# kohnakagawa/md_neighbor_list

Hardware: AMD Instinct MI355X
Metric: Verlet-list build ms and Mpairs/s at N=1M rho=1.0; achieved HBM GB/s (higher is better)
Workload: dtype f32

## Files before the change

### include/nl_hip.h

```cpp
#ifndef NL_HIP_H
#define NL_HIP_H

#include <stddef.h>
#include <stdint.h>

#ifdef __cplusplus
extern "C" {
#endif

typedef struct nl_handle_s* nl_handle_t;

typedef enum nl_dtype {
  NL_F32 = 0,
  NL_F64 = 1
} nl_dtype;

typedef enum nl_status {
  NL_OK = 0,
  NL_ERR_ARG = 1,
  NL_ERR_NOMEM = 2,
  NL_ERR_OUT_OF_BOX = 3,
  NL_ERR_CAPACITY = 4,
  NL_ERR_HIP = 5,
  NL_ERR_STATE = 6,
// ... 20 lines not shown

int nl_set_graph(nl_handle_t h, int on);

int nl_set_periodic(nl_handle_t h, int minimum_image);

int nl_set_periodic_axes(nl_handle_t h, int mask);
int nl_get_periodic_axes(nl_handle_t h, int* mask);

int nl_set_box(nl_handle_t h, double Lx, double Ly, double Lz, double xy, double xz, double yz);
int nl_get_box(nl_handle_t h, double box[6]);

int nl_destroy(nl_handle_t h);


int nl_make_list(nl_handle_t h, const void* q_dev, int32_t q_stride, int32_t n, void* stream, int sync);

#define NL_GID_IN_W ((const int32_t*)1)
int nl_make_list_slab(nl_handle_t h, const void* q_dev, int32_t q_stride, const int32_t* gid_dev, int32_t n_rows,
                      int32_t n, int32_t z_lo, int32_t z_hi, void* stream, int sync);

int nl_make_list_slab_begin(nl_handle_t h, const void* q_dev, int32_t q_stride, const int32_t* gid_dev, int32_t n_rows,
                            int32_t n, int32_t n_ghost_lo, int32_t z_lo, int32_t z_hi, void* stream);
int nl_make_list_slab_finish(nl_handle_t h, void* stream, int sync);

int nl_set_local_ids(nl_handle_t h, int on);
int nl_get_local_ids(nl_handle_t h, int* on);


typedef struct nl_comm_s* nl_comm_t;
#define NL_UNIQUE_ID_BYTES 128
typedef int (*nl_sendrecv_fn)(void* user, int peer_to, const void* send, size_t send_bytes, int peer_from, void* recv,
                              size_t recv_bytes);
int nl_comm_unique_id(void* id_out );
int nl_comm_create(nl_comm_t* out, int rank, int world, const void* unique_id, int device_id);
int nl_comm_create_callbacks(nl_comm_t* out, int rank, int world, nl_sendrecv_fn fn, void* user, int device_id);
int nl_comm_destroy(nl_comm_t comm);
int nl_comm_layers(nl_handle_t h, nl_comm_t comm, int32_t* z_lo, int32_t* z_hi);
int nl_make_list_distributed(nl_handle_t h, nl_comm_t comm, void* q_dev, int32_t q_capacity, int32_t n_owned, void* stream,
                             int sync);
int nl_distributed_ghosts(nl_comm_t comm, int32_t* n_ghost_lo, int32_t* n_ghost_hi);

int nl_synchronize(nl_handle_t h);


int nl_set_skin(nl_handle_t h, double skin);
int nl_update_list(nl_handle_t h, const void* q_dev, int32_t q_stride, int32_t n, void* stream, int sync);
int nl_get_update_stats(nl_handle_t h, int64_t stats[2]);


int nl_set_exclusions(nl_handle_t h, const int32_t* pairs_dev, int64_t n_pairs, int32_t n);
int nl_set_exclusions_global(nl_handle_t h, const int32_t* pairs_dev, int64_t n_pairs, int32_t n_ids);
int nl_get_exclusions(nl_handle_t h, const int32_t** offsets_dev, const int32_t** ids_dev, int32_t* n, int64_t* n_unique);


#define NL_MAX_TYPES 32
int nl_set_type_cutoffs(nl_handle_t h, const int32_t* types_dev, int32_t n, int32_t ntypes, const double* rc_host);
int nl_get_types(nl_handle_t h, const int32_t** types_dev, int32_t* n, int32_t* ntypes);


int nl_set_pair_images(nl_handle_t h, int on);
int nl_get_pair_images(nl_handle_t h, const int8_t** images_dev, int64_t* nentries);
int nl_pair_vectors(nl_handle_t h, const void* q_dev, int32_t q_stride, void* out_dev, void* stream);
int nl_pair_vectors_enqueue(nl_handle_t h, const void* q_dev, int32_t q_stride, void* out_dev, void* stream);


int nl_get_half_csr(nl_handle_t h, const int32_t** key_pointer_dev, const int32_t** sorted_list_dev,
                    const int32_t** number_of_partners_dev, int64_t* npairs);

int nl_get_full_csr(nl_handle_t h, const int32_t** key_pointer_dev, const int32_t** list_dev,
                    const int32_t** number_of_partners_dev, int64_t* nentries);

int nl_get_half_csr64(nl_handle_t h, const int64_t** key_pointer_dev, const int32_t** sorted_list_dev,
                      const int32_t** number_of_partners_dev, int64_t* npairs);
int nl_get_full_csr64(nl_handle_t h, const int64_t** key_pointer_dev, const int32_t** list_dev,
                      const int32_t** number_of_partners_dev, int64_t* nentries);

int nl_list_checksum(nl_handle_t h, uint64_t* checksum, int64_t* nentries);

int nl_get_full_transposed(nl_handle_t h, const int32_t** list_dev, const int32_t** count_dev, int64_t* row_stride,
                           int32_t* max_partners);

int nl_number_of_pairs(nl_handle_t h, int64_t* npairs);


int nl_get_cell_order(nl_handle_t h, const int32_t** order_dev, int32_t* n);
int nl_resort(nl_handle_t h, void* array_dev, size_t elem_bytes, void* stream);


int nl_lj_forces(nl_handle_t h, const void* q_dev, int32_t q_stride, double epsilon, double sigma, double rc_force,
                 void* f_dev, void* stream);
int nl_lj_forces_enqueue(nl_handle_t h, const void* q_dev, int32_t q_stride, double epsilon, double sigma, double rc_force,
                         void* f_dev, void* stream);
int nl_set_lj_type_params(nl_handle_t h, int32_t ntypes, const double* epsilon, const double* sigma, const double* rc_force);
int nl_lj_forces_typed(nl_handle_t h, const void* q_dev, int32_t q_stride, void* f_dev, void* stream);
int nl_lj_forces_typed_enqueue(nl_handle_t h, const void* q_dev, int32_t q_stride, void* f_dev, void* stream);

#define NL_VIRIAL_BLOCKS 2048
int nl_lj_virial(nl_handle_t h, const void* q_dev, int32_t q_stride, double epsilon, double sigma, double rc_force,
                 double* out_dev, void* stream);
int nl_lj_virial_enqueue(nl_handle_t h, const void* q_dev, int32_t q_stride, double epsilon, double sigma, double rc_force,
                         double* out_dev, void* stream);
int nl_lj_virial_typed(nl_handle_t h, const void* q_dev, int32_t q_stride, double* out_dev, void* stream);
int nl_lj_virial_typed_enqueue(nl_handle_t h, const void* q_dev, int32_t q_stride, double* out_dev, void* stream);

#define NL_TABLE_MAX_KNOTS 4096
#define NL_TABLE_BLOCKS 512
#define NL_TABLE_LDS_BYTES 65280
int nl_set_pair_table(nl_handle_t h, int32_t ntypes, int32_t nknots, double r_min, double r_max, const double* F_host,
                      const double* U_host);
int nl_get_pair_table(nl_handle_t h, int32_t* ntypes, int32_t* nknots, double* r_min, double* r_max);
int nl_table_forces(nl_handle_t h, const void* q_dev, int32_t q_stride, void* f_dev, void* stream);
int nl_table_forces_enqueue(nl_handle_t h, const void* q_dev, int32_t q_stride, void* f_dev, void* stream);
int nl_table_virial(nl_handle_t h, const void* q_dev, int32_t q_stride, double* out_dev, void* stream);
int nl_table_virial_enqueue(nl_handle_t h, const void* q_dev, int32_t q_stride, double* out_dev, void* stream);

int nl_set_eam(nl_handle_t h, int32_t ntypes, int32_t nknots_d, double r_min_d, double r_max_d, const double* f_host,
               const double* G_host, int32_t nknots_e, double rho_max, const double* E_host, const double* P_host);
int nl_get_eam(nl_handle_t h, int32_t* ntypes, int32_t* nknots_d, double* r_min_d, double* r_max_d, int32_t* nknots_e,
               double* rho_max, int32_t* lds_density, int32_t* lds_forces);
int nl_eam_forces(nl_handle_t h, const void* q_dev, int32_t q_stride, void* f_dev, void* stream);
int nl_eam_forces_enqueue(nl_handle_t h, const void* q_dev, int32_t q_stride, void* f_dev, void* stream);
int nl_eam_virial(nl_handle_t h, const void* q_dev, int32_t q_stride, double* out_dev, void* stream);
int nl_eam_virial_enqueue(nl_handle_t h, const void* q_dev, int32_t q_stride, double* out_dev, void* stream);
int nl_eam_get_density(nl_handle_t h, const void** rho_dev, const void** fp_dev, int32_t* n);

#define NL_SW_MAX_TYPES 4
#define NL_SW_MAX_NEAR 64
int nl_set_sw(nl_handle_t h, int32_t ntypes, int32_t nknots, double r_min_3, double r_max_3, const double* g_host,
              const double* G_host, const double* lambda_host, const double* cos0_host);
int nl_get_sw(nl_handle_t h, int32_t* ntypes, int32_t* nknots, double* r_min_3, double* r_max_3, int32_t* lds);
int nl_sw_forces(nl_handle_t h, const void* q_dev, int32_t q_stride, void* f_dev, void* stream);
int nl_sw_forces_enqueue(nl_handle_t h, const void* q_dev, int32_t q_stride, void* f_dev, void* stream);
int nl_sw_virial(nl_handle_t h, const void* q_dev, int32_t q_stride, double* out_dev, void* stream);
int nl_sw_virial_enqueue(nl_handle_t h, const void* q_dev, int32_t q_stride, double* out_dev, void* stream);

#define NL_HIST_MAX_BINS 4096
#define NL_HIST_LDS_COUNTERS 4096
int nl_pair_histogram(nl_handle_t h, const void* q_dev, int32_t q_stride, double r_max, int32_t nbins, uint64_t* hist_dev,
                      void* stream);
int nl_pair_histogram_enqueue(nl_handle_t h, const void* q_dev, int32_t q_stride, double r_max, int32_t nbins,
                              uint64_t* hist_dev, void* stream);
int nl_pair_histogram_typed(nl_handle_t h, const void* q_dev, int32_t q_stride, double r_max, int32_t nbins, uint64_t* hist_dev,
                            void* stream);
int nl_pair_histogram_typed_enqueue(nl_handle_t h, const void* q_dev, int32_t q_stride, double r_max, int32_t nbins,
                                    uint64_t* hist_dev, void* stream);


int nl_get_mesh(nl_handle_t h, int32_t mesh[3], int64_t* ncell);
int nl_get_sorted(nl_handle_t h, const int32_t** cell_start_dev, const void** sorted_pos_dev,
                  const int32_t** sorted_row_dev, int64_t* ncell_local);
int nl_debug_read(nl_handle_t h, uint64_t* out, int32_t n, int reset);
int nl_debug_occupancy(int32_t out[8]);
int nl_get_build_info(nl_handle_t h, int32_t info[8]);
int nl_get_build_stats(nl_handle_t h, int64_t stats[4]);
int nl_last_error(nl_handle_t h);
int nl_last_hip_error(nl_handle_t h);

enum {
  NL_STAGE_HASH = 0,
  NL_STAGE_CELL_SCAN = 1,
  NL_STAGE_REORDER = 2,
  NL_STAGE_COUNT = 3,
  NL_STAGE_ROW_SCAN = 4,
  NL_STAGE_FILL = 5,
  NL_STAGE_TOTAL = 6,
  NL_NUM_STAGES = 7
};
int nl_profile_stages(nl_handle_t h, const void* q_dev, int32_t q_stride, int32_t n, int32_t reps,
                      double ms[NL_NUM_STAGES]);
int nl_profile_last_build(nl_handle_t h, int32_t reps, double ms[NL_NUM_STAGES]);


int nl_buf_alloc(void** dev, void** host, size_t bytes);
int nl_buf_free(void* dev, void* host);
int nl_buf_h2d(void* dev, const void* host, size_t bytes);
int nl_buf_d2h(void* host, const void* dev, size_t bytes);
int nl_buf_fill32(void* dev, uint32_t pattern, size_t count);
int nl_buf_fill64(void* dev, uint64_t pattern, size_t count);
int nl_device_synchronize(void);
int nl_device_count(int* count);

#ifdef __cplusplus
}
#endif
#endif
```

### md_neighbor_list_amd/_lib.py

```python
from __future__ import annotations

import ctypes as C
import os

_HERE = os.path.dirname(os.path.abspath(__file__))
LIB_PATH = os.environ.get("NL_HIP_LIB") or os.path.join(_HERE, "lib", "libnl_hip.so")

NL_F32, NL_F64 = 0, 1
NL_OK = 0
(NL_ERR_ARG, NL_ERR_NOMEM, NL_ERR_OUT_OF_BOX, NL_ERR_CAPACITY, NL_ERR_HIP, NL_ERR_STATE, NL_ERR_MESH,
 NL_ERR_INDEX_OVERFLOW, NL_ERR_NO_DEVICE, NL_ERR_DOMAIN, NL_ERR_COMM) = range(1, 12)
NL_UNIQUE_ID_BYTES = 128
NL_MAX_TYPES = 32
SENDRECV_FN = C.CFUNCTYPE(C.c_int, C.c_void_p, C.c_int, C.c_void_p, C.c_size_t, C.c_int, C.c_void_p, C.c_size_t)
_P, _I32, _I64, _SZ, _D = C.c_void_p, C.c_int32, C.c_int64, C.c_size_t, C.c_double
NL_NUM_STAGES = 7
STAGE_NAMES = ("hash", "cell_scan", "reorder", "count", "row_scan", "fill", "total")

PROTOTYPES = {
    "nl_status_string": (C.c_char_p, [C.c_int]),
    "nl_create": (C.c_int, [C.POINTER(_P), C.c_int, _D, _D, _D, _D, C.c_int]),
    "nl_initialize": (C.c_int, [_P, _I32]),
    "nl_set_capacity": (C.c_int, [_P, _I64]),
    "nl_set_list_kind": (C.c_int, [_P, C.c_int]),
    "nl_set_periodic": (C.c_int, [_P, C.c_int]),
    "nl_set_periodic_axes": (C.c_int, [_P, C.c_int]),
    "nl_get_periodic_axes": (C.c_int, [_P, C.POINTER(C.c_int)]),
    "nl_set_box": (C.c_int, [_P, C.c_double, C.c_double, C.c_double, C.c_double, C.c_double, C.c_double]),
    "nl_get_box": (C.c_int, [_P, C.POINTER(C.c_double * 6)]),
    "nl_set_graph": (C.c_int, [_P, C.c_int]),
    "nl_set_local_ids": (C.c_int, [_P, C.c_int]),
    "nl_get_local_ids": (C.c_int, [_P, C.POINTER(C.c_int)]),
    "nl_destroy": (C.c_int, [_P]),
    "nl_make_list": (C.c_int, [_P, _P, _I32, _I32, _P, C.c_int]),
    "nl_make_list_slab": (C.c_int, [_P, _P, _I32, _P, _I32, _I32, _I32, _I32, _P, C.c_int]),
    "nl_make_list_slab_begin": (C.c_int, [_P, _P, _I32, _P, _I32, _I32, _I32, _I32, _I32, _P]),
    "nl_make_list_slab_finish": (C.c_int, [_P, _P, C.c_int]),
    "nl_synchronize": (C.c_int, [_P]),
    "nl_comm_unique_id": (C.c_int, [_P]),
    "nl_comm_create": (C.c_int, [C.POINTER(_P), C.c_int, C.c_int, _P, C.c_int]),
    "nl_comm_create_callbacks": (C.c_int, [C.POINTER(_P), C.c_int, C.c_int, SENDRECV_FN, _P, C.c_int]),
    "nl_comm_destroy": (C.c_int, [_P]),
    "nl_comm_layers": (C.c_int, [_P, _P, C.POINTER(_I32), C.POINTER(_I32)]),
    "nl_make_list_distributed": (C.c_int, [_P, _P, _P, _I32, _I32, _P, C.c_int]),
    "nl_distributed_ghosts": (C.c_int, [_P, C.POINTER(_I32), C.POINTER(_I32)]),
    "nl_get_half_csr": (C.c_int, [_P, C.POINTER(_P), C.POINTER(_P), C.POINTER(_P), C.POINTER(_I64)]),
    "nl_get_full_csr": (C.c_int, [_P, C.POINTER(_P), C.POINTER(_P), C.POINTER(_P), C.POINTER(_I64)]),
    "nl_get_half_csr64": (C.c_int, [_P, C.POINTER(_P), C.POINTER(_P), C.POINTER(_P), C.POINTER(_I64)]),
    "nl_get_full_csr64": (C.c_int, [_P, C.POINTER(_P), C.POINTER(_P), C.POINTER(_P), C.POINTER(_I64)]),
    "nl_list_checksum": (C.c_int, [_P, C.POINTER(C.c_uint64), C.POINTER(_I64)]),
    "nl_set_offset_width": (C.c_int, [_P, C.c_int]),
    "nl_get_cell_order": (C.c_int, [_P, C.POINTER(_P), C.POINTER(_I32)]),
    "nl_resort": (C.c_int, [_P, _P, _SZ, _P]),
    "nl_lj_forces": (C.c_int, [_P, _P, _I32, _D, _D, _D, _P, _P]),
    "nl_lj_forces_enqueue": (C.c_int, [_P, _P, _I32, _D, _D, _D, _P, _P]),
    "nl_set_skin": (C.c_int, [_P, _D]),
    "nl_update_list": (C.c_int, [_P, _P, _I32, _I32, _P, C.c_int]),
    "nl_get_update_stats": (C.c_int, [_P, C.POINTER(_I64 * 2)]),
    "nl_set_exclusions": (C.c_int, [_P, _P, _I64, _I32]),
    "nl_set_exclusions_global": (C.c_int, [_P, _P, _I64, _I32]),
    "nl_get_exclusions": (C.c_int, [_P, C.POINTER(_P), C.POINTER(_P), C.POINTER(_I32), C.POINTER(_I64)]),
    "nl_set_type_cutoffs": (C.c_int, [_P, _P, _I32, _I32, C.POINTER(_D)]),
    "nl_get_types": (C.c_int, [_P, C.POINTER(_P), C.POINTER(_I32), C.POINTER(_I32)]),
    "nl_set_lj_type_params": (C.c_int, [_P, _I32, C.POINTER(_D), C.POINTER(_D), C.POINTER(_D)]),
    "nl_lj_forces_typed": (C.c_int, [_P, _P, _I32, _P, _P]),
    "nl_lj_forces_typed_enqueue": (C.c_int, [_P, _P, _I32, _P, _P]),
    "nl_lj_virial": (C.c_int, [_P, _P, _I32, _D, _D, _D, _P, _P]),
    "nl_lj_virial_enqueue": (C.c_int, [_P, _P, _I32, _D, _D, _D, _P, _P]),
    "nl_lj_virial_typed": (C.c_int, [_P, _P, _I32, _P, _P]),
    "nl_lj_virial_typed_enqueue": (C.c_int, [_P, _P, _I32, _P, _P]),
    "nl_set_pair_table": (C.c_int, [_P, _I32, _I32, _D, _D, C.POINTER(_D), C.POINTER(_D)]),
    "nl_get_pair_table": (C.c_int, [_P, C.POINTER(_I32), C.POINTER(_I32), C.POINTER(_D), C.POINTER(_D)]),
    "nl_table_forces": (C.c_int, [_P, _P, _I32, _P, _P]),
    "nl_table_forces_enqueue": (C.c_int, [_P, _P, _I32, _P, _P]),
    "nl_table_virial": (C.c_int, [_P, _P, _I32, _P, _P]),
    "nl_table_virial_enqueue": (C.c_int, [_P, _P, _I32, _P, _P]),
    "nl_set_eam": (C.c_int, [_P, _I32, _I32, _D, _D, C.POINTER(_D), C.POINTER(_D), _I32, _D, C.POINTER(_D), C.POINTER(_D)]),
    "nl_get_eam": (C.c_int, [_P, C.POINTER(_I32), C.POINTER(_I32), C.POINTER(_D), C.POINTER(_D), C.POINTER(_I32), C.POINTER(_D),
                             C.POINTER(_I32), C.POINTER(_I32)]),
    "nl_eam_forces": (C.c_int, [_P, _P, _I32, _P, _P]),
    "nl_eam_forces_enqueue": (C.c_int, [_P, _P, _I32, _P, _P]),
    "nl_eam_virial": (C.c_int, [_P, _P, _I32, _P, _P]),
    "nl_eam_virial_enqueue": (C.c_int, [_P, _P, _I32, _P, _P]),
    "nl_eam_get_density": (C.c_int, [_P, C.POINTER(_P), C.POINTER(_P), C.POINTER(_I32)]),
    "nl_set_sw": (C.c_int, [_P, _I32, _I32, _D, _D, C.POINTER(_D), C.POINTER(_D), C.POINTER(_D), C.POINTER(_D)]),
    "nl_get_sw": (C.c_int, [_P, C.POINTER(_I32), C.POINTER(_I32), C.POINTER(_D), C.POINTER(_D), C.POINTER(_I32)]),
    "nl_sw_forces": (C.c_int, [_P, _P, _I32, _P, _P]),
    "nl_sw_forces_enqueue": (C.c_int, [_P, _P, _I32, _P, _P]),
    "nl_sw_virial": (C.c_int, [_P, _P, _I32, _P, _P]),
    "nl_sw_virial_enqueue": (C.c_int, [_P, _P, _I32, _P, _P]),
    "nl_pair_histogram": (C.c_int, [_P, _P, _I32, _D, _I32, _P, _P]),
    "nl_pair_histogram_enqueue": (C.c_int, [_P, _P, _I32, _D, _I32, _P, _P]),
    "nl_pair_histogram_typed": (C.c_int, [_P, _P, _I32, _D, _I32, _P, _P]),
    "nl_pair_histogram_typed_enqueue": (C.c_int, [_P, _P, _I32, _D, _I32, _P, _P]),
    "nl_set_pair_images": (C.c_int, [_P, C.c_int]),
    "nl_get_pair_images": (C.c_int, [_P, C.POINTER(_P), C.POINTER(_I64)]),
    "nl_pair_vectors": (C.c_int, [_P, _P, _I32, _P, _P]),
    "nl_pair_vectors_enqueue": (C.c_int, [_P, _P, _I32, _P, _P]),
    "nl_get_full_transposed": (C.c_int, [_P, C.POINTER(_P), C.POINTER(_P), C.POINTER(_I64), C.POINTER(_I32)]),
    "nl_number_of_pairs": (C.c_int, [_P, C.POINTER(_I64)]),
    "nl_get_mesh": (C.c_int, [_P, C.POINTER(_I32 * 3), C.POINTER(_I64)]),
    "nl_get_sorted": (C.c_int, [_P, C.POINTER(_P), C.POINTER(_P), C.POINTER(_P), C.POINTER(_I64)]),
    "nl_debug_read": (C.c_int, [_P, C.c_void_p, _I32, C.c_int]),
    "nl_debug_occupancy": (C.c_int, [C.POINTER(_I32 * 8)]),
    "nl_get_build_info": (C.c_int, [_P, C.POINTER(_I32 * 8)]),
    "nl_get_build_stats": (C.c_int, [_P, C.POINTER(_I64 * 4)]),
    "nl_last_error": (C.c_int, [_P]),
    "nl_last_hip_error": (C.c_int, [_P]),
    "nl_profile_stages": (C.c_int, [_P, _P, _I32, _I32, _I32, C.POINTER(_D * NL_NUM_STAGES)]),
    "nl_profile_last_build": (C.c_int, [_P, _I32, C.POINTER(_D * NL_NUM_STAGES)]),
    "nl_buf_alloc": (C.c_int, [C.POINTER(_P), C.POINTER(_P), _SZ]),
    "nl_buf_free": (C.c_int, [_P, _P]),
    "nl_buf_h2d": (C.c_int, [_P, _P, _SZ]),
    "nl_buf_d2h": (C.c_int, [_P, _P, _SZ]),
    "nl_buf_fill32": (C.c_int, [_P, C.c_uint32, _SZ]),
    "nl_buf_fill64": (C.c_int, [_P, C.c_uint64, _SZ]),
    "nl_device_synchronize": (C.c_int, []),
    "nl_device_count": (C.c_int, [C.POINTER(C.c_int)]),
}


class NLError(RuntimeError):

    def __init__(self, code, what=""):
        self.code = int(code)
        try:
            msg = load().nl_status_string(self.code).decode()
        except Exception:
            msg = "?"
        super().__init__(f"libnl_hip: status {self.code} ({msg}){' in ' + what if what else ''}")


_lib = None


def load():
    global _lib
    if _lib is None:
        if not os.path.exists(LIB_PATH):
            raise RuntimeError(
                f"{LIB_PATH} not found: the HIP extension is not built (run `make lib` or "
                "`python -c 'import __graft_entry__ as g; g.build()'`). There is no CPU fallback."
            )
        lib = C.CDLL(LIB_PATH)
        for name, (res, args) in PROTOTYPES.items():
            f = getattr(lib, name)
            f.restype, f.argtypes = res, args
        _lib = lib
    return _lib


def check(code, what=""):
    if code != NL_OK:
        raise NLError(code, what)
```

### md_neighbor_list_amd/csrc/nl_api.hip

```cpp
#include "../../include/nl_hip.h"

#include <hip/hip_runtime.h>

#include <algorithm>
#include <cmath>
#include <cstdio>
#include <cstdlib>
#include <cstring>
#include <new>
#include <tuple>
#include <type_traits>
#include <vector>

#include "nl_devbuf.hpp"
#include "nl_kernels.hpp"
#include "nl_stage.hpp"

using namespace nl;

namespace {

struct HostResult {
  uint32_t status;
  uint32_t tickets[17];
  uint32_t total_lo, total_hi;
  uint32_t bin_words[2];
  uint32_t kept_lo, kept_hi;
  int64_t total() const { return (int64_t)(((uint64_t)total_hi << 32) | total_lo); }
  int64_t kept() const { return (int64_t)(((uint64_t)kept_hi << 32) | kept_lo); }
};
constexpr int META_TOTAL = 18;
constexpr int META_FULL27 = 1;
constexpr int META_FILL_LIST = 10;
constexpr int META_WORDS = 20;
constexpr int META_KEPT = 22;
constexpr int META_WORDS_EXCL = 24;
constexpr int32_t LIST_QUIET_BUILDS = 4;

struct BuildArgs {
  const void* q = nullptr;
  int32_t stride = 4;
  const int32_t* gid = nullptr;
  int32_t n_rows = 0, n = 0;
  int32_t n_ghost_lo = 0;
  int32_t z_lo = 0, mzl = 0, slab = 0;
  const int32_t* dyn = nullptr;
  const int32_t* dyn_host = nullptr;
  int32_t n_est = 0;
  auto tie() const { return std::tie(q, stride, gid, n_rows, n, n_ghost_lo, z_lo, mzl, slab, dyn, dyn_host, n_est); }
  bool operator==(const BuildArgs& o) const { return tie() == o.tie(); }
};

enum Binning : int32_t {
  BINNING_BUCKET,
  BINNING_TWO_PASS,
  BINNING_ATOMIC,
};
enum Search : int32_t {
  SEARCH_ROWS,
  SEARCH_MASKS,
  SEARCH_DENSE,
  SEARCH_SWEEPS,
};

struct BuildPlan {
  int32_t binning = BINNING_ATOMIC;
  int32_t cap_row = 0;
  bool split = false;
  int32_t search = SEARCH_SWEEPS;
  int32_t rows_v = 0;
  int32_t mask_nb = 1;
  bool small = false;
  bool rows12 = false;
  bool list = true;
  bool full = false;
  bool wide = false;
  bool filter = false;
  bool images = false;
  int32_t pbc = 0;
  int32_t idc = 0;
  int32_t id_shift = 0;
  bool cull = false;
  bool id_rows = false;
  Box box = {{0, 0, 0}, 0, 0, 0};
  int32_t tilt = 0;
  bool rerun = false;
  auto tie() const {
    return std::tie(rerun, binning, cap_row, split, search, rows_v, mask_nb, small, rows12, list, full, wide, filter, images, pbc, idc, id_shift, cull, id_rows,
                    box.L[0], box.L[1], box.L[2], box.xy, box.xz, box.yz, tilt);
  }
  bool operator==(const BuildPlan& o) const { return tie() == o.tie(); }
};

struct GraphKey {
  BuildArgs args;
  BuildPlan plan;
  int64_t capacity = 0;
  uint64_t buffers_epoch = 0;
  uint64_t ex_gen = 0;
  uint64_t ty_gen = 0;
  int32_t update = 0;
  double skin = 0;
  auto tie() const { return std::tie(args, plan, capacity, buffers_epoch, ex_gen, ty_gen, update, skin); }
  bool operator==(const GraphKey& o) const { return tie() == o.tie(); }
};

}

struct nl_handle_s {
  int dtype = NL_F32, device = 0;
  double rc = 0, L[3] = {0, 0, 0}, rc2 = 0;
  int32_t m[3] = {0, 0, 0};
  int64_t ncell = 0;
  double xy = 0, xz = 0, yz = 0, shear[3] = {0, 0, 0}, L0[3] = {0, 0, 0};
  int64_t mesh_cells_cap = 0, mesh_rows_cap = 0;
  DevBuf<double> lat_dev;
  float ims_f[3];
  double ims_d[3];
  float rc2_f = 0;
  float ms_f[3];

  int32_t n_max = 0;
  int64_t capacity = 0;
  bool capacity_user = false;
  int list_kind = NL_LIST_HALF;
  int pbc = 0;
  bool local_ids = false;

  DevBuf<int32_t> rank;
  DevBuf<void> sorted;
  DevBuf<int32_t> sorted_row;
  DevBuf<int32_t> sorted_gid;
  DevBuf<int32_t> count;
  DevBuf<void> key_pointer;
  DevBuf<void> kp_alt;
  bool kp_alt_valid = false;
  int offset_width = 0;
  DevBuf<int32_t> progress;
  int32_t* row_count = nullptr;
  DevBuf<int32_t> row_start;
  DevBuf<int32_t> blk_base;
  DevBuf<void> tmp_pos;
  DevBuf<int32_t> tmp_row;
  size_t tmp_slots = 0;
  DevBuf<int32_t> row_cursor;
  int bucket_env = 1;
  int32_t bucket_scale = 1;
  bool bucket_off = false;
  int32_t bin_blocks = 0, bin_chunk = 0;
  bool bin_two_level = true;
  DevBuf<void> base_sorted;
  DevBuf<uint32_t> masks;
  DevBuf<int32_t> full27_list;
  DevBuf<void> resort_buf;
  int rows_env = -1;
  size_t dense_masks_limit = (size_t)64 << 30;
  int sweep_variant = 3;
  int num_cus = 256;
  DevBuf<unsigned long long> dbg_buf;
  int dbg_flags = 0;
  DevBuf<int32_t> cell_count;
  DevBuf<int32_t> cell_start;
  DevBuf<int32_t> cls_start;
  int idclass_env = 2;
  DevBuf<uint64_t> cull_bits;
  int cull_env = 1;
  DevBuf<uint64_t> scan_look;
  int32_t scan_blocks = 0;
  DevBuf<int64_t> totals;
  uint32_t* status = nullptr;
  DevBuf<int32_t> list;
  DevBuf<int32_t> t_list;
  DevBuf<int32_t> t_count;
  DevBuf<int32_t> t_cursor;
  int64_t t_rows_cap = 0;
  int32_t t_max = 0;
  bool t_valid = false;

  HostResult* host = nullptr;
  hipStream_t own_stream = nullptr;
  bool use_graph = false;
  hipGraph_t graph = nullptr;
  hipGraphExec_t graph_exec = nullptr;
  GraphKey graph_key;
  uint64_t buffers_epoch = 1;
  bool begun = false;
  hipStream_t last_stream = nullptr;
  hipEvent_t ev[NL_NUM_STAGES + 1] = {};

  BuildArgs args;
  BuildPlan plan;
  int32_t list_quiet = 0;
  int64_t reruns[2] = {0, 0};
  bool built = false, pending = false;
  int32_t n = 0, n_rows = 0;
  int last_error = NL_OK, last_hip = 0;

  double skin = 0;
  const uint32_t* gate = nullptr;
  DevBuf<void> snap;
  DevBuf<uint32_t> skin_words;
  bool upd_valid = false;
  bool last_update = false;
  const void* upd_q = nullptr;
  int32_t upd_stride = 0, upd_n = 0;

  DevBuf<int32_t> ex_off;
  DevBuf<int32_t> ex_ids;
  int32_t ex_n = 0;
  bool ex_global = false;
  int64_t ex_unique = 0;
  uint64_t ex_gen = 0;
  bool ex_relabel = false;
  DevBuf<void> kp_pre;
  DevBuf<int32_t> list_pre;

  DevBuf<int32_t> ty_types;
  DevBuf<void> ty_rc2;
  int32_t ty_n = 0, ty_ntypes = 0;
  double ty_rc[NL_MAX_TYPES * NL_MAX_TYPES] = {};
  uint64_t ty_gen = 0;
  DevBuf<void> lj_par;
  int32_t lj_ntypes = 0;
  double lj_rcf[NL_MAX_TYPES * NL_MAX_TYPES] = {};
  DevBuf<double> vir_part;

  struct TableSet {
    DevBuf<void> tab;
    int32_t ntypes = 0, nslots = 0, nknots = 0;
    double r_min = 0, r_max = 0;
    double x0 = 0, xc = 0, iD = 0;
    int lds_env = 1;
  };
  TableSet tb;
  TableSet ea;
  int32_t ea_nke = 0;
  double ea_rhomax = 0, ea_iDrho = 0;
  DevBuf<void> ea_part;
  TableSet sw;

  bool pair_images = false;
  DevBuf<uint32_t> images;
  DevBuf<uint16_t> img_code;
  DevBuf<uint32_t> img_words;
};

namespace {

#define HIPCHK(h, call)                         \
  do {                                          \
    hipError_t e_ = (call);                     \
    if (e_ != hipSuccess) {                     \
      (h)->last_hip = (int)e_;                  \
      (h)->last_error = NL_ERR_HIP;             \
      return NL_ERR_HIP;                        \
    }                                           \
  } while (0)

int fail(nl_handle_t h, int code) {
  if (h) h->last_error = code;
  return code;
}

int launch_exclude(nl_handle_t h, int32_t n_rows, hipStream_t s);
int excl_relabel(nl_handle_t h);
int launch_filter(nl_handle_t h, int32_t n_rows, hipStream_t s);
int types_relabel(nl_handle_t h);
int launch_images(nl_handle_t h, int32_t n_rows, hipStream_t s);

template <typename F> int dispatch_t_off(nl_handle_t h, F&& f) {
  const bool f32 = h->dtype == NL_F32;
  if (h->plan.wide) return f32 ? f(float(), int64_t()) : f(double(), int64_t());
  return f32 ? f(float(), int32_t()) : f(double(), int32_t());
}
template <typename F> void with_flag(bool v, F&& f) { v ? f(std::true_type()) : f(std::false_type()); }

int consumer_ready(nl_handle_t h, hipStream_t s, bool enqueue) {
  if (enqueue) {
    if (!h->pending && !h->built) return fail(h, NL_ERR_STATE);
    if (h->pending && (!h->last_update || s != h->last_stream)) return fail(h, NL_ERR_STATE);
  } else if (int rc = nl_synchronize(h)) {
    return rc;
  }
  if ((h->args.slab || h->n_rows != h->n) && (!h->local_ids || h->args.gid || h->args.dyn)) return fail(h, NL_ERR_STATE);
  return NL_OK;
}

bool filter_tables(nl_handle_t h) { return h->ex_ids || h->ty_types; }
bool filter_rows_only(nl_handle_t h) { return h->ty_types || (h->ex_ids && !h->ex_global); }
enum { PART_ALL = 0, PART_BEGIN = 1, PART_FINISH = 2 };

bool partial_build(const BuildArgs& a, int part) { return a.slab || a.gid || a.dyn || part != PART_ALL; }
bool excl_refuses(nl_handle_t h, const int32_t* gid, int32_t n_rows) {
  if (!h->ex_ids) return false;
  return h->ex_global ? !gid && n_rows > h->ex_n : n_rows != h->ex_n;
}
void* search_kp(nl_handle_t h) { return h->plan.filter ? h->kp_pre : h->key_pointer; }
int32_t* search_list(nl_handle_t h) { return h->plan.filter ? h->list_pre : h->list; }
int64_t list_total(nl_handle_t h) { return h->plan.filter ? h->host->kept() : h->host->total(); }

int hip_status(nl_handle_t h, hipError_t e) {
  if (e == hipSuccess) return NL_OK;
  (void)hipGetLastError();
  h->last_hip = (int)e;
  return fail(h, e == hipErrorOutOfMemory ? NL_ERR_NOMEM : NL_ERR_HIP);
}
template <typename T> int dev_alloc(nl_handle_t h, DevBuf<T>& b, size_t bytes, int64_t items = 0) {
  h->buffers_epoch++;
  return hip_status(h, b.replace(bytes, items));
}
template <typename T> int swap_alloc(nl_handle_t h, DevBuf<T>& b, size_t bytes, int64_t items = 0) {
  const hipError_t e = b.replace_keeping(bytes, items);
  if (e == hipSuccess) h->buffers_epoch++;
  return hip_status(h, e);
}
template <typename T> int side_alloc(nl_handle_t h, DevBuf<T>& b, size_t bytes) { return hip_status(h, b.replace(bytes)); }

constexpr int IMG_WORDS = 4;

// ... 47 lines not shown
    if ((rc = swap_alloc(h, h->row_start, 4 * (2 * rows_cap + 64)))) return rc;
    if ((rc = swap_alloc(h, h->blk_base, 4 * (rows_cap * (size_t)h->bin_blocks + 16)))) return rc;
    if ((rc = swap_alloc(h, h->row_cursor, 4 * (rows_cap + 16)))) return rc;
  }
  if (cells_cap > (size_t)h->mesh_cells_cap || rows_cap > (size_t)h->mesh_rows_cap) {
    if ((rc = swap_alloc(h, h->full27_list, 4 * (cells_cap + 16)))) return rc;
    if ((rc = swap_alloc(h, h->cell_count, 4 * (cells_cap + 64 + 2 * rows_cap)))) return rc;
    if ((rc = swap_alloc(h, h->cell_start, 4 * (4 * cells_cap + 32)))) return rc;
    if ((rc = swap_alloc(h, h->cls_start, 4 * (4 * cells_cap + 32)))) return rc;
    const size_t nblk = std::max<size_t>(n, cells_cap) / SCAN_BLOCK + 2;
    if ((rc = swap_alloc(h, h->scan_look, 8 * (nblk + 1)))) return rc;
    h->scan_blocks = (int32_t)nblk;
  }
  h->mesh_rows_cap = (int64_t)rows_cap, h->mesh_cells_cap = (int64_t)cells_cap;
  h->row_count = h->cell_count + h->ncell + 32;
  h->status = reinterpret_cast<uint32_t*>(h->cell_count + h->ncell);
  h->buffers_epoch++;
  HIPCHK(h, hipMemset(h->row_cursor, 0, 4 * (rows_cap + 16)));
  HIPCHK(h, hipMemset(h->scan_look, 0, 8 * ((size_t)h->scan_blocks + 1)));
  HIPCHK(h, hipMemset(h->cell_count, 0, 4 * (cells_cap + 64 + 2 * rows_cap)));
  return NL_OK;
}

float floor_to_float(double v) {
  float f = (float)v;
  if ((double)f > v) f = std::nextafterf(f, -INFINITY);
  return f;
}

int status_to_error(uint32_t st) {
  if (st & ST_OUT_OF_BOX) return NL_ERR_OUT_OF_BOX;
  if (st & ST_DOMAIN) return NL_ERR_DOMAIN;
  if (st & ST_ID_RANGE) return NL_ERR_ARG;
  if (st & ST_INDEX_OVERFLOW) return NL_ERR_INDEX_OVERFLOW;
  if (st & ST_CAPACITY) return NL_ERR_CAPACITY;
  return NL_OK;
}

bool has_tilt(nl_handle_t h) { return h->xy != 0 || h->xz != 0 || h->yz != 0; }
Box box_of(nl_handle_t h) { return Box{{h->L[0], h->L[1], h->L[2]}, h->xy, h->xz, h->yz}; }
void lattice_table(const Box& b, double* lat) {
  for (int wr = 0; wr < LATTICE_CODES; wr++) {
    const double na = (wr & 3) - 1, nb = ((wr >> 2) & 3) - 1, nc = ((wr >> 4) & 3) - 1;
    lat[3 * wr + 0] = (na * b.L[0] + nb * b.xy) + nc * b.xz;
    lat[3 * wr + 1] = nb * b.L[1] + nc * b.yz;
    lat[3 * wr + 2] = nc * b.L[2];
  }
}
bool box_changed(nl_handle_t h) {
  return has_tilt(h) || h->L[0] != h->L0[0] || h->L[1] != h->L0[1] || h->L[2] != h->L0[2];
}
bool tilt_mask_ok(nl_handle_t h) {
  return (h->xy == 0 || (h->pbc & 3) == 3) && (h->xz == 0 || (h->pbc & 5) == 5) && (h->yz == 0 || (h->pbc & 6) == 6);
}

template <typename T> Grid<T> make_grid(nl_handle_t h, const BuildArgs& a, int pbc) {
  Grid<T> g;
  for (int d = 0; d < 3; d++) {
    g.ims[d] = sizeof(T) == 4 ? (T)h->ims_f[d] : (T)h->ims_d[d];
    g.m[d] = h->m[d];
  }
  g.mzl = a.mzl;
  g.slab = a.slab;
  g.z_origin = a.slab ? ((a.z_lo - 1) % h->m[2] + h->m[2]) % h->m[2] : 0;
  g.n_rows = a.n_rows;
  g.pbc = pbc;
  g.dbg = h->dbg_flags;
  g.z_first = a.slab ? a.z_lo - 1 : 0;
  for (int d = 0; d < 3; d++) g.L[d] = (T)h->L[d];
  g.gate = h->gate;
  g.tilt = has_tilt(h) ? 1 : 0;
  for (int d = 0; d < 3; d++) g.k[d] = (T)h->shear[d];
  g.lat = h->lat_dev;
  return g;
}

template <typename OFF>
int launch_scan(nl_handle_t h, const int32_t* in, int64_t n, OFF* out, int64_t* total, hipStream_t s,
                uint32_t* total_split = nullptr) {
  if (n <= 0) {
    HIPCHK(h, hipMemsetAsync(out, 0, sizeof(OFF), s));
    HIPCHK(h, hipMemsetAsync(total, 0, sizeof(int64_t), s));
    if (total_split) HIPCHK(h, hipMemsetAsync(total_split, 0, 2 * sizeof(uint32_t), s));
    return NL_OK;
  }
  if (n <= SCAN_SMALL_MAX) {
    hipLaunchKernelGGL(k_scan_small<OFF>, dim3(1), dim3(1024), 0, s, in, (int32_t)n, total, out, total_split, h->gate);
    return NL_OK;
  }
  const int32_t nb = (int32_t)((n + SCAN_BLOCK - 1) / SCAN_BLOCK);
  if (nb > h->scan_blocks) return fail(h, NL_ERR_ARG);
  hipLaunchKernelGGL(k_scan_chained<OFF>, dim3(nb), dim3(SCAN_THREADS), 0, s, in, n, h->scan_look, h->scan_blocks, total, out,
                     h->status, total_split, h->gate);
  return NL_OK;
}

int32_t stage_grid(nl_handle_t h, int32_t units) { return std::max(1, std::min((units + 3) / 4, 16 * h->num_cus)); }

template <typename OFF, typename A>
int launch_passes(nl_handle_t h, int32_t n_rows, int32_t units, hipStream_t s, const A& a, void (*count)(A, int32_t*),
                  void (*compact)(A, const OFF*, int32_t*)) {
  const dim3 grid(stage_grid(h, units));
  if (n_rows > 0) hipLaunchKernelGGL(count, grid, dim3(STAGE_THREADS), 0, s, a, h->count);
  if (int rc = launch_scan(h, h->count, n_rows, static_cast<OFF*>(h->key_pointer), h->totals + 2, s, h->status + META_KEPT)) return rc;
  if (n_rows > 0) hipLaunchKernelGGL(compact, grid, dim3(STAGE_THREADS), 0, s, a, static_cast<const OFF*>(h->key_pointer), h->list);
  HIPCHK(h, hipGetLastError());
  return NL_OK;
}

FastDiv fastdiv_make(uint32_t d) {
  FastDiv f;
  f.d = d;
  uint32_t s = 0;
  while ((1ull << s) < d) s++;
  f.s = s;
  f.m = (uint32_t)(((1ull << 32) * ((1ull << s) - d)) / d + 1);
  return f;
}

template <typename T> SweepArgs<T> sweep_args(nl_handle_t h) {
  SweepArgs<T> a;
  a.sorted = static_cast<const Pos<T>*>(h->sorted);
  a.sorted_row = h->sorted_row;
  a.sorted_gid = h->plan.id_rows ? h->sorted_row : h->sorted_gid;
  a.cell_start = h->cell_start;
  a.cls_start = h->cls_start;
  a.mx = h->m[0], a.my = h->m[1], a.mzl = h->args.mzl, a.slab = h->args.slab;
  a.div_mx = fastdiv_make((uint32_t)h->m[0]), a.div_my = fastdiv_make((uint32_t)h->m[1]);
  a.rc2 = sizeof(T) == 4 ? (T)h->rc2_f : (T)h->rc2;
  a.count = h->count;
  a.progress = h->progress;
  a.key_pointer = search_kp(h);
  a.wide = h->plan.wide ? 1 : 0;
  a.n_rows = h->n_rows;
  a.list = search_list(h);
  a.total = h->totals + 1;
  a.capacity = h->capacity;
  a.status = h->status;
  a.masks = h->masks;
  a.masks_hi = reinterpret_cast<uint8_t*>(h->masks.get()) + h->masks.bytes() / MASK_ROW_BYTES * MASK_LO_BYTES;
  a.isplit = 1;
  a.mask_nb = h->plan.mask_nb;
  a.full27_list = h->full27_list;
  a.full27_count = reinterpret_cast<int32_t*>(h->status) + META_FULL27;
  a.fill_list_count = reinterpret_cast<int32_t*>(h->status) + META_FILL_LIST;
  a.pbc = h->plan.pbc;
  for (int d = 0; d < 3; d++) a.ms[d] = (T)(h->L[d] / h->m[d]);
  for (int d = 0; d < 3; d++) a.L[d] = (T)h->L[d];
  a.z_origin = h->args.slab ? h->args.z_lo - 1 : 0;
  a.dbg = h->dbg_flags;
  a.dbg_buf = h->dbg_buf;
  a.gate = h->gate;
  a.cull_bits = h->plan.cull ? h->cull_bits.get() : nullptr;
  for (int d = 0; d < 3; d++) a.k[d] = (T)h->shear[d];
  a.lat = h->lat_dev;
  return a;
}

RowsArgs rows_args(nl_handle_t h) {
  RowsArgs a;
  a.sorted = static_cast<const Pos<float>*>(h->sorted);
  a.sorted_row = h->sorted_row, a.sorted_gid = h->plan.id_rows ? h->sorted_row : h->sorted_gid;
  a.fine_start = h->cell_start;
  a.mx = h->m[0], a.my = h->m[1], a.mzl = h->args.mzl, a.slab = h->args.slab;
  a.div_mx = fastdiv_make((uint32_t)h->m[0]), a.div_my = fastdiv_make((uint32_t)h->m[1]);
  a.rc2 = h->rc2_f;
  a.count = h->count;
  a.masks = h->masks;
  a.key_pointer = search_kp(h);
  a.list = search_list(h);
  a.total = h->totals + 1;
  a.capacity = h->capacity;
  a.status = h->status;
  a.over_list = h->full27_list;
  a.over_count = reinterpret_cast<int32_t*>(h->status) + META_FULL27;
  a.wide = h->plan.wide ? 1 : 0;
  a.dbg_buf = h->dbg_buf;
  a.gate = h->gate;
  return a;
}

template <int V, bool FULL, typename OFF> void launch_rows(nl_handle_t h, int mode, int32_t ncells, hipStream_t s) {
  const RowsArgs a = rows_args(h);
  const int32_t over_grid = 2 * h->num_cus;
  if (mode == MODE_COUNT) {
    hipLaunchKernelGGL((k_sweep_rows_f32<V, FULL>), dim3(ncells), dim3(ROWS_WAVES * WAVE), 0, s, a);
    hipLaunchKernelGGL((k_rows_overflow<MODE_COUNT, FULL, int32_t>), dim3(over_grid), dim3(ROWS_WAVES * WAVE), 0, s, a);
    return;
  }
  hipLaunchKernelGGL((k_fill_rows<V, FULL, OFF>), dim3(ncells), dim3(ROWS_FW * WAVE), 0, s, a);
  hipLaunchKernelGGL((k_rows_overflow<MODE_FILL, FULL, OFF>), dim3(over_grid), dim3(ROWS_WAVES * WAVE), 0, s, a);
}

template <typename T, bool FULL, bool PBC, typename OFF> void launch_search(nl_handle_t h, int mode, hipStream_t s) {
  const BuildPlan& p = h->plan;
  const int32_t ncells = h->m[0] * h->m[1] * (h->args.slab ? h->args.mzl - 2 : h->args.mzl);
  constexpr bool F32_OPEN = sizeof(T) == 4 && !PBC;
  if (p.search == SEARCH_ROWS) {
    if constexpr (F32_OPEN) {
      if (p.rows_v == 0) launch_rows<0, FULL, OFF>(h, mode, ncells, s);
      else if (p.rows_v == 1) launch_rows<1, FULL, OFF>(h, mode, ncells, s);
      else launch_rows<2, FULL, OFF>(h, mode, ncells, s);
    }
    return;
  }
  const SweepArgs<T> a = sweep_args<T>(h);
  const dim3 cells(ncells), wg(SWEEP_WAVES * WAVE), list_grid(2 * h->num_cus);
  auto count_masks = [&] {
    if constexpr (sizeof(T) == 4) hipLaunchKernelGGL((k_sweep_count_masks_f32<FULL, PBC>), cells, wg, 0, s, a);
    else hipLaunchKernelGGL((k_sweep<T, MODE_COUNT_MASKS, FULL, PBC>), cells, wg, 0, s, a);
  };
  switch (p.search) {
    case SEARCH_MASKS:
      if (mode == MODE_COUNT) {
        if constexpr (F32_OPEN) {
          constexpr int CAP = SweepCfg<float>::CAP;
          if (p.small && p.id_rows) hipLaunchKernelGGL((k_sweep_lean_f32<FULL, 2, LEAN_SMALL_CAP, true>), cells, dim3(2 * WAVE), 0, s, a);
          else if (p.small) hipLaunchKernelGGL((k_sweep_lean_f32<FULL, 2, LEAN_SMALL_CAP>), cells, dim3(2 * WAVE), 0, s, a);
          else if (!FULL && p.idc == 2) hipLaunchKernelGGL((k_sweep_class_f32<2>), cells, wg, 0, s, a);
          else if (!FULL && p.idc == 4) hipLaunchKernelGGL((k_sweep_class_f32<4>), cells, wg, 0, s, a);
          else if (p.id_rows) hipLaunchKernelGGL((k_sweep_lean_f32<FULL, SWEEP_WAVES, CAP, true>), cells, wg, 0, s, a);
          else hipLaunchKernelGGL((k_sweep_lean_f32<FULL>), cells, wg, 0, s, a);
          if (p.list) hipLaunchKernelGGL((k_sweep_list_f32<FULL>), list_grid, wg, 0, s, a);
        } else {
          count_masks();
        }
        return;
      }
      if (p.small) {
        if constexpr (F32_OPEN)
          hipLaunchKernelGGL((k_fill_masks<T, FULL, PBC, OFF, 24, 1, SweepCfg<T>::CAP / 2>), cells, dim3(WAVE), 0, s, a);
      } else if (F32_OPEN && !FULL && p.idc) {
        if constexpr (F32_OPEN && !FULL) {
          constexpr int CAP = SweepCfg<T>::CAP;
          if (p.rows12 && p.idc == 2) hipLaunchKernelGGL((k_fill_masks<T, false, false, OFF, 12, EXPAND_WAVES, CAP, 2>), cells, dim3(EXPAND_WAVES * WAVE), 0, s, a);
          else if (p.rows12) hipLaunchKernelGGL((k_fill_masks<T, false, false, OFF, 12, EXPAND_WAVES, CAP, 4>), cells, dim3(EXPAND_WAVES * WAVE), 0, s, a);
          else if (p.idc == 2) hipLaunchKernelGGL((k_fill_masks<T, false, false, OFF, 24, EXPAND_WAVES, CAP, 2>), cells, dim3(EXPAND_WAVES * WAVE), 0, s, a);
          else hipLaunchKernelGGL((k_fill_masks<T, false, false, OFF, 24, EXPAND_WAVES, CAP, 4>), cells, dim3(EXPAND_WAVES * WAVE), 0, s, a);
        }
      } else if (p.rows12) {
        hipLaunchKernelGGL((k_fill_masks<T, FULL, PBC, OFF, 12>), cells, dim3(EXPAND_WAVES * WAVE), 0, s, a);
      } else {
        hipLaunchKernelGGL((k_fill_masks<T, FULL, PBC, OFF, 24>), cells, dim3(EXPAND_WAVES * WAVE), 0, s, a);
      }
      if (p.list) hipLaunchKernelGGL((k_fill_list<T, FULL, PBC>), list_grid, wg, 0, s, a);
      return;
    case SEARCH_DENSE:
      if (mode == MODE_COUNT) {
        count_masks();
        return;
      }
      if (h->n > 0)
        hipLaunchKernelGGL(k_row_base<OFF>, dim3((h->n + 255) / 256), dim3(256), 0, s, static_cast<const OFF*>(search_kp(h)),
                           h->sorted_row, h->n_rows, h->n, static_cast<OFF*>(h->base_sorted), h->gate);
      hipLaunchKernelGGL((k_fill_dense<T, FULL, PBC, OFF>), cells, dim3(FD_WAVES * WAVE), 0, s, a, static_cast<const OFF*>(h->base_sorted));
      return;
    default:
      if (mode == MODE_FILL) hipLaunchKernelGGL((k_sweep<T, MODE_FILL, FULL, PBC>), cells, wg, 0, s, a);
      else if constexpr (sizeof(T) == 4) hipLaunchKernelGGL((k_sweep_count_f32<FULL, PBC>), cells, wg, 0, s, a);
      else hipLaunchKernelGGL((k_sweep<T, MODE_COUNT, FULL, PBC>), cells, wg, 0, s, a);
  }
}

template <typename T, typename OFF> void launch_sweep_kind(nl_handle_t h, int mode, hipStream_t s) {
  const bool pbc = h->plan.pbc != 0;
  if (h->plan.full) pbc ? launch_search<T, true, true, OFF>(h, mode, s) : launch_search<T, true, false, OFF>(h, mode, s);
  else pbc ? launch_search<T, false, true, OFF>(h, mode, s) : launch_search<T, false, false, OFF>(h, mode, s);
}

template <typename T> void launch_sweep(nl_handle_t h, int mode, hipStream_t s) {
  if (h->plan.wide) launch_sweep_kind<T, int64_t>(h, mode, s);
  else launch_sweep_kind<T, int32_t>(h, mode, s);
}

bool mask_rows_ready(nl_handle_t h, int64_t nb, size_t row_bytes = MASK_ROW_BYTES) {
  const size_t need = row_bytes * (size_t)nb * ((size_t)h->n_max + 64);
  if (need > h->dense_masks_limit) return false;
  if (need > h->masks.bytes() || !h->masks) return dev_alloc(h, h->masks, need) == NL_OK;
  return true;
}

bool cull_bits_ready(nl_handle_t h, int64_t cells) {
  return follow(h, h->cull_bits, cells, sizeof(uint64_t) * CULL_WORDS * (size_t)cells) == NL_OK;
}

bool two_level_ok(nl_handle_t h, int32_t mzl) {
  return h->bin_two_level && (int64_t)h->m[1] * mzl <= BIN_MAX_ROWS && h->m[0] <= BIN_MAX_MX;
}

bool rows_layout_ok(nl_handle_t h, int32_t mzl) {
  const int64_t nrows = (int64_t)h->m[1] * mzl;
  return h->bin_two_level && nrows <= BIN_MAX_ROWS && h->m[0] <= BIN_FINE_MAX_MX && 4 * (int64_t)h->m[0] * nrows < 2147483000LL;
}
bool rows_margin_ok(nl_handle_t h) {
  const double ms = h->L[2] / h->m[2];
  return ms / h->rc >= 1.0 + 8.0 * h->m[2] * 5.9604644775390625e-8 + 9.5367431640625e-7;
}

template <typename T> int32_t bucket_cap(nl_handle_t h, int32_t n, int32_t mzl) {
  if (!h->bucket_env || h->bucket_off || !two_level_ok(h, mzl)) return 0;
  const int64_t nrows = (int64_t)h->m[1] * mzl;
  const int64_t cap = (int64_t)h->bucket_scale * ((int64_t)(1.25 * (double)n / (double)nrows) + 256);
  const size_t slots = (size_t)(nrows * cap) + 16;
  if (slots > 4 * ((size_t)h->n_max + 16) + 512 * (size_t)nrows) {
    h->bucket_off = true;
    return 0;
  }
  if (slots > h->tmp_slots) {
    if (dev_alloc(h, h->tmp_pos, sizeof(Pos<T>) * slots) || dev_alloc(h, h->tmp_row, sizeof(int32_t) * slots)) {
      h->bucket_off = true;
      h->tmp_slots = 0;
      const size_t n_slots = (size_t)h->n_max + 16;
      if (dev_alloc(h, h->tmp_pos, sizeof(Pos<T>) * n_slots) == NL_OK && dev_alloc(h, h->tmp_row, sizeof(int32_t) * n_slots) == NL_OK)
        h->tmp_slots = n_slots, h->last_error = NL_OK;
      return 0;
    }
    h->tmp_slots = slots;
  }
  return (int32_t)cap;
}

template <typename T> BuildPlan plan_build(nl_handle_t h, const BuildArgs& a, int part, bool rerun) {
  BuildPlan p;
  p.rerun = rerun;
  p.full = h->list_kind == NL_LIST_FULL;
  p.pbc = h->pbc;
  p.box = box_of(h);
  p.tilt = has_tilt(h) ? 1 : 0;
  p.filter = filter_tables(h);
  p.images = h->pair_images;
  p.wide = h->offset_width == 64 || (h->offset_width == 0 && h->capacity > 2147483647LL);

  const int32_t n = a.dyn ? a.n_est : a.n;
  const int64_t ncl = (int64_t)h->m[0] * h->m[1] * a.mzl;
  const bool variant3 = h->sweep_variant >= 3;
  const double mean_stream = ncl > 0 ? 27.0 * n / (double)ncl : 0.0;
  const bool sparse_enough = mean_stream <= 0.85 * SweepCfg<T>::CAP;
  bool masks = variant3 && sparse_enough && mask_rows_ready(h, 1);
  bool rows = false;
  if (sizeof(T) == 4 && variant3 && p.pbc == 0 && h->rows_env != 0 && rows_layout_ok(h, a.mzl) && rows_margin_ok(h)) {
    int v = -1;
    if (h->rows_env > 0 && h->rows_env <= 3) {
      v = h->rows_env - 1;
    } else if (h->rows_env == 4 || !sparse_enough) {
      const double span = mean_stream * 27.0 / 36.0;
      const int cap[3] = {RowsCfg<0>::CAP, RowsCfg<1>::CAP, RowsCfg<2>::CAP}, bits[3] = {16, 32, 32};
      for (int k = 0; k < 3 && v < 0; k++)
        if (mean_stream + 5.0 * std::sqrt(mean_stream) <= cap[k] && span + 6.0 * std::sqrt(span) <= 64.0 * bits[k]) v = k;
    }
    if (v >= 0 && mask_rows_ready(h, 1, v == 0 ? 128 : 256)) rows = true, p.rows_v = v, masks = true;
  }
  if (variant3 && !sparse_enough) {
    const int64_t nb = (int64_t)((mean_stream + 5.0 * std::sqrt(mean_stream) + 64.0) / SweepCfg<T>::CAP) + 1;
    if (nb <= FD_NB && mask_rows_ready(h, nb)) masks = true, p.mask_nb = (int32_t)nb;
  }
  p.search = rows ? SEARCH_ROWS : !masks ? SEARCH_SWEEPS : p.mask_nb > 1 ? SEARCH_DENSE : SEARCH_MASKS;
  p.small = sizeof(T) == 4 && p.search == SEARCH_MASKS && p.pbc == 0 &&
            mean_stream + 5.0 * std::sqrt(mean_stream) <= (double)LEAN_SMALL_CAP;
  p.rows12 = (double)a.n <= 21.0 * (double)std::max<int64_t>(1, ncl);

  const bool two_level = two_level_ok(h, a.mzl);
  p.split = part != PART_ALL && two_level && a.slab;
  const bool again_ok = !p.split && !a.dyn && !rerun;
  p.list = !again_ok || h->list_quiet < LIST_QUIET_BUILDS;
  p.cap_row = again_ok ? bucket_cap<T>(h, n, a.mzl) : 0;
  p.binning = !two_level ? BINNING_ATOMIC : p.cap_row > 0 ? BINNING_BUCKET : BINNING_TWO_PASS;
  p.id_rows = !a.gid && !p.tilt && p.binning != BINNING_ATOMIC;
  if (sizeof(T) == 4 && p.search == SEARCH_MASKS && !p.small && !p.full && p.pbc == 0 && h->idclass_env > 0 && !a.gid &&
      !a.slab && !a.dyn && !p.split && p.binning != BINNING_ATOMIC && h->m[0] * h->idclass_env <= 4 * BIN_FINE_MAX_MX &&
      h->m[0] >= 3 && h->m[1] >= 3 && a.mzl >= 3 && n > 0) {
    p.idc = h->idclass_env;
    while (((uint32_t)(n - 1) >> p.id_shift) >= (uint32_t)p.idc) p.id_shift++;
    p.cull = h->cull_env != 0 && cull_bits_ready(h, ncl);
  }
  return p;
}

BuildPlan plan_for(nl_handle_t h, const BuildArgs& a, int part, bool rerun) {
  return h->dtype == NL_F32 ? plan_build<float>(h, a, part, rerun) : plan_build<double>(h, a, part, rerun);
}

void adopt_build(nl_handle_t h, const BuildArgs& a, const BuildPlan& p) {
  h->args = a;
  h->plan = p;
  h->ex_relabel = true;
  h->kp_alt_valid = false;
}

template <typename T, bool BUCKET, typename L> void launch_unrolled(nl_handle_t h, L&& launch) {
  auto by_id = [&](auto u) {
    if (h->plan.id_rows) launch(u, std::true_type());
    else launch(u, std::false_type());
  };
  if constexpr (sizeof(T) == 4 || !BUCKET) {
    if (h->bin_chunk >= 8 * BIN_THREADS) return by_id(std::integral_constant<int, 8>());
  }
  by_id(std::integral_constant<int, 4>());
}

template <typename T>
void launch_bin_cells(nl_handle_t h, const Grid<T>& g, int32_t grid, int32_t nrows, const int32_t* row_start, const BinPhase& ph,
                      int32_t cap_row, hipStream_t s) {
  auto launch_as = [&](auto fine, auto idc, auto idrow) {
    hipLaunchKernelGGL((k_bin_cells<T, decltype(fine)::value, decltype(idc)::value, decltype(idrow)::value>), dim3(grid), dim3(256), 0, s, g, nrows, row_start,
                       static_cast<const Pos<T>*>(h->tmp_pos), h->tmp_row, h->cell_start, static_cast<Pos<T>*>(h->sorted),
                       h->sorted_row, h->sorted_gid, ph, cap_row, h->cls_start, h->plan.id_shift);
  };
  auto launch = [&](auto fine, auto idc) {
    if constexpr (decltype(idc)::value > 0) {
      launch_as(fine, idc, std::true_type());
    } else {
      if (h->plan.id_rows) launch_as(fine, idc, std::true_type());
      else launch_as(fine, idc, std::false_type());
    }
  };
  if constexpr (sizeof(T) == 4) {
    if (h->plan.search == SEARCH_ROWS) return launch(std::true_type(), std::integral_constant<int, 0>());
    if (h->plan.idc == 2) return launch(std::false_type(), std::integral_constant<int, 2>());
    if (h->plan.idc == 4) return launch(std::false_type(), std::integral_constant<int, 4>());
  }
  launch(std::false_type(), std::integral_constant<int, 0>());
}

template <typename T>
int enqueue_build(nl_handle_t h, const BuildArgs& a, const BuildPlan& p, hipStream_t s, hipEvent_t* ev, int part = PART_ALL) {
  adopt_build(h, a, p);
  if (p.filter && (excl_refuses(h, a.gid, a.n_rows) || (h->ty_types && a.n != h->ty_n) || (filter_rows_only(h) && partial_build(a, part))))
    return fail(h, NL_ERR_STATE);
  if (p.images && partial_build(a, part)) return fail(h, NL_ERR_STATE);
  if (!stage_ready(h, p)) return fail(h, NL_ERR_NOMEM);
  if (part != PART_ALL && !p.split) {
    if (part == PART_BEGIN) return NL_OK;
    part = PART_ALL;
  }
  const Grid<T> g = make_grid<T>(h, a, p.pbc);
  const int32_t n = a.n, nrows = h->m[1] * a.mzl, my = h->m[1];
  const T* q = static_cast<const T*>(a.q);
  auto run_pass = [&](const BinPhase& ph, int32_t* rc_arr, int32_t* rs_arr, int32_t cells_grid, bool events) {
    const int32_t np = ph.i_end - ph.i_beg;
    const int32_t blocks = std::max(1, (np + h->bin_chunk - 1) / h->bin_chunk);
    hipLaunchKernelGGL((k_bin_rows<T>), dim3(blocks), dim3(BIN_THREADS), 0, s, q, a.stride, n, h->bin_chunk, g, nrows, rc_arr,
                       h->blk_base, h->status, ph);
    if (events) (void)hipEventRecord(ev[NL_STAGE_CELL_SCAN], s);
    if (events) (void)hipEventRecord(ev[NL_STAGE_REORDER], s);
    launch_unrolled<T, false>(h, [&](auto u, auto idrow) {
      hipLaunchKernelGGL((k_bin_scatter<T, decltype(u)::value, decltype(idrow)::value>), dim3(blocks), dim3(BIN_THREADS), 0, s, q, a.stride, a.gid, n,
                         h->bin_chunk, g, nrows, rc_arr, rs_arr, h->blk_base, static_cast<Pos<T>*>(h->tmp_pos), h->tmp_row,
                         h->status, ph);
    });
    launch_bin_cells<T>(h, g, cells_grid, nrows, rs_arr, ph, 0, s);
  };
  switch (p.binning) {
    case BINNING_BUCKET: {
      if (ev) HIPCHK(h, hipEventRecord(ev[NL_STAGE_HASH], s));
      const int32_t blocks = std::max(1, (n + h->bin_chunk - 1) / h->bin_chunk);
      launch_unrolled<T, true>(h, [&](auto u, auto idrow) {
        hipLaunchKernelGGL((k_bin_bucket<T, decltype(u)::value, decltype(idrow)::value>), dim3(blocks), dim3(BIN_THREADS), 0, s, q, a.stride, a.gid, n,
                           h->bin_chunk, g, nrows, p.cap_row, h->row_cursor, h->row_start, static_cast<Pos<T>*>(h->tmp_pos),
                           h->tmp_row, h->status);
      });
      if (ev) HIPCHK(h, hipEventRecord(ev[NL_STAGE_CELL_SCAN], s));
      if (ev) HIPCHK(h, hipEventRecord(ev[NL_STAGE_REORDER], s));
      const BinPhase all = {0, n, nrows, 0, 0, 0, nrows, nrows, -1, nullptr};
      launch_bin_cells<T>(h, g, nrows, nrows, h->row_start, all, p.cap_row, s);
      break;
    }
    case BINNING_TWO_PASS:
      if (part == PART_ALL) {
        if (!h->gate) HIPCHK(h, hipMemsetAsync(h->cell_count + h->ncell, 0, sizeof(int32_t) * (size_t)(32 + nrows), s));
        if (ev) HIPCHK(h, hipEventRecord(ev[NL_STAGE_HASH], s));
        const BinPhase all = {0, n, nrows, 0, 0, 0, nrows, nrows, -1, a.dyn};
        run_pass(all, h->row_count, h->row_start, nrows, ev != nullptr);
      } else if (part == PART_BEGIN) {
        HIPCHK(h, hipMemsetAsync(h->cell_count + h->ncell, 0, sizeof(int32_t) * (size_t)(32 + 2 * (size_t)nrows), s));
        const BinPhase owned = {0, a.n_rows, nrows, a.n_ghost_lo, a.n_ghost_lo, my, nrows - 2 * my, nrows, -1};
        run_pass(owned, h->row_count, h->row_start, nrows - 2 * my, false);
        HIPCHK(h, hipGetLastError());
        return NL_OK;
      } else {
        const BinPhase ghosts = {a.n_rows, n, nrows - my, 0, a.n_rows, 0, my, nrows - my, a.n_ghost_lo};
        run_pass(ghosts, h->row_count + nrows, h->row_start + nrows + 16, 2 * my, false);
      }
      break;
    default: {
      const int32_t nbp = (n + 255) / 256;
      if (h->gate) {
        const int64_t words = h->ncell + 32;
        hipLaunchKernelGGL(k_zero_words, dim3((uint32_t)std::min<int64_t>((words + 1023) / 1024, 2048)), dim3(256), 0, s, h->cell_count, words, h->gate);
      } else {
        HIPCHK(h, hipMemsetAsync(h->cell_count, 0, sizeof(int32_t) * (size_t)(h->ncell + 32), s));
      }
      if (ev) HIPCHK(h, hipEventRecord(ev[NL_STAGE_HASH], s));
      if (n > 0) hipLaunchKernelGGL((k_hash<T>), dim3(nbp), dim3(256), 0, s, q, a.stride, n, g, h->cell_count, h->rank, h->status);
      if (ev) HIPCHK(h, hipEventRecord(ev[NL_STAGE_CELL_SCAN], s));
      if (int rc = launch_scan(h, h->cell_count, (int64_t)h->m[0] * h->m[1] * a.mzl, h->cell_start.get(), h->totals, s)) return rc;
      if (ev) HIPCHK(h, hipEventRecord(ev[NL_STAGE_REORDER], s));
      if (n > 0)
        hipLaunchKernelGGL((k_reorder<T>), dim3(nbp), dim3(256), 0, s, q, a.stride, a.gid, n, g, h->cell_start, h->rank,
                           static_cast<Pos<T>*>(h->sorted), h->sorted_row, h->sorted_gid);
    }
  }
  if (ev) HIPCHK(h, hipEventRecord(ev[NL_STAGE_COUNT], s));
  launch_sweep<T>(h, MODE_COUNT, s);
  if (ev) HIPCHK(h, hipEventRecord(ev[NL_STAGE_ROW_SCAN], s));
  if (p.wide) {
    if (int rc = launch_scan(h, h->count, a.n_rows, static_cast<int64_t*>(search_kp(h)), h->totals + 1, s, h->status + META_TOTAL)) return rc;
  } else {
    if (int rc = launch_scan(h, h->count, a.n_rows, static_cast<int32_t*>(search_kp(h)), h->totals + 1, s, h->status + META_TOTAL)) return rc;
  }
  if (ev) HIPCHK(h, hipEventRecord(ev[NL_STAGE_FILL], s));
  launch_sweep<T>(h, MODE_FILL, s);
  if (p.filter)
    if (int rc = launch_filter(h, a.n_rows, s)) return rc;
  if (p.images)
    if (int rc = launch_images(h, a.n_rows, s)) return rc;
  if (ev) HIPCHK(h, hipEventRecord(ev[NL_STAGE_TOTAL], s));
  HIPCHK(h, hipGetLastError());
  return NL_OK;
}

int enqueue_result_copy(nl_handle_t h, hipStream_t s) {
  const int words = h->plan.filter ? META_WORDS_EXCL : META_WORDS;
  HIPCHK(h, hipMemcpyAsync(h->host, h->status, sizeof(uint32_t) * words, hipMemcpyDeviceToHost, s));
  return NL_OK;
}

// ... 147 lines not shown
  return NL_OK;
}

template <typename T, typename OFF>
__global__ void __launch_bounds__(256) k_list_checksum(const OFF* __restrict__ kp, const int32_t* __restrict__ list, int32_t n_rows,
                                                       const int32_t* __restrict__ gid, const T* __restrict__ q,
                                                       unsigned long long* __restrict__ acc) {
  __shared__ unsigned long long part[4];
  const int lane = threadIdx.x & 63, w = threadIdx.x >> 6;
  unsigned long long h = 0;
  for (int64_t row = (int64_t)blockIdx.x * 4 + w; row < n_rows; row += (int64_t)gridDim.x * 4) {
    uint32_t id = (uint32_t)row;
    if (gid == reinterpret_cast<const int32_t*>(1)) {
      if constexpr (sizeof(T) == 4) id = (uint32_t)__float_as_int(q[(size_t)row * 4 + 3]);
      else id = (uint32_t)__double_as_longlong(q[(size_t)row * 4 + 3]);
    } else if (gid) {
      id = (uint32_t)gid[row];
    }
    const OFF b = kp[row], e = kp[row + 1];
    for (OFF k = b + lane; k < e; k += 64) {
      unsigned long long v = ((unsigned long long)id << 32) | (uint32_t)list[k];
      v *= 0x9E3779B97F4A7C15ULL;
      v ^= v >> 29;
      h += v;
    }
  }
#pragma unroll
  for (int d = 32; d > 0; d >>= 1) h += __shfl_xor(h, d, 64);
  if (lane == 0) part[w] = h;
  __syncthreads();
  if (threadIdx.x == 0) atomicAdd(acc, part[0] + part[1] + part[2] + part[3]);
}

template <int W>
__global__ void __launch_bounds__(256) k_gather_words(const uint32_t* __restrict__ src, const int32_t* __restrict__ order, int32_t n,
                                                      uint32_t* __restrict__ dst) {
  const int32_t s = blockIdx.x * blockDim.x + threadIdx.x;
  if (s >= n) return;
  const uint32_t* p = src + (size_t)order[s] * W;
  uint32_t* d = dst + (size_t)s * W;
  if constexpr (W % 4 == 0) {
#pragma unroll
    for (int k = 0; k < W / 4; k++) reinterpret_cast<uint4*>(d)[k] = reinterpret_cast<const uint4*>(p)[k];
  } else if constexpr (W % 2 == 0) {
#pragma unroll
    for (int k = 0; k < W / 2; k++) reinterpret_cast<uint2*>(d)[k] = reinterpret_cast<const uint2*>(p)[k];
  } else {
#pragma unroll
    for (int k = 0; k < W; k++) d[k] = p[k];
  }
}

int get_csr(nl_handle_t h, bool full, int width, const void** key_pointer_dev, const int32_t** list_dev,
            const int32_t** number_of_partners_dev, int64_t* nentries) {
  if (!h) return NL_ERR_ARG;
  int rc = nl_synchronize(h);
  if (rc) return rc;
  if (h->plan.full != full) return fail(h, NL_ERR_STATE);
  if (key_pointer_dev)
    if ((rc = key_pointer_as(h, width, key_pointer_dev))) return rc;
  if (!key_pointer_dev && width == 32 && list_total(h) > 2147483647LL) return fail(h, NL_ERR_INDEX_OVERFLOW);
  if (list_dev) *list_dev = h->list;
  if (number_of_partners_dev) *number_of_partners_dev = h->count;
  if (nentries) *nentries = list_total(h);
  return NL_OK;
}
}


extern "C" {

const char* nl_status_string(int s) {
  switch (s) {
    case NL_OK: return "ok";
    case NL_ERR_ARG: return "bad argument";
    case NL_ERR_NOMEM: return "out of memory";
    case NL_ERR_OUT_OF_BOX: return "particle more than one box length outside the box (or NaN)";
    case NL_ERR_CAPACITY: return "pair list capacity exceeded";
    case NL_ERR_HIP: return "HIP runtime error";
    case NL_ERR_STATE: return "call order violated";
    case NL_ERR_MESH: return "fewer than 3 cells along an axis";
    case NL_ERR_INDEX_OVERFLOW: return "more than INT32_MAX list entries behind a 32-bit key_pointer";
    case NL_ERR_NO_DEVICE: return "no usable HIP device";
    case NL_ERR_DOMAIN: return "particle outside the layers declared for this rank";
    case NL_ERR_COMM: return "communication failed (RCCL not loadable, communicator or transport error)";
    default: return "unknown status";
  }
}

int nl_device_count(int* count) {
  if (!count) return NL_ERR_ARG;
  int c = 0;
  if (hipGetDeviceCount(&c) != hipSuccess) c = 0;
  *count = c;
  return NL_OK;
}

int nl_create(nl_handle_t* out, int dtype, double rc, double Lx, double Ly, double Lz, int device_id) {
  if (!out) return NL_ERR_ARG;
  *out = nullptr;
  if ((dtype != NL_F32 && dtype != NL_F64) || !(rc > 0) || !(Lx > 0) || !(Ly > 0) || !(Lz > 0)) return NL_ERR_ARG;
  const double L[3] = {Lx, Ly, Lz};
  int32_t m[3];
  for (int d = 0; d < 3; d++) {
    const double r = L[d] / rc;
    if (!(r < 2147483647.0)) return NL_ERR_ARG;
    m[d] = (int32_t)r;
    if (m[d] < 3) return NL_ERR_MESH;
  }
  if ((double)m[0] * m[1] * m[2] > 2.0e9) return NL_ERR_ARG;
  int ndev = 0;
  if (hipGetDeviceCount(&ndev) != hipSuccess || ndev <= 0) return NL_ERR_NO_DEVICE;
  int dev = device_id;
  if (dev < 0 && hipGetDevice(&dev) != hipSuccess) return NL_ERR_NO_DEVICE;
  if (dev >= ndev) return NL_ERR_ARG;
  if (hipSetDevice(dev) != hipSuccess) return NL_ERR_NO_DEVICE;

  nl_handle_t h = new (std::nothrow) nl_handle_s();
  if (!h) return NL_ERR_NOMEM;
  h->dtype = dtype, h->device = dev, h->rc = rc;
  h->rc2 = rc * rc;
  h->rc2_f = floor_to_float(h->rc2);
  for (int d = 0; d < 3; d++) {
    h->L[d] = L[d], h->m[d] = m[d], h->L0[d] = L[d];
    const float ms_f = (float)(L[d] / m[d]);
    h->ms_f[d] = ms_f;
    h->ims_f[d] = (float)(1.0 / (double)ms_f);
    const double ms_d = L[d] / m[d];
    h->ims_d[d] = 1.0 / ms_d;
  }
  h->ncell = (int64_t)m[0] * m[1] * m[2];
  double lat0[LATTICE_CODES * 3];
  lattice_table(box_of(h), lat0);
  if (h->lat_dev.replace(sizeof(lat0)) != hipSuccess ||
      hipMemcpy(h->lat_dev, lat0, sizeof(lat0), hipMemcpyHostToDevice) != hipSuccess ||
      hipStreamCreateWithFlags(&h->own_stream, hipStreamNonBlocking) != hipSuccess ||
      hipHostMalloc(reinterpret_cast<void**>(&h->host), sizeof(HostResult), hipHostMallocDefault) != hipSuccess) {
    nl_destroy(h);
    return NL_ERR_HIP;
  }
  for (auto& e : h->ev)
    if (hipEventCreate(&e) != hipSuccess) {
      nl_destroy(h);
      return NL_ERR_HIP;
    }
  memset(h->host, 0, sizeof(HostResult));
  {
    hipDeviceProp_t prop;
    if (hipGetDeviceProperties(&prop, dev) == hipSuccess && prop.multiProcessorCount > 0) h->num_cus = prop.multiProcessorCount;
    if (const char* v = getenv("NL_SWEEP_VARIANT")) h->sweep_variant = atoi(v) <= 1 ? 1 : 3;
    if (const char* v = getenv("NL_ROWS")) h->rows_env = std::max(-1, std::min(atoi(v), 4));
    if (const char* v = getenv("NL_IDCLASS")) h->idclass_env = atoi(v) >= 4 ? 4 : atoi(v) >= 2 ? 2 : 0;
    if (const char* v = getenv("NL_CULL")) h->cull_env = atoi(v) != 0;
    if (const char* v = getenv("NL_OFFSET_WIDTH")) h->offset_width = atoi(v) == 64 ? 64 : atoi(v) == 32 ? 32 : 0;
    if (const char* v = getenv("NL_BINNING")) h->bin_two_level = atoi(v) != 1;
    if (const char* v = getenv("NL_BIN_BUCKETS")) h->bucket_env = atoi(v) != 0;
    if (const char* v = getenv("NL_GRAPH")) h->use_graph = atoi(v) != 0;
    if (const char* v = getenv("NL_DEBUG_FLAGS")) h->dbg_flags = atoi(v);
  }
  *out = h;
  return NL_OK;
}

int nl_destroy(nl_handle_t h) {
  if (!h) return NL_ERR_ARG;
  (void)hipSetDevice(h->device);
  if (h->pending && h->last_stream) (void)hipStreamSynchronize(h->last_stream);
  if (h->host) (void)hipHostFree(h->host);
  for (auto& e : h->ev)
    if (e) (void)hipEventDestroy(e);
  if (h->graph_exec) (void)hipGraphExecDestroy(h->graph_exec);
  if (h->graph) (void)hipGraphDestroy(h->graph);
  if (h->own_stream) (void)hipStreamDestroy(h->own_stream);
  delete h;
  return NL_OK;
}

int nl_initialize(nl_handle_t h, int32_t n_max) {
  if (!h || n_max < 0) return fail(h, NL_ERR_ARG);
  HIPCHK(h, hipSetDevice(h->device));
  if (h->pending) {
    int rc = finish(h, false);
    (void)rc;
  }
  h->built = false;
  h->upd_valid = false;
  const size_t n = (size_t)n_max;
  const size_t pos_bytes = h->dtype == NL_F32 ? sizeof(Pos<float>) : sizeof(Pos<double>);
  int rc;
  if ((rc = dev_alloc(h, h->rank, 4 * (n + 16)))) return rc;
  if ((rc = dev_alloc(h, h->sorted, pos_bytes * (n + 16)))) return rc;
  if ((rc = dev_alloc(h, h->sorted_row, 4 * (n + 64)))) return rc;
  if ((rc = dev_alloc(h, h->sorted_gid, 4 * (n + 16)))) return rc;
  if ((rc = dev_alloc(h, h->count, 4 * (n + 32)))) return rc;
  HIPCHK(h, hipMemset(h->count, 0, 4 * (n + 32)));
  if ((rc = dev_alloc(h, h->key_pointer, 8 * (n + 32)))) return rc;
  h->kp_alt.release();
  h->kp_alt_valid = false;
  h->resort_buf.release();
  h->ea_part.release();
  h->t_list.release(), h->t_count.release(), h->t_cursor.release();
  h->t_rows_cap = 0;
  if ((rc = dev_alloc(h, h->progress, 4 * (n + 16)))) return rc;
  if ((rc = dev_alloc(h, h->base_sorted, 8 * (n + 64)))) return rc;
  h->bin_chunk = n >= (1 << 19) ? 8192 : 4096;
  if (const char* v = getenv("NL_DEBUG_BIN_CHUNK")) h->bin_chunk = std::max(1024, atoi(v));
  while ((n + h->bin_chunk - 1) / h->bin_chunk > 1024) h->bin_chunk *= 2;
  h->bin_blocks = (int32_t)((n + h->bin_chunk - 1) / h->bin_chunk);
  if (h->bin_blocks < 1) h->bin_blocks = 1;
  if ((rc = dev_alloc(h, h->tmp_pos, pos_bytes * (n + 16)))) return rc;
  if ((rc = dev_alloc(h, h->tmp_row, 4 * (n + 16)))) return rc;
  h->tmp_slots = n + 16;
  if (h->sweep_variant >= 3)
    if ((rc = dev_alloc(h, h->masks, (size_t)MASK_ROW_BYTES * (n + 64)))) return rc;
  if ((rc = dev_alloc(h, h->dbg_buf, 8 * (64 + 4 * 4096)))) return rc;
  HIPCHK(h, hipMemset(h->dbg_buf, 0, 8 * (64 + 4 * 4096)));
  if ((rc = dev_alloc(h, h->totals, 8 * 4))) return rc;
  HIPCHK(h, hipMemset(h->totals, 0, 32));
  for (DevBuf<int32_t>* b : {&h->row_start, &h->blk_base, &h->row_cursor, &h->full27_list, &h->cell_count, &h->cell_start, &h->cls_start})
    b->release();
  h->scan_look.release();
  h->mesh_cells_cap = h->mesh_rows_cap = 0;
  if ((rc = reserve_mesh(h, n))) return rc;
  h->n_max = n_max;
  if ((rc = estimate_capacity(h))) return rc;
  h->t_valid = false;
  return stage_reserve(h);
}

int nl_set_periodic_axes(nl_handle_t h, int mask) {
  if (!h) return NL_ERR_ARG;
  if (mask < 0 || mask > 7) return fail(h, NL_ERR_ARG);
  HIPCHK(h, hipSetDevice(h->device));
  if (h->pending) (void)finish(h, false);
  h->upd_valid = false;
  if (mask != h->pbc) {
    h->pbc = mask;
    h->built = false;
    h->t_valid = false;
  }
  return NL_OK;
}

int nl_set_box(nl_handle_t h, double Lx, double Ly, double Lz, double xy, double xz, double yz) {
  if (!h) return NL_ERR_ARG;
  const double L[3] = {Lx, Ly, Lz};
  for (double v : {Lx, Ly, Lz, xy, xz, yz})
    if (!std::isfinite(v)) return fail(h, NL_ERR_ARG);
  if (!(Lx > 0) || !(Ly > 0) || !(Lz > 0)) return fail(h, NL_ERR_ARG);
  const double sx = (xy * yz - Ly * xz) / (Ly * Lz);
  const double w[3] = {Lx / std::sqrt(1.0 + (xy / Ly) * (xy / Ly) + sx * sx), Ly / std::sqrt(1.0 + (yz / Lz) * (yz / Lz)), Lz};
  int32_t m[3];
  for (int d = 0; d < 3; d++) {
    const double r = w[d] / h->rc;
    if (!(r < 2147483647.0)) return fail(h, NL_ERR_ARG);
    m[d] = (int32_t)r;
  }
  if ((double)m[0] * m[1] * m[2] > 2.0e9) return fail(h, NL_ERR_ARG);
  for (int d = 0; d < 3; d++)
    if (m[d] < 3) return fail(h, NL_ERR_MESH);
  HIPCHK(h, hipSetDevice(h->device));
  if (h->pending) (void)finish(h, false);
  if (Lx == h->L[0] && Ly == h->L[1] && Lz == h->L[2] && xy == h->xy && xz == h->xz && yz == h->yz) return NL_OK;
  double old_L[3], old_ims_d[3], old_shear[3];
  float old_ms_f[3], old_ims_f[3];
  int32_t old_m[3];
  for (int d = 0; d < 3; d++)
    old_L[d] = h->L[d], old_m[d] = h->m[d], old_ms_f[d] = h->ms_f[d], old_ims_f[d] = h->ims_f[d], old_ims_d[d] = h->ims_d[d],
    old_shear[d] = h->shear[d];
  const double old_tilt[3] = {h->xy, h->xz, h->yz};
  const int64_t old_ncell = h->ncell;
  auto restore = [&](int rc) {
    for (int d = 0; d < 3; d++)
      h->L[d] = old_L[d], h->m[d] = old_m[d], h->ms_f[d] = old_ms_f[d], h->ims_f[d] = old_ims_f[d], h->ims_d[d] = old_ims_d[d],
      h->shear[d] = old_shear[d];
    h->xy = old_tilt[0], h->xz = old_tilt[1], h->yz = old_tilt[2];
    h->ncell = old_ncell;
    if (h->mesh_cells_cap > 0) (void)reserve_mesh(h, (size_t)h->n_max);
    double lat[LATTICE_CODES * 3];
    lattice_table(box_of(h), lat);
    (void)hipMemcpy(h->lat_dev, lat, sizeof(lat), hipMemcpyHostToDevice);
    return fail(h, rc);
  };
  for (int d = 0; d < 3; d++) {
    h->L[d] = L[d], h->m[d] = m[d];
    const float ms_f = (float)(L[d] / m[d]);
    h->ms_f[d] = ms_f;
    h->ims_f[d] = (float)(1.0 / (double)ms_f);
    h->ims_d[d] = 1.0 / (L[d] / m[d]);
  }
  h->xy = xy, h->xz = xz, h->yz = yz;
  h->shear[0] = xy / Ly, h->shear[1] = (xz * Ly - xy * yz) / (Ly * Lz), h->shear[2] = yz / Lz;
  h->ncell = (int64_t)m[0] * m[1] * m[2];
  if (h->mesh_cells_cap > 0) {
    if (int rc = reserve_mesh(h, (size_t)h->n_max)) return restore(rc);
    if (!h->capacity_user) {
      const int64_t want = estimate_want(h);
      if (want > h->capacity) {
        if (int rc = swap_alloc(h, h->list, 4 * (size_t)want)) return restore(rc);
        h->capacity = want;
      }
    }
    if (int rc = stage_reserve(h)) return restore(rc);
  }
  double lat[LATTICE_CODES * 3];
  lattice_table(box_of(h), lat);
// ... 195 lines not shown
  if (!h || !checksum) return fail(h, NL_ERR_ARG);
  int rc = nl_synchronize(h);
  if (rc) return rc;
  HIPCHK(h, hipSetDevice(h->device));
  hipStream_t s = h->last_stream;
  unsigned long long* acc = reinterpret_cast<unsigned long long*>(h->totals + 3);
  HIPCHK(h, hipMemsetAsync(acc, 0, 8, s));
  const int32_t n = h->n_rows;
  if (n > 0) {
    const int32_t grid = std::max(1, std::min((n + 3) / 4, 8 * h->num_cus));
    const bool w = h->plan.wide, f32 = h->dtype == NL_F32;
    const int32_t* gid = h->args.gid;
    const void* q = h->args.q;
    if (f32 && !w)
      hipLaunchKernelGGL((k_list_checksum<float, int32_t>), dim3(grid), dim3(256), 0, s, static_cast<const int32_t*>(h->key_pointer), h->list, n, gid, static_cast<const float*>(q), acc);
    else if (f32)
      hipLaunchKernelGGL((k_list_checksum<float, int64_t>), dim3(grid), dim3(256), 0, s, static_cast<const int64_t*>(h->key_pointer), h->list, n, gid, static_cast<const float*>(q), acc);
    else if (!w)
      hipLaunchKernelGGL((k_list_checksum<double, int32_t>), dim3(grid), dim3(256), 0, s, static_cast<const int32_t*>(h->key_pointer), h->list, n, gid, static_cast<const double*>(q), acc);
    else
      hipLaunchKernelGGL((k_list_checksum<double, int64_t>), dim3(grid), dim3(256), 0, s, static_cast<const int64_t*>(h->key_pointer), h->list, n, gid, static_cast<const double*>(q), acc);
    HIPCHK(h, hipGetLastError());
  }
  unsigned long long out = 0;
  HIPCHK(h, hipMemcpyAsync(&out, acc, 8, hipMemcpyDeviceToHost, s));
  HIPCHK(h, hipStreamSynchronize(s));
  *checksum = (uint64_t)out;
  if (nentries) *nentries = list_total(h);
  return NL_OK;
}

int nl_get_cell_order(nl_handle_t h, const int32_t** order_dev, int32_t* n) {
  if (!h) return NL_ERR_ARG;
  int rc = nl_synchronize(h);
  if (rc) return rc;
  if (order_dev) *order_dev = h->sorted_row;
  if (n) *n = h->n;
  return NL_OK;
}

int nl_resort(nl_handle_t h, void* array_dev, size_t elem_bytes, void* stream) {
  if (!h || !array_dev || elem_bytes == 0 || elem_bytes % 4 != 0 || elem_bytes > 32 || elem_bytes == 20 || elem_bytes == 28)
    return fail(h, NL_ERR_ARG);
  int rc = nl_synchronize(h);
  if (rc) return rc;
  if (h->args.slab || h->n_rows != h->n) return fail(h, NL_ERR_STATE);
  h->upd_valid = false;
  HIPCHK(h, hipSetDevice(h->device));
  const int32_t n = h->n;
  if (n == 0) return NL_OK;
  if (h->ex_relabel) {
    if (h->ex_ids && !h->ex_global && h->ex_n == n)
      if ((rc = excl_relabel(h))) return rc;
    if (h->ty_types && h->ty_n == n)
      if ((rc = types_relabel(h))) return rc;
    h->ex_relabel = false;
  }
  if (!h->resort_buf)
    if ((rc = side_alloc(h, h->resort_buf, 32 * ((size_t)h->n_max + 16)))) return rc;
  hipStream_t s = (hipStream_t)stream;
  if (s != h->last_stream) HIPCHK(h, hipStreamSynchronize(h->last_stream));
  const uint32_t* src = static_cast<const uint32_t*>(array_dev);
  uint32_t* buf = static_cast<uint32_t*>(h->resort_buf);
  const dim3 grid((n + 255) / 256), block(256);
  switch (elem_bytes / 4) {
    case 1: hipLaunchKernelGGL(k_gather_words<1>, grid, block, 0, s, src, h->sorted_row, n, buf); break;
    case 2: hipLaunchKernelGGL(k_gather_words<2>, grid, block, 0, s, src, h->sorted_row, n, buf); break;
    case 3: hipLaunchKernelGGL(k_gather_words<3>, grid, block, 0, s, src, h->sorted_row, n, buf); break;
    case 4: hipLaunchKernelGGL(k_gather_words<4>, grid, block, 0, s, src, h->sorted_row, n, buf); break;
    case 6: hipLaunchKernelGGL(k_gather_words<6>, grid, block, 0, s, src, h->sorted_row, n, buf); break;
    default: hipLaunchKernelGGL(k_gather_words<8>, grid, block, 0, s, src, h->sorted_row, n, buf); break;
  }
  HIPCHK(h, hipGetLastError());
  HIPCHK(h, hipMemcpyAsync(array_dev, buf, elem_bytes * (size_t)n, hipMemcpyDeviceToDevice, s));
  return NL_OK;
}

int nl_set_offset_width(nl_handle_t h, int bits) {
  if (!h || (bits != 0 && bits != 32 && bits != 64)) return fail(h, NL_ERR_ARG);
  HIPCHK(h, hipSetDevice(h->device));
  if (h->pending) (void)finish(h, false);
  h->upd_valid = false;
  if (bits != h->offset_width) {
    h->offset_width = bits;
    h->built = false;
    h->t_valid = false;
  }
  return NL_OK;
}

int nl_number_of_pairs(nl_handle_t h, int64_t* npairs) {
  if (!h || !npairs) return fail(h, NL_ERR_ARG);
  int rc = nl_synchronize(h);
  if (rc) return rc;
  *npairs = h->plan.full ? list_total(h) / 2 : list_total(h);
  return NL_OK;
}

int nl_get_mesh(nl_handle_t h, int32_t mesh[3], int64_t* ncell) {
  if (!h) return NL_ERR_ARG;
  if (mesh)
    for (int d = 0; d < 3; d++) mesh[d] = h->m[d];
  if (ncell) *ncell = h->ncell;
  return NL_OK;
}

int nl_get_sorted(nl_handle_t h, const int32_t** cell_start_dev, const void** sorted_pos_dev,
                  const int32_t** sorted_row_dev, int64_t* ncell_local) {
  if (!h) return NL_ERR_ARG;
  int rc = nl_synchronize(h);
  if (rc) return rc;
  if (cell_start_dev) *cell_start_dev = h->cell_start;
  if (sorted_pos_dev) *sorted_pos_dev = h->sorted;
  if (sorted_row_dev) *sorted_row_dev = h->sorted_row;
  if (ncell_local) *ncell_local = (int64_t)h->m[0] * h->m[1] * h->args.mzl;
  return NL_OK;
}

int nl_debug_read(nl_handle_t h, uint64_t* out, int32_t n, int reset) {
  if (!h || !out || !h->dbg_buf || n < 0 || n > 64 + 4 * 4096) return NL_ERR_ARG;
  HIPCHK(h, hipDeviceSynchronize());
  HIPCHK(h, hipMemcpy(out, h->dbg_buf, 8 * (size_t)n, hipMemcpyDeviceToHost));
  if (reset) HIPCHK(h, hipMemset(h->dbg_buf, 0, 8 * (64 + 4 * 4096)));
  return NL_OK;
}

int nl_debug_occupancy(int32_t out[8]) {
  if (!out) return NL_ERR_ARG;
  int v = 0;
  hipDeviceProp_t prop;
  if (hipGetDeviceProperties(&prop, 0) != hipSuccess) return NL_ERR_NO_DEVICE;
  out[0] = (int32_t)(prop.maxSharedMemoryPerMultiProcessor / 1024);
  out[1] = (int32_t)(prop.sharedMemPerBlock / 1024);
  out[2] = out[3] = 0;
  (void)hipOccupancyMaxActiveBlocksPerMultiprocessor(&v, k_sweep_count_f32<false, false>, SWEEP_WAVES * WAVE, 0);
  out[4] = v;
  (void)hipOccupancyMaxActiveBlocksPerMultiprocessor(&v, k_sweep<float, MODE_FILL>, SWEEP_WAVES * WAVE, 0);
  out[5] = v;
  hipFuncAttributes fa;
  (void)hipFuncGetAttributes(&fa, reinterpret_cast<const void*>(k_sweep_count_masks_f32<false, false>));
  out[6] = (int32_t)fa.sharedSizeBytes;
  out[7] = fa.numRegs;
  return NL_OK;
}

int nl_get_build_info(nl_handle_t h, int32_t info[8]) {
  if (!h || !info) return NL_ERR_ARG;
  for (int k = 4; k < 8; k++) info[k] = 0;
  const BuildPlan& p = h->plan;
  info[4] = p.wide ? 64 : 32;
  info[5] = p.mask_nb;
  info[6] = p.search == SEARCH_ROWS ? 1 + p.rows_v : 0;
  const int32_t binning = p.binning == BINNING_TWO_PASS ? 0 : p.binning == BINNING_BUCKET ? 1 : 2;
  info[7] = (p.small ? 1 : 0) | p.idc << 8 | binning << 16 | (p.cull ? 1 : 0) << 18;
  info[0] = p.search != SEARCH_SWEEPS ? 1 : 0;
  info[1] = h->sweep_variant;
  info[2] = h->dtype == NL_F32 ? SweepCfg<float>::CAP : SweepCfg<double>::CAP;
  info[3] = h->num_cus;
  return NL_OK;
}

int nl_get_build_stats(nl_handle_t h, int64_t stats[4]) {
  if (!h || !stats) return NL_ERR_ARG;
  stats[0] = h->reruns[0];
  stats[1] = h->reruns[1];
  stats[2] = h->plan.cap_row;
  stats[3] = h->plan.list ? 1 : 0;
  return NL_OK;
}

int nl_last_error(nl_handle_t h) { return h ? h->last_error : NL_ERR_ARG; }
int nl_last_hip_error(nl_handle_t h) { return h ? h->last_hip : 0; }

int nl_profile_last_build(nl_handle_t h, int32_t reps, double ms[NL_NUM_STAGES]) {
  if (!h || !ms || reps <= 0) return fail(h, NL_ERR_ARG);
  int rc = nl_synchronize(h);
  if (rc) return rc;
  HIPCHK(h, hipSetDevice(h->device));
  for (int k = 0; k < NL_NUM_STAGES; k++) ms[k] = 0;
  hipStream_t s = h->own_stream;
  HIPCHK(h, hipStreamSynchronize(h->last_stream));
  BuildArgs a = h->args;
  a.n = h->n;
  h->upd_valid = false, h->last_update = false;
  h->built = false;
  h->t_valid = false;
  const BuildPlan p = plan_for(h, a, PART_ALL, h->plan.rerun);
  for (int r = 0; r < reps; r++) {
    rc = dispatch_build(h, a, p, s, h->ev);
    if (rc) return rc;
    HIPCHK(h, hipStreamSynchronize(s));
    for (int k = 0; k < NL_STAGE_TOTAL; k++) {
      float t = 0;
      HIPCHK(h, hipEventElapsedTime(&t, h->ev[k], h->ev[k + 1]));
      ms[k] += t;
    }
    float t = 0;
    HIPCHK(h, hipEventElapsedTime(&t, h->ev[0], h->ev[NL_STAGE_TOTAL]));
    ms[NL_STAGE_TOTAL] += t;
  }
  for (int k = 0; k < NL_NUM_STAGES; k++) ms[k] /= reps;
  rc = enqueue_result_copy(h, s);
  if (rc) return rc;
  h->last_stream = s;
  h->pending = true;
  return finish(h, false);
}

int nl_profile_stages(nl_handle_t h, const void* q_dev, int32_t q_stride, int32_t n, int32_t reps,
                      double ms[NL_NUM_STAGES]) {
  if (!h || !ms || reps <= 0) return fail(h, NL_ERR_ARG);
  HIPCHK(h, hipSetDevice(h->device));
  HIPCHK(h, hipDeviceSynchronize());
  int rc = nl_make_list(h, q_dev, q_stride, n, nullptr, 1);
  if (rc) return rc;
  return nl_profile_last_build(h, reps, ms);
}


int nl_buf_alloc(void** dev, void** host, size_t bytes) {
  if (!dev && !host) return NL_ERR_ARG;
  if (dev) *dev = nullptr;
  if (host) *host = nullptr;
  if (dev && hipMalloc(dev, bytes ? bytes : 16) != hipSuccess) return NL_ERR_NOMEM;
  if (host && hipHostMalloc(host, bytes ? bytes : 16, hipHostMallocDefault) != hipSuccess) {
    if (dev) {
      (void)hipFree(*dev);
      *dev = nullptr;
    }
    return NL_ERR_NOMEM;
  }
  return NL_OK;
}
int nl_buf_free(void* dev, void* host) {
  int rc = NL_OK;
  if (dev && hipFree(dev) != hipSuccess) rc = NL_ERR_HIP;
  if (host && hipHostFree(host) != hipSuccess) rc = NL_ERR_HIP;
  return rc;
}
int nl_buf_h2d(void* dev, const void* host, size_t bytes) {
  return hipMemcpy(dev, host, bytes, hipMemcpyHostToDevice) == hipSuccess ? NL_OK : NL_ERR_HIP;
}
int nl_buf_d2h(void* host, const void* dev, size_t bytes) {
  return hipMemcpy(host, dev, bytes, hipMemcpyDeviceToHost) == hipSuccess ? NL_OK : NL_ERR_HIP;
}
int nl_buf_fill32(void* dev, uint32_t pattern, size_t count) {
  if (hipMemsetD32(reinterpret_cast<hipDeviceptr_t>(dev), (int)pattern, count) != hipSuccess) return NL_ERR_HIP;
  return hipDeviceSynchronize() == hipSuccess ? NL_OK : NL_ERR_HIP;
}
int nl_buf_fill64(void* dev, uint64_t pattern, size_t count) {
  const uint32_t lo = (uint32_t)pattern, hi = (uint32_t)(pattern >> 32);
  if (lo == hi) return nl_buf_fill32(dev, lo, count * 2);
  uint64_t* tmp = static_cast<uint64_t*>(malloc(sizeof(uint64_t) * (count ? count : 1)));
  if (!tmp) return NL_ERR_NOMEM;
  for (size_t i = 0; i < count; i++) tmp[i] = pattern;
  const hipError_t e = hipMemcpy(dev, tmp, sizeof(uint64_t) * count, hipMemcpyHostToDevice);
  free(tmp);
  return e == hipSuccess ? NL_OK : NL_ERR_HIP;
}
int nl_device_synchronize(void) { return hipDeviceSynchronize() == hipSuccess ? NL_OK : NL_ERR_HIP; }

}

#include "nl_transpose.inc"
#include "nl_skin.inc"
#include "nl_consumer.inc"
#include "nl_dist.inc"
#include "nl_exclude.inc"
#include "nl_types.inc"
#include "nl_images.inc"
#include "nl_virial.inc"
#include "nl_table.inc"
#include "nl_eam.inc"
#include "nl_sw.inc"
#include "nl_histogram.inc"
```

### md_neighbor_list_amd/csrc/nl_kernels.hpp

```cpp
#pragma once

#include <hip/hip_runtime.h>
#include <stdint.h>

#include <type_traits>

namespace nl {

constexpr int WAVE = 64;

enum : uint32_t { ST_OUT_OF_BOX = 1u, ST_CAPACITY = 2u, ST_DOMAIN = 4u, ST_INDEX_OVERFLOW = 8u, ST_ROW_OVERFLOW = 16u, ST_ID_RANGE = 32u };

template <typename T> struct Pos;
template <> struct alignas(16) Pos<float> {
  float x, y, z;
  int32_t gid;
};
template <> struct alignas(32) Pos<double> {
  double x, y, z;
  int32_t gid;
  int32_t row;
};

struct Box {
// ... 659 lines not shown
  const int32_t r = bx < ph.cells_n0 ? ph.cells_row0 + bx : ph.cells_row1 + (bx - ph.cells_n0);
  const int32_t beg = row_start[r], end = row_start[r + 1];
  const Pos<T>* __restrict__ src = cap_row ? tmp + ((int64_t)r * cap_row - beg) : tmp;
  const int32_t* __restrict__ src_row = cap_row ? tmp_row + ((int64_t)r * cap_row - beg) : tmp_row;
  for (int32_t c = tid; c < nb; c += 256) cnt[c] = 0;
  if (tid == 0) carry_s = 0;
  __syncthreads();
  auto xcell1 = [&](T x) {
    const T tx = mul_rn(x, g.ims[0]);
    int32_t v = (int32_t)tx;
    if ((g.pbc & 1) && tx < (T)0 && (T)v != tx) v -= 1;
    if (v < 0) v += mx;
    if (v >= mx) v -= mx;
    return v;
  };
  auto quarter = [&](T q, T ims) {
    const T t = mul_rn(q, ims);
    const T f = sub_rn(t, (T)(int32_t)t);
    return (f >= (T)0.25 ? 1 : 0) + (f >= (T)0.5 ? 1 : 0) + (f >= (T)0.75 ? 1 : 0);
  };
  const bool tilt = !FINE && IDC == 0 && !IDROW && g.tilt;
  auto bin_of = [&](const Pos<T>& p) {
    const int32_t c = tilt ? p.gid : xcell1(p.x);
    if constexpr (FINE) return quarter(p.z, g.ims[2]) * mx + c;
    else if constexpr (IDC > 0) return c * IDC + min((int32_t)((uint32_t)p.gid >> id_shift), IDC - 1);
    else return c;
  };
  constexpr int BC_KEEP = 6;
  const bool keep = end - beg <= BC_KEEP * 256 && end > beg && !(g.dbg & 512);
  Pos<T> pk[BC_KEEP];
  int32_t rk[BC_KEEP];
  if (keep) {
#pragma unroll
    for (int u = 0; u < BC_KEEP; u++) {
      const int32_t k = min(beg + tid + u * 256, end - 1);
      pk[u] = src[k];
      if constexpr (!IDROW) rk[u] = src_row[k];
    }
#pragma unroll
    for (int u = 0; u < BC_KEEP; u++) {
      keep_in_flight(pk[u].x), keep_in_flight(pk[u].y), keep_in_flight(pk[u].z), keep_in_flight(pk[u].gid);
      if constexpr (!IDROW) keep_in_flight(rk[u]);
      if constexpr (sizeof(T) == 8) keep_in_flight(pk[u].row);
    }
#pragma unroll
    for (int u = 0; u < BC_KEEP; u++)
      if (beg + tid + u * 256 < end) atomicAdd(&cnt[bin_of(pk[u])], 1);
  } else {
    for (int32_t k = beg + tid; k < end; k += 256) atomicAdd(&cnt[bin_of(src[k])], 1);
  }
  __syncthreads();
  for (int32_t base = 0; base < nb; base += 256) {
    const int32_t c = base + tid;
    const int32_t v = c < nb ? cnt[c] : 0;
    const int32_t inc = wave_incl_scan(v, lane);
    if (lane == 63) wsum[w] = inc;
    __syncthreads();
    int32_t woff = 0;
    for (int k = 0; k < w; k++) woff += wsum[k];
    const int32_t carry = carry_s;
    const int32_t excl = carry + woff + inc - v;
    if (c < nb) {
      cnt[c] = excl;
      if constexpr (FINE) {
        cell_start[((size_t)r * mx + (c % mx)) * 4 + c / mx] = beg + excl;
      } else if constexpr (IDC > 0) {
        cls_start[(size_t)r * nb + c] = beg + excl;
        if (c % IDC == 0) cell_start[(size_t)r * mx + c / IDC] = beg + excl;
      } else {
        cell_start[(size_t)r * nb + c] = beg + excl;
      }
    }
    __syncthreads();
    if (tid == 255) carry_s = carry + woff + inc;
    __syncthreads();
  }
  if (r == nrows - 1 && tid == 0) {
    if constexpr (IDC > 0) cls_start[(size_t)nrows * nb] = end, cell_start[(size_t)nrows * mx] = end;
    else cell_start[(size_t)nrows * nb] = end;
  }
  auto place = [&](Pos<T> p, int32_t row_of) {
    const int32_t dst = beg + atomicAdd(&cnt[bin_of(p)], 1);
    if (tilt) {
      p.gid = row_of;
    } else if (g.pbc & 1) {
      const T tx = mul_rn(p.x, g.ims[0]);
      int32_t v = (int32_t)tx;
      if (tx < (T)0 && (T)v != tx) v -= 1;
      if (v < 0) p.x = add_rn(p.x, g.L[0]);
      if (v >= mx) p.x = add_rn(p.x, -g.L[0]);
    }
    sorted[dst] = p;
    sorted_row[dst] = row_of;
    if constexpr (!IDROW) sorted_gid[dst] = p.gid;
  };
  if (keep) {
#pragma unroll
    for (int u = 0; u < BC_KEEP; u++)
      if (beg + tid + u * 256 < end) place(pk[u], IDROW ? pk[u].gid : rk[u]);
  } else {
    for (int32_t k = beg + tid; k < end; k += 256) {
      const Pos<T> p = src[k];
      place(p, IDROW ? p.gid : src_row[k]);
    }
  }
}

enum { MODE_COUNT = 0, MODE_FILL = 1, MODE_COUNT_MASKS = 2 };

struct FastDiv {
  uint32_t d, m, s;
};
__device__ __forceinline__ uint32_t fastdiv(uint32_t n, const FastDiv& f) {
  if (f.d == 1) return n;
  const uint32_t t = __umulhi(n, f.m);
  return (t + ((n - t) >> 1)) >> (f.s - 1);
}

template <typename T> struct SweepArgs {
  const Pos<T>* __restrict__ sorted;
  const int32_t* __restrict__ sorted_row;
  const int32_t* __restrict__ sorted_gid;
  const int32_t* __restrict__ cell_start;
  const int32_t* __restrict__ cls_start;
  int32_t mx, my, mzl, slab;
  FastDiv div_mx, div_my;
  T rc2;
  int32_t* __restrict__ count;
  int32_t* __restrict__ progress;
  const void* __restrict__ key_pointer;
  int32_t wide;
  int32_t n_rows;
  int32_t* __restrict__ list;
  const int64_t* __restrict__ total;
  int64_t capacity;
  uint32_t* __restrict__ status;
  T L[3];
  int32_t pbc;
  T ms[3];
  int32_t z_origin;
  int32_t isplit;
  int32_t mask_nb;
  int32_t* __restrict__ full27_list;
  int32_t* __restrict__ full27_count;
  int32_t* __restrict__ fill_list_count;
  uint32_t* __restrict__ masks;
  uint8_t* __restrict__ masks_hi;
  unsigned long long* dbg_buf;
  int32_t dbg;
  const uint32_t* gate = nullptr;
  T k[3];
  const double* lat;
  uint64_t* cull_bits = nullptr;
};

template <typename T>
__device__ __forceinline__ void face_shift(const SweepArgs<T>& a, int32_t wr, T& sx, T& sy, T& sz) {
  T s[3];
  lattice_shift(a.lat, wr, s);
  sx = s[0], sy = s[1], sz = s[2];
}

__device__ __forceinline__ void recheck_image(const SweepArgs<double>& a, int32_t wr, Pos<double>& pe) {
  const double* p = a.lat + 3 * wr;
  pe.x = add_rn(pe.x, p[0]);
  __builtin_amdgcn_sched_barrier(0);
  pe.y = add_rn(pe.y, p[1]);
  __builtin_amdgcn_sched_barrier(0);
  pe.z = add_rn(pe.z, p[2]);
}

template <typename T> struct SweepCfg;
constexpr int MASK_LO_BYTES = 2 * WAVE, MASK_HI_BYTES = WAVE, MASK_ROW_BYTES = MASK_LO_BYTES + MASK_HI_BYTES;
__device__ __forceinline__ bool hi_plane_used(int32_t mask_nb, int32_t ntiles) { return mask_nb > 1 || ntiles > 16; }
template <bool NT = false>
__device__ __forceinline__ void mask_store(uint32_t* masks, uint8_t* masks_hi, size_t row, int lane, uint32_t bits, bool hi) {
  uint16_t* const lo_p = reinterpret_cast<uint16_t*>(reinterpret_cast<char*>(masks) + row * MASK_LO_BYTES) + lane;
  uint8_t* const hi_p = masks_hi + row * MASK_HI_BYTES + lane;
  if constexpr (NT) {
    __builtin_nontemporal_store((uint16_t)bits, lo_p);
    if (hi) __builtin_nontemporal_store((uint8_t)(bits >> 16), hi_p);
  } else {
    *lo_p = (uint16_t)bits;
    if (hi) *hi_p = (uint8_t)(bits >> 16);
  }
}
template <bool NT, typename P> __device__ __forceinline__ P mask_ld(const P* p) {
  if constexpr (NT) return __builtin_nontemporal_load(p);
  else return *p;
}
__device__ __forceinline__ uint32_t mask_load(const uint32_t* masks, const uint8_t* masks_hi, size_t row, int lane) {
  return (uint32_t)reinterpret_cast<const uint16_t*>(reinterpret_cast<const char*>(masks) + row * MASK_LO_BYTES)[lane] |
         (uint32_t)(masks_hi + row * MASK_HI_BYTES)[lane] << 16;
}
template <> struct SweepCfg<float> { static constexpr int CAP = 1280; };
template <> struct SweepCfg<double> { static constexpr int CAP = 1280; };

constexpr int SWEEP_WAVES = 4;
constexpr int SWEEP_G = 5;
constexpr int NSEG = 18;

struct alignas(16) PosS {
  float x, y, z;
  int32_t gid;
};
struct ScreenCtx {
  float lo, hi;
  float lo_in, hi_out;
  const int32_t* sidx;
  const uint8_t* swrap;
};
template <typename T, bool SCREEN> struct TileOf { typedef Pos<T> type; };
template <typename T> struct TileOf<T, true> { typedef PosS type; };

#ifndef NL_STAMP
#define NL_STAMP 0
#endif
#ifndef NL_STAMP_FILL
#define NL_STAMP_FILL 0
#endif
#ifndef NL_DIAG
#define NL_DIAG 0
#endif
constexpr int NL_PRIO = 3;
template <int GC>
__device__ __forceinline__ void r2_group_f32(float xj, float yj, float zj, const float* xi, const float* yi, const float* zi, float* r2) {
#pragma unroll
  for (int k = 0; k < GC; k++) {
    const float dx = sub_rn(xj, xi[k]), dy = sub_rn(yj, yi[k]), dz = sub_rn(zj, zi[k]);
    r2[k] = add_rn(add_rn(mul_rn(dx, dx), mul_rn(dy, dy)), mul_rn(dz, dz));
  }
}

template <typename T, int MODE, int GC, bool FULL = false, bool NOSELF = false, bool SCREEN = false, bool PBC = false>
__device__ __forceinline__ int32_t search_group(const SweepArgs<T>& a, const typename TileOf<T, SCREEN>::type* tile, int32_t nj,
                                                int32_t ntiles, int lane, const Pos<T>& pi_l, int64_t base_l,
                                                int32_t slot0 = 0, bool store_masks = false, int32_t self0 = 0, int32_t batch = 0,
                                                const ScreenCtx* sc = nullptr, float uxi_l = 0.f, float uyi_l = 0.f, float uzi_l = 0.f,
                                                uint32_t* words_out = nullptr) {
  static_assert(!NOSELF || (FULL && MODE == MODE_COUNT_MASKS), "NOSELF is a form of the full-list COUNT_MASKS search");
  static_assert(SweepCfg<T>::CAP / WAVE <= 24, "one bit per j-tile in the 24-bit word a lane keeps (mask_store)");
  static_assert(!SCREEN || sizeof(T) == 8, "the screened search is the fp64 search");
  typedef typename TileOf<T, SCREEN>::type TileT;
  typedef typename std::conditional<SCREEN, float, T>::type R;
  R xi[GC], yi[GC], zi[GC];
  int32_t gi[GC];
  uint32_t cur[GC];
  int32_t* rowp[GC];
  uint32_t bits[GC];
  constexpr bool VBITS_F32 = MODE == MODE_COUNT_MASKS && !SCREEN && sizeof(T) == 4 && (!FULL || NOSELF);
  constexpr bool VBITS_SCREEN = MODE == MODE_COUNT_MASKS && SCREEN && (!FULL || NOSELF);
  constexpr bool VBITS = VBITS_F32 || VBITS_SCREEN;
  uint32_t gi1[GC];
#pragma unroll
  for (int k = 0; k < GC; k++) bits[k] = 0;
#pragma unroll
  for (int k = 0; k < GC; k++) {
    if constexpr (SCREEN) {
      xi[k] = __builtin_bit_cast(float, __builtin_amdgcn_readlane(__builtin_bit_cast(int32_t, uxi_l), k));
      yi[k] = __builtin_bit_cast(float, __builtin_amdgcn_readlane(__builtin_bit_cast(int32_t, uyi_l), k));
      zi[k] = __builtin_bit_cast(float, __builtin_amdgcn_readlane(__builtin_bit_cast(int32_t, uzi_l), k));
    } else if constexpr (sizeof(T) == 4) {
      xi[k] = __builtin_bit_cast(float, __builtin_amdgcn_readlane(__builtin_bit_cast(int32_t, pi_l.x), k));
      yi[k] = __builtin_bit_cast(float, __builtin_amdgcn_readlane(__builtin_bit_cast(int32_t, pi_l.y), k));
      zi[k] = __builtin_bit_cast(float, __builtin_amdgcn_readlane(__builtin_bit_cast(int32_t, pi_l.z), k));
    } else {
      xi[k] = __shfl(pi_l.x, k, WAVE);
      yi[k] = __shfl(pi_l.y, k, WAVE);
      zi[k] = __shfl(pi_l.z, k, WAVE);
    }
    gi[k] = __builtin_amdgcn_readlane(pi_l.gid, k);
    cur[k] = 0u;
    gi1[k] = (uint32_t)gi[k] + 1u;
    if (MODE == MODE_FILL) {
      const uint32_t lo = (uint32_t)__builtin_amdgcn_readlane((int32_t)(uint32_t)base_l, k);
      const uint32_t hi = (uint32_t)__builtin_amdgcn_readlane((int32_t)(uint32_t)((uint64_t)base_l >> 32), k);
      rowp[k] = a.list + (int64_t)(((uint64_t)hi << 32) | lo);
    }
  }

  auto test_tile = [&](const TileT& pj, int32_t tix) {
    if constexpr (VBITS_SCREEN) {
      constexpr int HALF = (GC + 1) / 2;
      uint32_t uacc = 0;
#pragma unroll
      for (int k = 0; k < GC; k++) {
        if (k == HALF) __builtin_amdgcn_sched_barrier(0);
        const float dx = pj.x - xi[k], dy = pj.y - yi[k], dz = pj.z - zi[k];
        const float r2 = __builtin_fmaf(dz, dz, __builtin_fmaf(dy, dy, dx * dx));
        const uint32_t t_in = __builtin_bit_cast(uint32_t, sc->lo_in - r2), t_out = __builtin_bit_cast(uint32_t, r2 - sc->hi_out);
        uint32_t w = t_in;
        if (!NOSELF) w |= (uint32_t)pj.gid - gi1[k];
        bits[k] = __builtin_amdgcn_alignbit(bits[k], w, 31);
        uacc |= t_in & t_out;
      }
      if (__builtin_amdgcn_ballot_w64((int32_t)uacc < 0) != 0) {
        const int32_t at = tix * WAVE + lane;
        Pos<double> pe;
        pe.x = 0, pe.y = 0, pe.z = 0;
        if ((int32_t)uacc < 0) {
          pe = a.sorted[sc->sidx[at]];
          if (PBC) recheck_image(a, sc->swrap[at], pe);
        }
#pragma unroll
        for (int k = 0; k < GC; k++) {
          const float dx = pj.x - xi[k], dy = pj.y - yi[k], dz = pj.z - zi[k];
// ... 389 lines not shown
    int64_t pre_base = 0;
    auto fetch_group = [&](int32_t g) {
      const int32_t idx = ibeg + min(group_begin(g) + lane, ni - 1);
      pre_p = a.sorted[idx];
      pre_row = a.sorted_row[idx];
      if (MODE == MODE_FILL)
        pre_base = a.wide ? static_cast<const int64_t*>(a.key_pointer)[pre_row] : (int64_t)static_cast<const int32_t*>(a.key_pointer)[pre_row];
      pre_prog = batch ? a.progress[pre_row] : 0;
    };
    const bool ahead = !(a.dbg & 1024);
    if (wave < ngroups && ahead) fetch_group(wave);
    for (int32_t g = wave; g < ngroups; g += NW) {
      const int32_t i0 = group_begin(g);
      const int32_t gcount = gbase + (g < grem ? 1 : 0);
      if (gcount <= 0) break;
      if (!ahead) fetch_group(g);
      Pos<T> pi_l = pre_p;
      const int32_t row_l = pre_row, before = pre_prog;
      int64_t base_l = pre_base + before;
      if (lane >= gcount) pi_l.x = 0, pi_l.y = 0, pi_l.z = 0, pi_l.gid = 0;
      if (ahead && g + NW < ngroups && group_begin(g + NW) < ni) fetch_group(g + NW);
      const int32_t slot0 = ibeg + i0;
      float uxi = 0.f, uyi = 0.f, uzi = 0.f;
      ScreenCtx sc;
      sc.lo = sc.hi = 0.f, sc.sidx = sidx, sc.swrap = swrap;
      if constexpr (SCREEN) {
        float ri = 0.f;
        if (lane < gcount) {
          uxi = (float)(pi_l.x - ox), uyi = (float)(pi_l.y - oy), uzi = (float)(pi_l.z - oz);
          ri = fabsf(uxi) + fabsf(uyi) + fabsf(uzi);
        }
#pragma unroll
        for (int d = 32; d > 0; d >>= 1) ri = fmaxf(ri, __shfl_xor(ri, d, WAVE));
        const float rc2f = (float)a.rc2;
        const float band = 9.5367432e-7f * (ri + rj) * (ri + rj) + 2.3841858e-7f * rc2f;
        sc.lo = rc2f - band, sc.hi = rc2f + band;
        sc.lo_in = nextafterf(sc.lo, -1.0f), sc.hi_out = nextafterf(sc.hi, 3.0e38f);
      }
      const bool keep = nbatch <= a.mask_nb && CAP == SweepCfg<T>::CAP;
      int32_t mine;
      if constexpr (CAN_NOSELF) {
        if (nbatch == 1) {
          switch (gcount) {
            case 1: mine = search_group<T, MODE, 1, FULL, true, SCREEN, PBC>(a, tile, nj, ntiles, lane, pi_l, base_l, slot0, keep, own + i0, 0, &sc, uxi, uyi, uzi); break;
            case 2: mine = search_group<T, MODE, 2, FULL, true, SCREEN, PBC>(a, tile, nj, ntiles, lane, pi_l, base_l, slot0, keep, own + i0, 0, &sc, uxi, uyi, uzi); break;
            case 3: mine = search_group<T, MODE, 3, FULL, true, SCREEN, PBC>(a, tile, nj, ntiles, lane, pi_l, base_l, slot0, keep, own + i0, 0, &sc, uxi, uyi, uzi); break;
            case 4: mine = search_group<T, MODE, 4, FULL, true, SCREEN, PBC>(a, tile, nj, ntiles, lane, pi_l, base_l, slot0, keep, own + i0, 0, &sc, uxi, uyi, uzi); break;
            default: mine = search_group<T, MODE, 5, FULL, true, SCREEN, PBC>(a, tile, nj, ntiles, lane, pi_l, base_l, slot0, keep, own + i0, 0, &sc, uxi, uyi, uzi); break;
          }
          if (lane < gcount) a.count[row_l] = mine;
          continue;
        }
      }
#if NL_STAMP
      stamp(3);
#endif
      switch (gcount) {
        case 1: mine = search_group<T, MODE, 1, FULL, false, SCREEN, PBC>(a, tile, nj, ntiles, lane, pi_l, base_l, slot0, keep, 0, batch, &sc, uxi, uyi, uzi); break;
        case 2: mine = search_group<T, MODE, 2, FULL, false, SCREEN, PBC>(a, tile, nj, ntiles, lane, pi_l, base_l, slot0, keep, 0, batch, &sc, uxi, uyi, uzi); break;
        case 3: mine = search_group<T, MODE, 3, FULL, false, SCREEN, PBC>(a, tile, nj, ntiles, lane, pi_l, base_l, slot0, keep, 0, batch, &sc, uxi, uyi, uzi); break;
        case 4: mine = search_group<T, MODE, 4, FULL, false, SCREEN, PBC>(a, tile, nj, ntiles, lane, pi_l, base_l, slot0, keep, 0, batch, &sc, uxi, uyi, uzi); break;
        default: mine = search_group<T, MODE, 5, FULL, false, SCREEN, PBC>(a, tile, nj, ntiles, lane, pi_l, base_l, slot0, keep, 0, batch, &sc, uxi, uyi, uzi); break;
      }
#if NL_STAMP
      stamp(4);
      n_tests += (uint64_t)(gcount * ntiles);
#endif
      if (lane < gcount) {
        if (nbatch > 1) {
          mine += before;
          a.progress[row_l] = mine;
        }
        if (MODE != MODE_FILL && batch == nbatch - 1) a.count[row_l] = mine;
      }
#if NL_STAMP
      stamp(5);
#endif
    }
  }
#if NL_STAMP
  if (MODE == MODE_COUNT_MASKS && lane == 0) {
    unsigned long long* const slot = a.dbg_buf + 64 + (blockIdx.x & 1023) * 16;
    for (int ph = 1; ph < 6; ph++) atomicAdd(slot + ph, (unsigned long long)t_acc[ph]);
    atomicAdd(slot + 8, (unsigned long long)n_tests);
    atomicAdd(slot + 9, 1ull);
  }
#endif
}

template <typename T, int MODE> constexpr int sweep_cap() { return SweepCfg<T>::CAP; }

template <typename T, int MODE, bool FULL = false, bool PBC = false>
__device__ __forceinline__ void sweep_cell(const SweepArgs<T>& a) {
  if (gate_closed(a.gate)) return;
  constexpr int CAP = sweep_cap<T, MODE>();
  constexpr bool SCREEN = sizeof(T) == 8;
  __shared__ __attribute__((aligned(32))) char tile_bytes[SCREEN ? screen_lds_bytes(CAP) : CAP * (int)sizeof(Pos<T>)];
  Pos<T>* const tile = reinterpret_cast<Pos<T>*>(tile_bytes);
  if (MODE == MODE_FILL) {
    if (a.total[0] > a.capacity) {
      if (blockIdx.x == 0 && threadIdx.x == 0) atomicOr(a.status, ST_CAPACITY);
      return;
    }
  }
  const int tid = threadIdx.x, lane = tid & 63, wave = __builtin_amdgcn_readfirstlane(tid >> 6);
  CellCtx c;
  if (MODE == MODE_COUNT_MASKS) __builtin_amdgcn_s_setprio(NL_PRIO);
#if NL_STAMP
  const uint64_t t_entry = __builtin_amdgcn_s_memtime();
#endif
  if (MODE == MODE_COUNT_MASKS || a.isplit <= 1) {
    if (!cell_setup(a, lane, c)) return;
  } else {
    const int32_t wp = xcd_cell_index(), w = wp / a.isplit, part = wp - w * a.isplit;
    const int32_t wy = (int32_t)fastdiv((uint32_t)w, a.div_mx), cx = w - wy * a.mx;
    const int32_t wz = (int32_t)fastdiv((uint32_t)wy, a.div_my), cy = wy - wz * a.my, cz = wz + (a.slab ? 1 : 0);
    if (!cell_setup_at(a, lane, cx, cy, cz, c)) return;
    const int32_t lo = (int32_t)((int64_t)c.ni * part / a.isplit), hi = (int32_t)((int64_t)c.ni * (part + 1) / a.isplit);
    c.ibeg += lo, c.ni = hi - lo;
    if (c.ni <= 0) return;
  }
#if NL_STAMP
  if (MODE == MODE_COUNT_MASKS && lane == 0) atomicAdd(a.dbg_buf + 64 + (blockIdx.x & 1023) * 16, (unsigned long long)(__builtin_amdgcn_s_memtime() - t_entry));
#endif
  cell_search<T, MODE, CAP, SWEEP_WAVES, FULL, PBC, SCREEN>(a, c, tile, tid, lane, wave);
}

template <typename T, int MODE, bool FULL = false, bool PBC = false>
__global__ void __launch_bounds__(SWEEP_WAVES* WAVE) k_sweep(SweepArgs<T> a) {
  sweep_cell<T, MODE, FULL, PBC>(a);
}
template <bool FULL = false, bool PBC = false>
__global__ void __launch_bounds__(SWEEP_WAVES* WAVE) __attribute__((amdgpu_num_sgpr(80)))
k_sweep_count_f32(SweepArgs<float> a) {
  sweep_cell<float, MODE_COUNT, FULL, PBC>(a);
}
template <bool FULL = false, bool PBC = false>
__global__ void __launch_bounds__(SWEEP_WAVES* WAVE) __attribute__((amdgpu_num_sgpr(80)))
k_sweep_count_masks_f32(SweepArgs<float> a) {
  sweep_cell<float, MODE_COUNT_MASKS, FULL, PBC>(a);
}

__device__ __forceinline__ int32_t scan64_dpp(int32_t v) {
  v += __builtin_amdgcn_update_dpp(0, v, 0x111, 0xf, 0xf, false);
  v += __builtin_amdgcn_update_dpp(0, v, 0x112, 0xf, 0xf, false);
  v += __builtin_amdgcn_update_dpp(0, v, 0x114, 0xf, 0xf, false);
  v += __builtin_amdgcn_update_dpp(0, v, 0x118, 0xf, 0xf, false);
  v += __builtin_amdgcn_update_dpp(0, v, 0x142, 0xa, 0xf, false);
  v += __builtin_amdgcn_update_dpp(0, v, 0x143, 0xc, 0xf, false);
  return v;
}

constexpr int CLS_OWN = 13;
template <int IDC> struct ClsCtx {
  static constexpr int NWIN = 27 * IDC, NT = (NWIN + WAVE - 1) / WAVE;
  int32_t ibeg, ni, total_j;
  int32_t cx, cy, cz;
  int32_t src[NT], len[NT], off[NT];
  __device__ __forceinline__ int32_t get(const int32_t (&v)[NT], int32_t w) const {
    if constexpr (NT == 1) return __builtin_amdgcn_readlane(v[0], w);
    else return w < WAVE ? __builtin_amdgcn_readlane(v[0], w) : __builtin_amdgcn_readlane(v[1], w - WAVE);
  }
};

template <int IDC>
__device__ __forceinline__ bool cls_setup_at(const SweepArgs<float>& a, int lane, int32_t cx, int32_t cy, int32_t cz, ClsCtx<IDC>& c) {
  typedef ClsCtx<IDC> X;
  const int32_t cell = cx + (cy + cz * a.my) * a.mx;
  const uint32_t st_word = *a.status;
  c.ibeg = a.cell_start[cell];
  c.ni = a.cell_start[cell + 1] - c.ibeg;
  c.cx = cx, c.cy = cy, c.cz = cz;
#pragma unroll
  for (int j = 0; j < X::NT; j++) {
    const int32_t w = j * WAVE + lane;
    int32_t src = 0, len = 0;
    if (w < X::NWIN) {
      const int32_t k = w / 27, s = w - 27 * k, r9 = s / 3;
      int32_t x = cx + (s - 3 * r9) - 1, y = cy + r9 % 3 - 1, z = cz + r9 / 3 - 1;
      x += x < 0 ? a.mx : x >= a.mx ? -a.mx : 0;
      y += y < 0 ? a.my : y >= a.my ? -a.my : 0;
      z += z < 0 ? a.mzl : z >= a.mzl ? -a.mzl : 0;
      const int32_t e = (x + (y + z * a.my) * a.mx) * IDC + k;
      src = a.cls_start[e];
      len = a.cls_start[e + 1] - src;
    }
    c.src[j] = src, c.len[j] = len;
  }
  if (c.ni <= 0 || (st_word & ST_DOMAIN)) return false;
  int32_t carry = 0;
#pragma unroll
  for (int j = 0; j < X::NT; j++) {
    const int32_t incl = scan64_dpp(c.len[j]);
    c.off[j] = carry + incl - c.len[j];
    carry += __builtin_amdgcn_readlane(incl, 63);
  }
  c.total_j = carry;
  return true;
}
template <int IDC> __device__ __forceinline__ bool cls_setup(const SweepArgs<float>& a, int lane, ClsCtx<IDC>& c) {
  const int32_t w = xcd_cell_index();
  const int32_t wy = (int32_t)fastdiv((uint32_t)w, a.div_mx), cx = w - wy * a.mx;
  const int32_t cz = (int32_t)fastdiv((uint32_t)wy, a.div_my), cy = wy - cz * a.my;
  return cls_setup_at(a, lane, cx, cy, cz, c);
}

template <int IDC, int NW, typename E>
__device__ __forceinline__ void cls_stage(const E* __restrict__ from, const ClsCtx<IDC>& c, E* dst, int lane, int wave) {
#pragma unroll 1
  for (int32_t pc = wave; pc < 9 * IDC; pc += NW) {
    const int32_t w = 3 * pc;
    const int32_t s0 = c.get(c.src, w), l0 = c.get(c.len, w), s1 = c.get(c.src, w + 1), l1 = c.get(c.len, w + 1);
    const int32_t s2 = c.get(c.src, w + 2), l2 = c.get(c.len, w + 2), off = c.get(c.off, w);
    const int32_t len = l0 + l1 + l2;
#pragma unroll 1
    for (int32_t kb = 0; kb < len; kb += WAVE) {
      const int32_t i = kb + lane;
      if (i < len) {
        const int32_t at = i < l0 ? s0 + i : i < l0 + l1 ? s1 + (i - l0) : s2 + (i - l0 - l1);
        const __attribute__((address_space(1))) void* const gp = (const __attribute__((address_space(1))) void*)(from + at);
        __attribute__((address_space(3))) void* const lp = (__attribute__((address_space(3))) void*)(dst + off + kb);
        if constexpr (sizeof(E) == 16) __builtin_amdgcn_global_load_lds(gp, lp, 16, 0, 0);
        else __builtin_amdgcn_global_load_lds(gp, lp, 4, 0, 0);
      }
    }
  }
}

constexpr int CULL_WORDS = SweepCfg<float>::CAP / WAVE;
constexpr float CULL_DELTA = 1.0f / (float)(1 << 20);

__device__ __forceinline__ float min_raw(float a, float b) {
  float r;
  asm("v_min_f32 %0, %1, %2" : "=v"(r) : "v"(a), "v"(b));
  return r;
}
__device__ __forceinline__ void wave_min6(float (&v)[6]) {
#define NL_MIN6_STEP(ctrl) \
  "v_min_f32_dpp %0, %0, %0 " ctrl "\n\tv_min_f32_dpp %1, %1, %1 " ctrl "\n\tv_min_f32_dpp %2, %2, %2 " ctrl "\n\t" \
  "v_min_f32_dpp %3, %3, %3 " ctrl "\n\tv_min_f32_dpp %4, %4, %4 " ctrl "\n\tv_min_f32_dpp %5, %5, %5 " ctrl "\n\t"
  asm("s_nop 1\n\t" NL_MIN6_STEP("row_shr:1 row_mask:0xf bank_mask:0xf") NL_MIN6_STEP("row_shr:2 row_mask:0xf bank_mask:0xf")
      NL_MIN6_STEP("row_shr:4 row_mask:0xf bank_mask:0xf") NL_MIN6_STEP("row_shr:8 row_mask:0xf bank_mask:0xf")
      NL_MIN6_STEP("row_bcast:15 row_mask:0xa bank_mask:0xf") NL_MIN6_STEP("row_bcast:31 row_mask:0xc bank_mask:0xf") "s_nop 1"
      : "+v"(v[0]), "+v"(v[1]), "+v"(v[2]), "+v"(v[3]), "+v"(v[4]), "+v"(v[5]));
#undef NL_MIN6_STEP
#pragma unroll
  for (int k = 0; k < 6; k++) v[k] = __builtin_bit_cast(float, __builtin_amdgcn_readlane(__builtin_bit_cast(int32_t, v[k]), 63));
}

struct CullMap {
  uint32_t lo, hi;
  int32_t excl;
  int32_t kept;
};
__device__ __forceinline__ CullMap cull_map(uint64_t word) {
  CullMap m;
  m.lo = (uint32_t)word, m.hi = (uint32_t)(word >> 32);
  const int32_t cnt = __popc(m.lo) + __popc(m.hi);
  const int32_t incl = scan64_dpp(cnt);
  m.excl = incl - cnt;
  m.kept = __builtin_amdgcn_readlane(incl, 63);
  return m;
}
__device__ __forceinline__ int32_t cull_rank(const CullMap& m, int32_t s) {
  const int32_t at = (s >> 6) << 2, b = s & 63;
  const uint32_t lo = (uint32_t)__builtin_amdgcn_ds_bpermute(at, (int32_t)m.lo), hi = (uint32_t)__builtin_amdgcn_ds_bpermute(at, (int32_t)m.hi);
  const int32_t ex = __builtin_amdgcn_ds_bpermute(at, m.excl);
  const uint32_t below_lo = b >= 32 ? 0xFFFFFFFFu : (1u << (b & 31)) - 1u, below_hi = b > 32 ? (1u << (b & 31)) - 1u : 0u;
  return ex + __popc(lo & below_lo) + __popc(hi & below_hi);
}
__device__ __forceinline__ bool cull_slot(const CullMap& m, int32_t t, int32_t& dst) {
  const uint32_t lo = (uint32_t)__builtin_amdgcn_readlane((int32_t)m.lo, t), hi = (uint32_t)__builtin_amdgcn_readlane((int32_t)m.hi, t);
  dst = __builtin_amdgcn_readlane(m.excl, t) + (int32_t)__builtin_amdgcn_mbcnt_hi(hi, __builtin_amdgcn_mbcnt_lo(lo, 0u));
  return (((uint64_t)hi << 32 | lo) >> (threadIdx.x & 63) & 1u) != 0;
}
template <int IDC> __device__ __forceinline__ void cull_offsets(const CullMap& m, ClsCtx<IDC>& c) {
#pragma unroll
  for (int j = 0; j < ClsCtx<IDC>::NT; j++) c.off[j] = cull_rank(m, c.off[j]);
  c.total_j = m.kept;
}

template <int IDC, int NW, int CAP>
__device__ __forceinline__ void cls_cull(const SweepArgs<float>& a, ClsCtx<IDC>& c, Pos<float>* buf, int32_t cell, int tid, int lane, int wave) {
  constexpr int TW = (CAP / WAVE + NW - 1) / NW;
  static_assert(CAP / WAVE == CULL_WORDS && CAP % WAVE == 0, "a ballot word per tile of the buffer");
  const int32_t nj = c.total_j, ntiles = (nj + WAVE - 1) / WAVE;
  uint64_t* const out = a.cull_bits + (size_t)cell * CULL_WORDS;
  if (ntiles * WAVE > CAP - WAVE) {
    if (wave == 0 && lane < ntiles) out[lane] = lane + 1 < ntiles ? ~0ull : ~0ull >> (ntiles * WAVE - nj);
    return;
  }
  uint64_t* const words = reinterpret_cast<uint64_t*>(buf + CAP) - CULL_WORDS;
  const float inf = __builtin_inff();
  float bx[6] = {inf, inf, inf, inf, inf, inf};
  float chk = 0.f;
  for (int32_t kb = 0; kb < c.ni; kb += WAVE) {
    int32_t i = min(kb + lane, c.ni - 1), slot = 0;
#pragma unroll
    for (int k = IDC - 1; k >= 0; k--) {
      const int32_t own = c.get(c.off, 27 * k + CLS_OWN), first = c.get(c.src, 27 * k + CLS_OWN) - c.ibeg;
      slot = (k == IDC - 1 || i < first + c.get(c.len, 27 * k + CLS_OWN)) ? own + (i - first) : slot;
    }
    const Pos<float> p = buf[slot];
    bx[0] = min_raw(bx[0], p.x), bx[1] = min_raw(bx[1], p.y), bx[2] = min_raw(bx[2], p.z);
    bx[3] = min_raw(bx[3], -p.x), bx[4] = min_raw(bx[4], -p.y), bx[5] = min_raw(bx[5], -p.z);
    chk = chk + ((p.x + p.y) + p.z);
  }
  wave_min6(bx);
  const float lx = bx[0], ly = bx[1], lz = bx[2], hx = -bx[3], hy = -bx[4], hz = -bx[5];
  const float reach = __builtin_amdgcn_ballot_w64(chk != chk) != 0 ? inf : mul_rn(a.rc2, 1.0f + CULL_DELTA);
  Pos<float> p[TW];
#pragma unroll
  for (int u = 0; u < TW; u++) p[u] = buf[min(wave + u * NW, ntiles - 1) * WAVE + lane];
#pragma unroll
  for (int u = 0; u < TW; u++) {
    const int32_t t = wave + u * NW;
    if (t >= ntiles) break;
    const float gx = fmaxf(fmaxf(sub_rn(p[u].x, hx), sub_rn(lx, p[u].x)), 0.f);
    const float gy = fmaxf(fmaxf(sub_rn(p[u].y, hy), sub_rn(ly, p[u].y)), 0.f);
    const float gz = fmaxf(fmaxf(sub_rn(p[u].z, hz), sub_rn(lz, p[u].z)), 0.f);
    float g2 = add_rn(add_rn(mul_rn(gx, gx), mul_rn(gy, gy)), mul_rn(gz, gz));
    g2 = __builtin_fmaf(add_rn(add_rn(p[u].x, p[u].y), p[u].z), 0.f, g2);
    uint64_t kept = __builtin_amdgcn_ballot_w64(!(g2 > reach));
    if (t == ntiles - 1) kept &= ~0ull >> (ntiles * WAVE - nj);
    if (lane == 0) words[t] = kept;
  }
  asm volatile("s_waitcnt lgkmcnt(0)\n\ts_barrier" ::: "memory");
  const CullMap m = cull_map(lane < ntiles ? words[lane] : 0ull);
  if (wave == 0 && lane < ntiles) out[lane] = (uint64_t)m.hi << 32 | m.lo;
#pragma unroll
  for (int u = 0; u < TW; u++) {
    const int32_t t = wave + u * NW;
    if (t >= ntiles) break;
    int32_t dst;
    if (cull_slot(m, t, dst)) buf[dst] = p[u];
  }
  const int32_t pad = m.kept + tid;
  if (pad < ((m.kept + WAVE - 1) & ~(WAVE - 1))) {
    Pos<float> sentinel;
    sentinel.x = 1.0e18f, sentinel.y = 0.f, sentinel.z = 0.f, sentinel.gid = INT32_MIN;
    buf[pad] = sentinel;
  }
  cull_offsets<IDC>(m, c);
  asm volatile("s_waitcnt lgkmcnt(0)\n\ts_barrier" ::: "memory");
}

template <bool FULL> constexpr int EXPAND_RMAX_OF = FULL ? 192 : 160;
constexpr int EXPAND_WAVES = 2;

template <typename T, bool FULL = false, bool PBC = false, typename OFF = int32_t, int RB = 24, int EW = EXPAND_WAVES, int CAP = SweepCfg<T>::CAP,
          int IDC = 0>
__global__ void __launch_bounds__(EW* WAVE, (sizeof(OFF) == 8 ? 4 : sizeof(T) == 4 ? (FULL || RB > 12 ? 7 : 8) : 4)) __attribute__((amdgpu_num_sgpr(80)))
k_fill_masks(SweepArgs<T> a) {
  static_assert(IDC == 0 || (sizeof(T) == 4 && !FULL && !PBC), "id classes: fp32 half list, open box");
  if (gate_closed(a.gate)) return;
  constexpr int EXPAND_RMAX = EXPAND_RMAX_OF<FULL>;
  __shared__ __attribute__((aligned(32))) int32_t lds[CAP + EW * 4 * EXPAND_RMAX];
  int32_t* const gids = lds;
  const int tid = threadIdx.x, lane = tid & 63, wave = __builtin_amdgcn_readfirstlane(tid >> 6);
#if NL_STAMP_FILL
  uint64_t ft_prev = __builtin_amdgcn_s_memtime(), ft_acc[6] = {0, 0, 0, 0, 0, 0};
  auto fstamp = [&](int phase) {
    const uint64_t now = __builtin_amdgcn_s_memtime();
    ft_acc[phase] += now - ft_prev;
    ft_prev = now;
  };
#endif
  const int64_t total = a.total[0];
  uint64_t kept_word = 0;
  if constexpr (IDC > 0) {
    static_assert(EW * 4 * EXPAND_RMAX >= CAP, "the staged ids of a cull build land in the row buffers");
    if (a.cull_bits) kept_word = a.cull_bits[(size_t)xcd_cell_index() * CULL_WORDS + min(lane, CULL_WORDS - 1)];
  }
  typename std::conditional<(IDC > 0), ClsCtx<IDC ? IDC : 2>, CellCtx>::type c;
  bool ok;
  if constexpr (IDC > 0) ok = cls_setup<IDC>(a, lane, c);
  else ok = cell_setup(a, lane, c);
#if NL_STAMP_FILL
  fstamp(0);
#endif
  if (total > a.capacity) {
    if (blockIdx.x == 0 && threadIdx.x == 0) atomicOr(a.status, ST_CAPACITY);
    return;
  }
  if (!ok) return;
  if (c.total_j > CAP) {
    if (tid == 0) a.full27_list[atomicAdd(a.fill_list_count, 1)] = c.cx + (c.cy + c.cz * a.my) * a.mx;
    return;
  }

  const int32_t per_wave = (c.ni + EW - 1) / EW;
  const int32_t r_beg = min(wave * per_wave, c.ni), r_end = min(r_beg + per_wave, c.ni);
  uint32_t w[RB];
  OFF base_l;
  CullMap cm = {0u, 0u, 0, 0};
  bool cull = false;
  const int32_t staged_tiles = (c.total_j + WAVE - 1) / WAVE;
  if constexpr (IDC > 0) {
    cull = a.cull_bits != nullptr;
    if (cull) cm = cull_map(lane < staged_tiles ? kept_word : 0ull);
  }
  const bool hi_plane = hi_plane_used(1, ((cull ? cm.kept : c.total_j) + WAVE - 1) / WAVE);
  auto load_rows = [&](int32_t r0) {
    {
      const int32_t srow = a.sorted_row[c.ibeg + r0 + min(lane, RB - 1)];
      base_l = static_cast<const OFF*>(a.key_pointer)[min((uint32_t)srow, (uint32_t)a.n_rows)];
    }
    const size_t slot0 = (size_t)(c.ibeg + r0);
    const char* const lo0 = reinterpret_cast<const char*>(a.masks) + slot0 * MASK_LO_BYTES;
    if (hi_plane) {
      const uint8_t* const hi0 = a.masks_hi + slot0 * MASK_HI_BYTES;
#pragma unroll
      for (int u = 0; u < RB; u++)
        w[u] = (uint32_t)mask_ld<EW == 2>(reinterpret_cast<const uint16_t*>(lo0 + u * MASK_LO_BYTES) + lane) | (uint32_t)mask_ld<EW == 2>(hi0 + u * MASK_HI_BYTES + lane) << 16;
    } else {
#pragma unroll
      for (int u = 0; u < RB; u++) w[u] = (uint32_t)mask_ld<EW == 2>(reinterpret_cast<const uint16_t*>(lo0 + u * MASK_LO_BYTES) + lane);
    }
  };
  auto base = [&](int u) -> OFF {
    const uint32_t lo = (uint32_t)__builtin_amdgcn_readlane((int32_t)(uint32_t)base_l, u);
    if constexpr (sizeof(OFF) == 4) return (OFF)lo;
    const uint32_t hi = (uint32_t)__builtin_amdgcn_readlane((int32_t)(uint32_t)((uint64_t)base_l >> 32), u);
    return (OFF)((uint64_t)hi << 32 | lo);
  };
  load_rows(r_beg);
  if (a.dbg & 32) return;

  int32_t cls_row[IDC > 0 ? IDC : 1], cls_t0[IDC > 0 ? IDC : 1];
  int32_t* const staged = cull ? lds + CAP : gids;
  (void)staged;
  if constexpr (IDC > 0) {
    cls_stage<IDC, EW>(a.sorted_gid, c, staged, lane, wave);
  } else
#pragma unroll
  for (int s = 0; s < (NSEG + EW - 1) / EW; s++) {
    const int sg = min(wave + s * EW, NSEG - 1);
    const int32_t len = wave + s * EW < NSEG ? __builtin_amdgcn_readlane(c.seg_len, sg) : 0;
    const int32_t src = __builtin_amdgcn_readlane(c.seg_src, sg);
    const int32_t off = __builtin_amdgcn_readlane(c.seg_off, sg);
    for (int32_t kb = 0; kb < len; kb += WAVE) {
      if (kb + lane < len)
        __builtin_amdgcn_global_load_lds((const __attribute__((address_space(1))) void*)(a.sorted_gid + src + kb + lane),
                                         (__attribute__((address_space(3))) void*)(gids + off + kb), 4, 0, 0);
    }
  }
#if NL_STAMP_FILL
  fstamp(1);
#endif
  __syncthreads();
#if NL_STAMP_FILL
  fstamp(2);
#endif
  if constexpr (IDC > 0) {
    if (cull) {
      for (int32_t t = wave; t < staged_tiles; t += EW) {
        int32_t dst;
        const int32_t id = staged[t * WAVE + lane];
        if (cull_slot(cm, t, dst)) gids[dst] = id;
      }
      cull_offsets<IDC>(cm, c);
      __syncthreads();
    }
#pragma unroll
    for (int k = 0; k < IDC; k++) {
      cls_row[k] = c.get(c.src, 27 * k + CLS_OWN) - c.ibeg;
      cls_t0[k] = c.get(c.off, 27 * k) & ~(WAVE - 1);
    }
  }

  const int32_t* const g = gids + lane;
  for (int32_t r0 = r_beg; r0 < r_end; r0 += RB) {
    if (r0 != r_beg) load_rows(r0);
#pragma unroll
    for (int u0 = 0; u0 < RB; u0 += 4) {
      if (r0 + u0 >= r_end) continue;
      uint32_t word[4], ptr[4];
      int32_t nrow[4];
      const int32_t* gq[4];
#pragma unroll
      for (int q = 0; q < 4; q++) {
        if constexpr (IDC > 0) {
          int32_t t0 = cls_t0[0];
#pragma unroll
          for (int k = 1; k < IDC; k++) t0 = r0 + u0 + q >= cls_row[k] ? cls_t0[k] : t0;
          gq[q] = g + t0;
        } else {
          gq[q] = g;
        }
      }
#pragma unroll
      for (int q = 0; q < 4; q++) {
        word[q] = r0 + u0 + q < r_end ? (w[u0 + q] & 0xFFFFFFu) : 0u;
        if (a.dbg & 16) word[q] = 0;
        const int32_t cnt = __popc(word[q]);
        const int32_t incl = scan64_dpp(cnt);
        nrow[q] = __builtin_amdgcn_readlane(incl, 63);
        ptr[q] = (uint32_t)(incl - cnt);
      }
      const int32_t nmax = max(max(nrow[0], nrow[1]), max(nrow[2], nrow[3]));
#if NL_STAMP_FILL
      fstamp(3);
#endif
      __amdgpu_buffer_rsrc_t dst[4];
#pragma unroll
      for (int q = 0; q < 4; q++) dst[q] = __builtin_amdgcn_make_buffer_rsrc(a.list + (ptrdiff_t)base(u0 + q), 0, nrow[q] * 4, 0x00020000);
      typedef __attribute__((address_space(3))) int32_t lds_i32;
      uint32_t src[4];
#pragma unroll
      for (int q = 0; q < 4; q++) src[q] = (uint32_t)(uintptr_t)(lds_i32*)gq[q];
      auto read_next = [&](int32_t (&val)[4], bool (&on)[4]) {
        uint32_t rd[4];
#pragma unroll
        for (int q = 0; q < 4; q++) rd[q] = src[q] + ((uint32_t)__builtin_ctz(word[q]) << 8);
        asm volatile("" : "+v"(rd[0]), "+v"(rd[1]), "+v"(rd[2]), "+v"(rd[3]));
#pragma unroll
        for (int q = 0; q < 4; q++) {
          on[q] = word[q] != 0;
          val[q] = *(const lds_i32*)(uintptr_t)(on[q] ? rd[q] : src[q]);
        }
        asm volatile("" : "+v"(val[0]), "+v"(val[1]), "+v"(val[2]), "+v"(val[3]));
      };
      if (nmax < EXPAND_RMAX) {
        const uint32_t cw = (uint32_t)(uintptr_t)(lds_i32*)(lds + CAP + wave * 4 * EXPAND_RMAX);
        uint32_t dump = cw + 4 * (uint32_t)nrow[0];
        asm volatile("" : "+v"(dump));
        uint32_t at[4];
#pragma unroll
        for (int q = 0; q < 4; q++) at[q] = cw + 4 * (q * EXPAND_RMAX + ptr[q]);
        do {
          int32_t val[4];
          bool on[4];
          read_next(val, on);
#pragma unroll
          for (int q = 0; q < 4; q++) {
            *(lds_i32*)(uintptr_t)(on[q] ? at[q] : dump) = val[q];
            at[q] += 4;
            word[q] &= word[q] - 1;
          }
        } while (__builtin_amdgcn_ballot_w64((word[0] | word[1] | word[2] | word[3]) != 0) != 0);
#if NL_STAMP_FILL
        fstamp(4);
#endif
        __builtin_amdgcn_wave_barrier();
        for (int32_t e0 = 0; e0 < nmax; e0 += WAVE) {
          const int32_t e = e0 + lane;
          const uint32_t rd = cw + 4 * (uint32_t)min(e, EXPAND_RMAX - 1);
          int32_t val[4];
#pragma unroll
          for (int q = 0; q < 4; q++) val[q] = *(const lds_i32*)(uintptr_t)(rd + 4 * q * EXPAND_RMAX);
          asm volatile("" ::"v"(val[0]), "v"(val[1]), "v"(val[2]), "v"(val[3]) : "memory");
#pragma unroll
          for (int q = 0; q < 4; q++) __builtin_amdgcn_raw_buffer_store_b32((uint32_t)val[q], dst[q], e * 4, 0, 0);
// ... 179 lines not shown
```

### md_neighbor_list_amd/csrc/nl_lean.hpp

```cpp
#pragma once

namespace nl {

constexpr int PIPE_G = 7;

template <int NW = SWEEP_WAVES>
__device__ __forceinline__ void pipe_stage(const SweepArgs<float>& a, const CellCtx& c, Pos<float>* dst, int tid, int lane, int wave) {
#pragma unroll 1
  for (int sg = wave; sg < NSEG; sg += NW) {
    const int32_t len = __builtin_amdgcn_readlane(c.seg_len, sg);
    const int32_t src = __builtin_amdgcn_readlane(c.seg_src, sg);
    const int32_t off = __builtin_amdgcn_readlane(c.seg_off, sg);
#pragma unroll 1
    for (int32_t kb = 0; kb < len; kb += WAVE) {
      if (kb + lane < len)
        __builtin_amdgcn_global_load_lds((const __attribute__((address_space(1))) void*)(a.sorted + src + kb + lane),
                                         (__attribute__((address_space(3))) void*)(dst + off + kb), 16, 0, 0);
    }
  }
  const int32_t pad = c.total_j + tid;
  if (pad < ((c.total_j + WAVE - 1) & ~(WAVE - 1))) {
    Pos<float> sentinel;
    sentinel.x = 1.0e18f, sentinel.y = 0.f, sentinel.z = 0.f, sentinel.gid = INT32_MIN;
    dst[pad] = sentinel;
  }
}

struct PipePending {
  uint32_t w[PIPE_G];
  int32_t mine, row_l, slot0, gcount;
};

template <bool NT>
__device__ __forceinline__ void pipe_flush(const SweepArgs<float>& a, PipePending& p, int lane, bool hi) {
  if (p.gcount <= 0) return;
  if (lane < p.gcount) a.count[p.row_l] = p.mine;
#pragma unroll
  for (int k = 0; k < PIPE_G; k++)
    if (k < p.gcount) mask_store<NT>(a.masks, a.masks_hi, (size_t)(p.slot0 + k) * a.mask_nb, lane, p.w[k], hi);
  p.gcount = 0;
}

template <bool FULL, int GC>
__device__ __forceinline__ void pipe_group(const SweepArgs<float>& a, const Pos<float>* tile, int32_t nj, int32_t ntiles, int lane,
                                           const Pos<float>& pi_l, int32_t slot0, int32_t self0, PipePending& p) {
  uint32_t words[GC];
  p.mine = search_group<float, MODE_COUNT_MASKS, GC, FULL, FULL, false, false>(a, tile, nj, ntiles, lane, pi_l, 0, slot0, true, self0,
                                                                             0, nullptr, 0.f, 0.f, 0.f, words);
#pragma unroll
  for (int k = 0; k < GC; k++) p.w[k] = words[k];
}

template <bool FULL, int NW = SWEEP_WAVES, bool IDROW = false>
__device__ __forceinline__ void pipe_search(const SweepArgs<float>& a, const CellCtx& c, const Pos<float>* tile, int lane, int wave,
                                            PipePending& p) {
  constexpr int G = PIPE_G;
  const int32_t ibeg = c.ibeg, ni = c.ni, nj = c.total_j;
  const int32_t ntiles = (nj + WAVE - 1) / WAVE;
  const int32_t rounds = (ni + NW * G - 1) / (NW * G);
  const int32_t ngroups = rounds * NW;
  const int32_t gbase = ni / ngroups, grem = ni - gbase * ngroups;
  const int32_t s4 = __builtin_amdgcn_readlane(c.seg_src, 4), l4 = __builtin_amdgcn_readlane(c.seg_len, 4);
  const bool in4 = ibeg >= s4 && ibeg < s4 + l4;
  const int32_t own = in4 ? __builtin_amdgcn_readlane(c.seg_off, 4) + ibeg - s4
                          : __builtin_amdgcn_readlane(c.seg_off, 13) + ibeg - __builtin_amdgcn_readlane(c.seg_src, 13);
  for (int32_t g = wave; g < ngroups; g += NW) {
    const int32_t i0 = g * gbase + min(g, grem);
    const int32_t gcount = gbase + (g < grem ? 1 : 0);
    if (gcount <= 0) break;
    pipe_flush<NW == SWEEP_WAVES>(a, p, lane, hi_plane_used(a.mask_nb, ntiles));
    const int32_t k = min(lane, gcount - 1);
    Pos<float> pi_l = tile[own + i0 + k];
    int32_t row_l;
    if constexpr (IDROW) row_l = pi_l.gid;
    else row_l = a.sorted_row[ibeg + i0 + k];
    if (lane >= gcount) pi_l.x = 0, pi_l.y = 0, pi_l.z = 0, pi_l.gid = 0;
    const int32_t slot0 = ibeg + i0, self0 = own + i0;
    switch (gcount) {
      case 1: pipe_group<FULL, 1>(a, tile, nj, ntiles, lane, pi_l, slot0, self0, p); break;
      case 2: pipe_group<FULL, 2>(a, tile, nj, ntiles, lane, pi_l, slot0, self0, p); break;
      case 3: pipe_group<FULL, 3>(a, tile, nj, ntiles, lane, pi_l, slot0, self0, p); break;
      case 4: pipe_group<FULL, 4>(a, tile, nj, ntiles, lane, pi_l, slot0, self0, p); break;
      case 5: pipe_group<FULL, 5>(a, tile, nj, ntiles, lane, pi_l, slot0, self0, p); break;
      case 6: pipe_group<FULL, 6>(a, tile, nj, ntiles, lane, pi_l, slot0, self0, p); break;
      default: pipe_group<FULL, 7>(a, tile, nj, ntiles, lane, pi_l, slot0, self0, p); break;
    }
    p.row_l = row_l, p.slot0 = slot0, p.gcount = gcount;
  }
}

constexpr int LEAN_SMALL_CAP = SweepCfg<float>::CAP / 2;
template <bool FULL, int NW = SWEEP_WAVES, int CAP = SweepCfg<float>::CAP, bool IDROW = false>
__global__ void __launch_bounds__(NW* WAVE, 8) __attribute__((amdgpu_num_sgpr(80))) k_sweep_lean_f32(SweepArgs<float> a) {
  if (gate_closed(a.gate)) return;
  __shared__ __attribute__((aligned(32))) Pos<float> buf[CAP];
  const int tid = threadIdx.x, lane = tid & 63, wave = __builtin_amdgcn_readfirstlane(tid >> 6);
  __builtin_amdgcn_s_setprio(NL_PRIO);
  CellCtx c;
  if (!cell_setup(a, lane, c)) return;
  if (c.total_j > CAP) {
    if (tid == 0) a.full27_list[atomicAdd(a.full27_count, 1)] = c.cx + (c.cy + c.cz * a.my) * a.mx;
    return;
  }
  pipe_stage<NW>(a, c, buf, tid, lane, wave);
  asm volatile("s_waitcnt vmcnt(0) lgkmcnt(0)\n\ts_barrier" ::: "memory");
  PipePending pend;
  pend.gcount = 0, pend.mine = 0, pend.row_l = 0, pend.slot0 = 0;
  pipe_search<FULL, NW, IDROW>(a, c, buf, lane, wave, pend);
  pipe_flush<NW == SWEEP_WAVES>(a, pend, lane, hi_plane_used(a.mask_nb, (c.total_j + WAVE - 1) / WAVE));
}

template <int GC>
__device__ __forceinline__ int32_t class_group(const SweepArgs<float>& a, const Pos<float>* tile, int32_t t0, int32_t tsplit,
                                               int32_t ntiles, int lane, const Pos<float>& pi_l, uint32_t* words) {
  float xi[GC], yi[GC], zi[GC];
  uint32_t gi1[GC], bits[GC];
#pragma unroll
  for (int k = 0; k < GC; k++) {
    xi[k] = __builtin_bit_cast(float, __builtin_amdgcn_readlane(__builtin_bit_cast(int32_t, pi_l.x), k));
    yi[k] = __builtin_bit_cast(float, __builtin_amdgcn_readlane(__builtin_bit_cast(int32_t, pi_l.y), k));
    zi[k] = __builtin_bit_cast(float, __builtin_amdgcn_readlane(__builtin_bit_cast(int32_t, pi_l.z), k));
    gi1[k] = (uint32_t)__builtin_amdgcn_readlane(pi_l.gid, k) + 1u;
    bits[k] = 0;
  }
  auto test_tile = [&](const Pos<float>& pj, auto id) {
    constexpr int HALF = (GC + 1) / 2;
#pragma unroll
    for (int k = 0; k < GC; k++) {
      if (k == HALF) __builtin_amdgcn_sched_barrier(0);
      const float dx = sub_rn(pj.x, xi[k]), dy = sub_rn(pj.y, yi[k]), dz = sub_rn(pj.z, zi[k]);
      const float r2 = add_rn(add_rn(mul_rn(dx, dx), mul_rn(dy, dy)), mul_rn(dz, dz));
      uint32_t w = __builtin_bit_cast(uint32_t, sub_rn(a.rc2, r2));
      if constexpr (decltype(id)::value) w |= (uint32_t)pj.gid - gi1[k];
      bits[k] = __builtin_amdgcn_alignbit(bits[k], w, 31);
    }
  };
  const std::true_type with_id;
  const std::false_type no_id;
  const int32_t last = (ntiles - 1) * WAVE + lane;
  Pos<float> pa = tile[t0 * WAVE + lane], pb;
  int32_t t = t0;
  __builtin_amdgcn_s_setprio(0);
  for (; t + 1 < tsplit; t += 2) {
    pb = tile[(t + 1) * WAVE + lane];
    test_tile(pa, with_id);
    pa = tile[min((t + 2) * WAVE + lane, last)];
    test_tile(pb, with_id);
  }
  if (t < tsplit) {
    test_tile(pa, with_id);
    t++;
    pa = tile[min(t * WAVE + lane, last)];
  }
  for (; t + 1 < ntiles; t += 2) {
    pb = tile[(t + 1) * WAVE + lane];
    test_tile(pa, no_id);
    pa = tile[min((t + 2) * WAVE + lane, last)];
    test_tile(pb, no_id);
  }
  if (t < ntiles) test_tile(pa, no_id);
  __builtin_amdgcn_s_setprio(NL_PRIO);
  const int32_t nt = ntiles - t0;
  uint32_t tot[GC];
#pragma unroll
  for (int k = 0; k < GC; k++) words[k] = __brev(~bits[k]) >> (32 - nt);
#pragma unroll
  for (int k = 0; k < GC; k += 2) {
    const uint32_t two = wave_sum_dpp((uint32_t)__popc(words[k]) | (k + 1 < GC ? (uint32_t)__popc(words[k + 1]) << 16 : 0u));
    tot[k] = two & 0xffffu;
    if (k + 1 < GC) tot[k + 1] = two >> 16;
  }
  uint32_t mine = 0;
#pragma unroll
  for (int k = 0; k < GC; k++) mine = lane == k ? tot[k] : mine;
  return (int32_t)mine;
}

template <int GC>
__device__ __forceinline__ void class_pipe_group(const SweepArgs<float>& a, const Pos<float>* tile, int32_t t0, int32_t tsplit,
                                                 int32_t ntiles, int lane, const Pos<float>& pi_l, PipePending& p) {
  uint32_t words[GC];
  p.mine = class_group<GC>(a, tile, t0, tsplit, ntiles, lane, pi_l, words);
#pragma unroll
  for (int k = 0; k < GC; k++) p.w[k] = words[k];
}

template <int IDC, int NW>
__device__ __forceinline__ void class_search(const SweepArgs<float>& a, const ClsCtx<IDC>& c, const Pos<float>* tile, int lane, int wave,
                                             PipePending& p) {
  constexpr int G = PIPE_G, NP = IDC / 2, WP = NW / NP;
  static_assert(NW % NP == 0, "waves a pair of classes");
  const int32_t ntiles = (c.total_j + WAVE - 1) / WAVE;
  const bool hi = hi_plane_used(1, ntiles);
  const int pair = wave / WP, wj = wave - pair * WP;
#pragma unroll
  for (int h = 0; h < 2; h++) {
    const int32_t k = h == 0 ? pair : IDC - 1 - pair;
    const int32_t ni = c.get(c.len, 27 * k + CLS_OWN);
    const int32_t own = c.get(c.off, 27 * k + CLS_OWN), slot_b = c.get(c.src, 27 * k + CLS_OWN);
    const int32_t t0 = c.get(c.off, 27 * k) / WAVE;
    const int32_t tsplit = k + 1 < IDC ? (c.get(c.off, 27 * (k + 1)) + WAVE - 1) / WAVE : ntiles;
    const int32_t ngroups = (ni + WP * G - 1) / (WP * G) * WP;
    if (ni <= 0) continue;
    const int32_t gbase = ni / ngroups, grem = ni - gbase * ngroups;
    for (int32_t g = wj; g < ngroups; g += WP) {
      const int32_t i0 = g * gbase + min(g, grem);
      const int32_t gcount = gbase + (g < grem ? 1 : 0);
      if (gcount <= 0) break;
      pipe_flush<NW == SWEEP_WAVES>(a, p, lane, hi);
      const int32_t kk = min(lane, gcount - 1);
      Pos<float> pi_l = tile[own + i0 + kk];
      const int32_t row_l = pi_l.gid;
      if (lane >= gcount) pi_l.x = 0, pi_l.y = 0, pi_l.z = 0, pi_l.gid = 0;
      switch (gcount) {
        case 1: class_pipe_group<1>(a, tile, t0, tsplit, ntiles, lane, pi_l, p); break;
        case 2: class_pipe_group<2>(a, tile, t0, tsplit, ntiles, lane, pi_l, p); break;
        case 3: class_pipe_group<3>(a, tile, t0, tsplit, ntiles, lane, pi_l, p); break;
        case 4: class_pipe_group<4>(a, tile, t0, tsplit, ntiles, lane, pi_l, p); break;
        case 5: class_pipe_group<5>(a, tile, t0, tsplit, ntiles, lane, pi_l, p); break;
        case 6: class_pipe_group<6>(a, tile, t0, tsplit, ntiles, lane, pi_l, p); break;
        default: class_pipe_group<7>(a, tile, t0, tsplit, ntiles, lane, pi_l, p); break;
      }
      p.row_l = row_l, p.slot0 = slot_b + i0, p.gcount = gcount;
    }
  }
}

template <int IDC, int NW = SWEEP_WAVES, int CAP = SweepCfg<float>::CAP>
__global__ void __launch_bounds__(NW* WAVE, 8) __attribute__((amdgpu_num_sgpr(80))) k_sweep_class_f32(SweepArgs<float> a) {
  if (gate_closed(a.gate)) return;
  __shared__ __attribute__((aligned(32))) Pos<float> buf[CAP];
  const int tid = threadIdx.x, lane = tid & 63, wave = __builtin_amdgcn_readfirstlane(tid >> 6);
  __builtin_amdgcn_s_setprio(NL_PRIO);
  ClsCtx<IDC> c;
  if (!cls_setup<IDC>(a, lane, c)) return;
  if (c.total_j > CAP) {
    if (tid == 0) a.full27_list[atomicAdd(a.full27_count, 1)] = c.cx + (c.cy + c.cz * a.my) * a.mx;
    return;
  }
  cls_stage<IDC, NW>(a.sorted, c, buf, lane, wave);
  const int32_t pad = c.total_j + tid;
  if (pad < ((c.total_j + WAVE - 1) & ~(WAVE - 1))) {
    Pos<float> sentinel;
    sentinel.x = 1.0e18f, sentinel.y = 0.f, sentinel.z = 0.f, sentinel.gid = INT32_MIN;
    buf[pad] = sentinel;
  }
  asm volatile("s_waitcnt vmcnt(0) lgkmcnt(0)\n\ts_barrier" ::: "memory");
  if (a.cull_bits) cls_cull<IDC, NW, CAP>(a, c, buf, c.cx + (c.cy + c.cz * a.my) * a.mx, tid, lane, wave);
  PipePending pend;
  pend.gcount = 0, pend.mine = 0, pend.row_l = 0, pend.slot0 = 0;
  class_search<IDC, NW>(a, c, buf, lane, wave, pend);
  pipe_flush<NW == SWEEP_WAVES>(a, pend, lane, hi_plane_used(1, (c.total_j + WAVE - 1) / WAVE));
}

template <bool FULL>
__global__ void __launch_bounds__(SWEEP_WAVES* WAVE) __attribute__((amdgpu_num_sgpr(80))) k_sweep_list_f32(SweepArgs<float> a) {
  if (gate_closed(a.gate)) return;
  constexpr int CAP = SweepCfg<float>::CAP;
  __shared__ __attribute__((aligned(32))) Pos<float> tile[CAP];
  const int tid = threadIdx.x, lane = tid & 63, wave = __builtin_amdgcn_readfirstlane(tid >> 6);
  const int32_t count = *a.full27_count;
  for (int32_t idx = blockIdx.x; idx < count; idx += gridDim.x) {
    if (idx != (int32_t)blockIdx.x) __syncthreads();
    const int32_t cell = a.full27_list[idx];
    const int32_t row = cell / a.mx, cx = cell - row * a.mx, cz = row / a.my, cy = row - cz * a.my;
    CellCtx c;
    if (!cell_setup_at(a, lane, cx, cy, cz, c)) continue;
    cell_search<float, MODE_COUNT_MASKS, CAP, SWEEP_WAVES, FULL, false, false>(a, c, tile, tid, lane, wave);
  }
}

}
```

### md_neighbor_list_amd/neighlist.py

```python
from __future__ import annotations

import ctypes as C

import torch

from . import _lib
from ._lib import NLError, check


class _DevView:

    def __init__(self, ptr, shape, typestr, owner):
        self.__cuda_array_interface__ = {
            "shape": tuple(int(s) for s in shape),
            "typestr": typestr,
            "data": (int(ptr), False),
            "version": 2,
            "strides": None,
        }
        self._owner = owner


def _as_tensor(ptr, shape, typestr, owner, device):
    n = 1
# ... 408 lines not shown
        nt, nk, lo, hi = C.c_int32(), C.c_int32(), C.c_double(), C.c_double()
        code = self._lib.nl_get_pair_table(self._h, C.byref(nt), C.byref(nk), C.byref(lo), C.byref(hi))
        if code == _lib.NL_ERR_STATE:
            return None
        check(code, "nl_get_pair_table")
        return {"ntypes": nt.value, "nknots": nk.value, "r_min": lo.value, "r_max": hi.value}

    def table_forces(self, q, wait=True, out=None):
        return self._consume("nl_table_forces", q, (), wait, out, totals=False)

    def table_virial(self, q, wait=True, out=None):
        return self._consume("nl_table_virial", q, (), wait, out, totals=True)

    def set_eam(self, f, G, r_min, r_max, E, P, rho_max):
        import numpy as np

        f, G, E, P = (np.ascontiguousarray(np.atleast_2d(np.asarray(m, dtype=np.float64))) for m in (f, G, E, P))
        if f.shape != G.shape or E.shape != P.shape or f.ndim != 2 or E.ndim != 2 or f.shape[0] != E.shape[0]:
            raise TypeError("f, G must both be (ntypes, nknots_d) and E, P both (ntypes, nknots_e)")
        ptr = lambda m: m.ctypes.data_as(C.POINTER(C.c_double))
        check(self._lib.nl_set_eam(self._h, int(f.shape[0]), int(f.shape[1]), float(r_min), float(r_max), ptr(f), ptr(G), int(E.shape[1]),
                                   float(rho_max), ptr(E), ptr(P)), "nl_set_eam")

    def clear_eam(self):
        check(self._lib.nl_set_eam(self._h, 0, 0, 0.0, 0.0, None, None, 0, 0.0, None, None), "nl_set_eam")

    def eam(self):
        nt, nd, ne, l1, l2 = (C.c_int32() for _ in range(5))
        lo, hi, rm = C.c_double(), C.c_double(), C.c_double()
        code = self._lib.nl_get_eam(self._h, C.byref(nt), C.byref(nd), C.byref(lo), C.byref(hi), C.byref(ne), C.byref(rm), C.byref(l1), C.byref(l2))
        if code == _lib.NL_ERR_STATE:
            return None
        check(code, "nl_get_eam")
        return {"ntypes": nt.value, "nknots_d": nd.value, "r_min": lo.value, "r_max": hi.value, "nknots_e": ne.value, "rho_max": rm.value,
                "lds_density": bool(l1.value), "lds_forces": bool(l2.value)}

    def eam_forces(self, q, wait=True, out=None):
        return self._consume("nl_eam_forces", q, (), wait, out, totals=False)

    def eam_virial(self, q, wait=True, out=None):
        return self._consume("nl_eam_virial", q, (), wait, out, totals=True)

    def eam_density(self):
        rho, fp, n = C.c_void_p(), C.c_void_p(), C.c_int32()
        check(self._lib.nl_eam_get_density(self._h, C.byref(rho), C.byref(fp), C.byref(n)), "nl_eam_get_density")
        ts = "<f4" if self.dtype == torch.float32 else "<f8"
        return tuple(_as_tensor(p.value, (n.value,), ts, self, self.device).clone() for p in (rho, fp))

    def set_sw(self, g, G, r_min, r_max, lam, cos0):
        import numpy as np

        g, G = (np.ascontiguousarray(np.atleast_2d(np.asarray(m, dtype=np.float64))) for m in (g, G))
        lam, cos0 = (np.ascontiguousarray(np.asarray(m, dtype=np.float64)).reshape(-1) for m in (lam, cos0))
        nt = int(round(g.shape[0] ** 0.5))
        if g.shape != G.shape or g.ndim != 2 or nt * nt != g.shape[0] or lam.shape != (nt ** 3,) or cos0.shape != (nt ** 3,):
            raise TypeError("g, G must both be (ntypes^2, nknots) and lam, cos0 both hold ntypes^3 values")
        ptr = lambda m: m.ctypes.data_as(C.POINTER(C.c_double))
        check(self._lib.nl_set_sw(self._h, nt, int(g.shape[1]), float(r_min), float(r_max), ptr(g), ptr(G), ptr(lam), ptr(cos0)), "nl_set_sw")

    def clear_sw(self):
        check(self._lib.nl_set_sw(self._h, 0, 0, 0.0, 0.0, None, None, None, None), "nl_set_sw")

    def sw(self):
        nt, nk, lds = (C.c_int32() for _ in range(3))
        lo, hi = C.c_double(), C.c_double()
        code = self._lib.nl_get_sw(self._h, C.byref(nt), C.byref(nk), C.byref(lo), C.byref(hi), C.byref(lds))
        if code == _lib.NL_ERR_STATE:
            return None
        check(code, "nl_get_sw")
        return {"ntypes": nt.value, "nknots": nk.value, "r_min": lo.value, "r_max": hi.value, "lds": bool(lds.value)}

    def sw_forces(self, q, wait=True, out=None):
        return self._consume("nl_sw_forces", q, (), wait, out, totals=False)

    def sw_virial(self, q, wait=True, out=None):
        return self._consume("nl_sw_virial", q, (), wait, out, totals=True)

    def pair_histogram(self, q, r_max, nbins, typed=False, wait=True, out=None):
        n = self._check_q(q, None)
        if n != self._n:
            raise ValueError("q must hold the particles the list was built from")
        nbins = int(nbins)
        if typed:
            nt = self._get_types()[2]
            shape = (nt * (nt + 1) // 2, nbins)
        else:
            shape = (nbins,)
        o = torch.zeros(shape, dtype=torch.int64, device=self.device) if out is None else out
        if tuple(o.shape) != shape or o.dtype != torch.int64 or not o.is_contiguous() or o.device != q.device:
            raise TypeError(f"out must be a contiguous int64 tensor of shape {shape} on the list's device")
        stream = torch.cuda.current_stream(self.device).cuda_stream
        name = "nl_pair_histogram" + ("_typed" if typed else "") + ("" if wait else "_enqueue")
        check(getattr(self._lib, name)(self._h, q.data_ptr(), q.shape[1], float(r_max), nbins, o.data_ptr(), stream), name)
        return o

    def rdf(self, hist, r_max, frames=1, types=None):
        import numpy as np

        from . import rdf as _rdf

        if self.periodic_mask() != 7:
            raise ValueError("rdf() needs a box periodic on all three axes")
        if self._n_rows != self._n:
            raise ValueError("rdf() needs the global counts: sum the ranks' histograms of a slab build and call rdf.rdf")
        Lx, Ly, Lz = self.box[:3]
        h = hist.detach().cpu().numpy() if isinstance(hist, torch.Tensor) else np.asarray(hist)
        if types is None:
            if h.ndim != 1:
                raise ValueError("a typed histogram needs types=(a, b)")
            return _rdf.rdf(h, r_max, Lx * Ly * Lz, self._n, frames=frames)
        a, b = (int(t) for t in types)
        nt = self._get_types()[2]
        if h.ndim != 2 or h.shape[0] != _rdf.nslots(nt):
            raise ValueError(f"types=(a, b) picks a row of a typed histogram of {_rdf.nslots(nt)} rows")
        counts = torch.bincount(self.types().to(torch.int64), minlength=nt).cpu()
        return _rdf.rdf(h[_rdf.slot(a, b, nt)], r_max, Lx * Ly * Lz, int(counts[a]), None if a == b else int(counts[b]),
                        frames=frames)

    def cell_order(self):
        ptr, n = C.c_void_p(), C.c_int32()
        check(self._lib.nl_get_cell_order(self._h, C.byref(ptr), C.byref(n)), "nl_get_cell_order")
        return _as_tensor(ptr.value, (n.value,), "<i4", self, self.device)

    def resort(self, *arrays):
        stream = torch.cuda.current_stream(self.device).cuda_stream
        for t in arrays:
            if not isinstance(t, torch.Tensor) or t.device.type != "cuda" or not t.is_contiguous() or t.shape[0] != self._n:
                raise TypeError("resort() takes contiguous device tensors with one leading entry per particle")
            check(self._lib.nl_resort(self._h, t.data_ptr(), t.element_size() * (t.numel() // max(t.shape[0], 1)), stream), "nl_resort")

    def sorted_state(self):
        cs, sp, sr, ncl = C.c_void_p(), C.c_void_p(), C.c_void_p(), C.c_int64()
        check(self._lib.nl_get_sorted(self._h, C.byref(cs), C.byref(sp), C.byref(sr), C.byref(ncl)), "nl_get_sorted")
        entries = ncl.value * (4 if self.build_info()["fine_rows"] else 1) + 1
        return (_as_tensor(cs.value, (entries,), "<i4", self, self.device),
                _as_tensor(sr.value, (self._n,), "<i4", self, self.device))

    def profile_stages(self, q, reps=10):
        n = self._check_q(q, None)
        ms = (C.c_double * _lib.NL_NUM_STAGES)()
        check(self._lib.nl_profile_stages(self._h, q.data_ptr(), q.shape[1], n, int(reps), C.byref(ms)),
              "nl_profile_stages")
        self._n = self._n_rows = n
        return dict(zip(_lib.STAGE_NAMES, (float(v) for v in ms)))


    def build_info(self):
        info = (C.c_int32 * 8)()
        check(self._lib.nl_get_build_info(self._h, C.byref(info)), "nl_get_build_info")
        return {"masks": bool(info[0]), "variant": int(info[1]), "lds_batch": int(info[2]), "cus": int(info[3]),
                "offset_bits": int(info[4]), "mask_rows": int(info[5]), "fine_rows": int(info[6]),
                "small_cells": int(info[7]) & 0xFF, "id_classes": int(info[7]) >> 8 & 0xFF,
                "binning": ("two_pass", "bucket", "atomic")[int(info[7]) >> 16 & 3],
                "reach_cull": bool(int(info[7]) >> 18 & 1)}

    def build_stats(self):
        st = (C.c_int64 * 4)()
        check(self._lib.nl_get_build_stats(self._h, C.byref(st)), "nl_get_build_stats")
        return {"row_overflow_reruns": int(st[0]), "list_reruns": int(st[1]), "cap_row": int(st[2]),
                "list_launched": bool(st[3])}

    def profile_last_build(self, reps=10):
        ms = (C.c_double * _lib.NL_NUM_STAGES)()
        check(self._lib.nl_profile_last_build(self._h, int(reps), C.byref(ms)), "nl_profile_last_build")
        return dict(zip(_lib.STAGE_NAMES, (float(v) for v in ms)))


def axes_mask(axes) -> int:
    if isinstance(axes, str):
        if any(c not in "xyz" for c in axes.lower()):
            raise ValueError(f"periodic axes {axes!r}: use letters from 'xyz'")
        return sum(1 << "xyz".index(c) for c in set(axes.lower()))
    if not hasattr(axes, "__len__"):
        return 7 if axes else 0
    axes = tuple(axes)
    if len(axes) != 3:
        raise ValueError(f"periodic axes {axes!r}: a 3-tuple of bools or a string from 'xyz'")
    return sum(1 << d for d in range(3) if axes[d])


def npairs_exceeds_int32(nl) -> bool:
    n = C.c_int64()
    check(nl._lib.nl_number_of_pairs(nl._h, C.byref(n)), "nl_number_of_pairs")
    return (2 if nl.full_list else 1) * int(n.value) > 2147483647


def device_count() -> int:
    c = C.c_int()
    check(_lib.load().nl_device_count(C.byref(c)))
    return int(c.value)
```

Before: 181,900.

## Stage culled count stream through registers and pick a 3-wave class kernel

Adds a register-staged variant of the class count kernel. Each wave gathers its tiles of the 27-cell stream into VGPRs, runs the reach-cull ballots on them, and writes only the kept particles into LDS, instead of DMA-staging the whole stream and compacting it in place. A host-side estimate of the expected kept count then picks a smaller 3-wave, 1024-entry workgroup when it fits, to raise occupancy. Cells whose kept count overflows the capacity fall back to the full-27 list, and the fill kernel gets a matching overflow check. Optional timestamp instrumentation is compiled in only under NL_STAMP.

```diff
diff --git a/include/nl_hip.h b/include/nl_hip.h
--- a/include/nl_hip.h
+++ b/include/nl_hip.h
@@ -196,6 +196,7 @@
 int nl_debug_read(nl_handle_t h, uint64_t* out, int32_t n, int reset);
 int nl_debug_occupancy(int32_t out[8]);
 int nl_get_build_info(nl_handle_t h, int32_t info[8]);
+int nl_count_waves_estimate(int64_t n, const int32_t m[3], const double L[3], double rc, double* kept_mean);
 int nl_get_build_stats(nl_handle_t h, int64_t stats[4]);
 int nl_last_error(nl_handle_t h);
 int nl_last_hip_error(nl_handle_t h);
diff --git a/md_neighbor_list_amd/_lib.py b/md_neighbor_list_amd/_lib.py
--- a/md_neighbor_list_amd/_lib.py
+++ b/md_neighbor_list_amd/_lib.py
@@ -104,6 +104,7 @@
     "nl_debug_read": (C.c_int, [_P, C.c_void_p, _I32, C.c_int]),
     "nl_debug_occupancy": (C.c_int, [C.POINTER(_I32 * 8)]),
     "nl_get_build_info": (C.c_int, [_P, C.POINTER(_I32 * 8)]),
+    "nl_count_waves_estimate": (C.c_int, [_I64, C.POINTER(_I32 * 3), C.POINTER(_D * 3), _D, C.POINTER(_D)]),
     "nl_get_build_stats": (C.c_int, [_P, C.POINTER(_I64 * 4)]),
     "nl_last_error": (C.c_int, [_P]),
     "nl_last_hip_error": (C.c_int, [_P]),
diff --git a/md_neighbor_list_amd/csrc/nl_api.hip b/md_neighbor_list_amd/csrc/nl_api.hip
--- a/md_neighbor_list_amd/csrc/nl_api.hip
+++ b/md_neighbor_list_amd/csrc/nl_api.hip
@@ -81,12 +81,15 @@
   int32_t idc = 0;
   int32_t id_shift = 0;
   bool cull = false;
+  bool count_regstage = false;
+  int32_t count_waves = 0;
   bool id_rows = false;
   Box box = {{0, 0, 0}, 0, 0, 0};
   int32_t tilt = 0;
   bool rerun = false;
   auto tie() const {
-    return std::tie(rerun, binning, cap_row, split, search, rows_v, mask_nb, small, rows12, list, full, wide, filter, images, pbc, idc, id_shift, cull, id_rows,
+    return std::tie(rerun, binning, cap_row, split, search, rows_v, mask_nb, small, rows12, list, full, wide, filter, images, pbc, idc, id_shift, cull, count_regstage, count_waves,
+                    id_rows,
                     box.L[0], box.L[1], box.L[2], box.xy, box.xz, box.yz, tilt);
   }
   bool operator==(const BuildPlan& o) const { return tie() == o.tie(); }
@@ -165,6 +168,8 @@
   int idclass_env = 2;
   DevBuf<uint64_t> cull_bits;
   int cull_env = 1;
+  int regstage_env = 1;
+  int count_waves_env = 0;
   DevBuf<uint64_t> scan_look;
   int32_t scan_blocks = 0;
   DevBuf<int64_t> totals;
@@ -518,6 +523,7 @@
   a.dbg_buf = h->dbg_buf;
   a.gate = h->gate;
   a.cull_bits = h->plan.cull ? h->cull_bits.get() : nullptr;
+  a.kept_cap = !h->plan.count_regstage ? INT32_MAX : (h->plan.count_waves == CLS3_WAVES ? CLS3_CAP : SweepCfg<float>::CAP) - WAVE;
   for (int d = 0; d < 3; d++) a.k[d] = (T)h->shear[d];
   a.lat = h->lat_dev;
   return a;
@@ -583,6 +589,10 @@
           constexpr int CAP = SweepCfg<float>::CAP;
           if (p.small && p.id_rows) hipLaunchKernelGGL((k_sweep_lean_f32<FULL, 2, LEAN_SMALL_CAP, true>), cells, dim3(2 * WAVE), 0, s, a);
           else if (p.small) hipLaunchKernelGGL((k_sweep_lean_f32<FULL, 2, LEAN_SMALL_CAP>), cells, dim3(2 * WAVE), 0, s, a);
+          else if (!FULL && p.idc == 2 && p.count_regstage && p.count_waves == CLS3_WAVES)
+            hipLaunchKernelGGL((k_sweep_class_f32<2, CLS3_WAVES, CLS3_CAP, true>), cells, dim3(CLS3_WAVES * WAVE), 0, s, a);
+          else if (!FULL && p.idc == 2 && p.count_regstage) hipLaunchKernelGGL((k_sweep_class_f32<2, SWEEP_WAVES, CAP, true>), cells, wg, 0, s, a);
+          else if (!FULL && p.idc == 4 && p.count_regstage) hipLaunchKernelGGL((k_sweep_class_f32<4, SWEEP_WAVES, CAP, true>), cells, wg, 0, s, a);
           else if (!FULL && p.idc == 2) hipLaunchKernelGGL((k_sweep_class_f32<2>), cells, wg, 0, s, a);
           else if (!FULL && p.idc == 4) hipLaunchKernelGGL((k_sweep_class_f32<4>), cells, wg, 0, s, a);
           else if (p.id_rows) hipLaunchKernelGGL((k_sweep_lean_f32<FULL, SWEEP_WAVES, CAP, true>), cells, wg, 0, s, a);
@@ -686,6 +696,15 @@
   return (int32_t)cap;
 }
 
+int count_waves_estimate(double n, const int32_t m[3], const double L[3], double rc, double* kept_mean) {
+  const double a = L[0] / m[0], b = L[1] / m[1], c = L[2] / m[2], pi = 3.14159265358979323846;
+  const double v_reach = a * b * c + 2.0 * rc * (a * b + b * c + c * a) + pi * rc * rc * (a + b + c) + 4.0 / 3.0 * pi * rc * rc * rc;
+  const double mean_stream = 27.0 * n / ((double)m[0] * m[1] * m[2]);
+  const double kept = mean_stream * v_reach / (27.0 * a * b * c);
+  if (kept_mean) *kept_mean = kept;
+  return kept + 6.0 * std::sqrt(kept) <= (double)(CLS3_CAP - WAVE) ? CLS3_WAVES : SWEEP_WAVES;
+}
+
 template <typename T> BuildPlan plan_build(nl_handle_t h, const BuildArgs& a, int part, bool rerun) {
   BuildPlan p;
   p.rerun = rerun;
@@ -738,6 +757,12 @@
     p.idc = h->idclass_env;
     while (((uint32_t)(n - 1) >> p.id_shift) >= (uint32_t)p.idc) p.id_shift++;
     p.cull = h->cull_env != 0 && cull_bits_ready(h, ncl);
+    p.count_regstage = p.cull && h->regstage_env != 0;
+    p.count_waves = SWEEP_WAVES;
+    if (p.count_regstage && p.idc == 2) {
+      const int32_t mesh[3] = {h->m[0], h->m[1], a.mzl};
+      p.count_waves = h->count_waves_env ? h->count_waves_env : count_waves_estimate((double)n, mesh, h->L, h->rc, nullptr);
+    }
   }
   return p;
 }
@@ -1191,6 +1216,8 @@
     if (const char* v = getenv("NL_ROWS")) h->rows_env = std::max(-1, std::min(atoi(v), 4));
     if (const char* v = getenv("NL_IDCLASS")) h->idclass_env = atoi(v) >= 4 ? 4 : atoi(v) >= 2 ? 2 : 0;
     if (const char* v = getenv("NL_CULL")) h->cull_env = atoi(v) != 0;
+    if (const char* v = getenv("NL_REGSTAGE")) h->regstage_env = atoi(v) != 0;
+    if (const char* v = getenv("NL_COUNT_WAVES")) h->count_waves_env = atoi(v) == CLS3_WAVES ? CLS3_WAVES : atoi(v) == SWEEP_WAVES ? SWEEP_WAVES : 0;
     if (const char* v = getenv("NL_OFFSET_WIDTH")) h->offset_width = atoi(v) == 64 ? 64 : atoi(v) == 32 ? 32 : 0;
     if (const char* v = getenv("NL_BINNING")) h->bin_two_level = atoi(v) != 1;
     if (const char* v = getenv("NL_BIN_BUCKETS")) h->bucket_env = atoi(v) != 0;
@@ -1692,12 +1719,17 @@
   info[5] = p.mask_nb;
   info[6] = p.search == SEARCH_ROWS ? 1 + p.rows_v : 0;
   const int32_t binning = p.binning == BINNING_TWO_PASS ? 0 : p.binning == BINNING_BUCKET ? 1 : 2;
-  info[7] = (p.small ? 1 : 0) | p.idc << 8 | binning << 16 | (p.cull ? 1 : 0) << 18;
+  info[7] = (p.small ? 1 : 0) | p.idc << 8 | binning << 16 | (p.cull ? 1 : 0) << 18 | p.count_waves << 19 | (p.count_regstage ? 1 : 0) << 22;
   info[0] = p.search != SEARCH_SWEEPS ? 1 : 0;
   info[1] = h->sweep_variant;
   info[2] = h->dtype == NL_F32 ? SweepCfg<float>::CAP : SweepCfg<double>::CAP;
   info[3] = h->num_cus;
   return NL_OK;
+}
+
+int nl_count_waves_estimate(int64_t n, const int32_t m[3], const double L[3], double rc, double* kept_mean) {
+  if (!m || !L || n < 0 || m[0] <= 0 || m[1] <= 0 || m[2] <= 0 || !(L[0] > 0 && L[1] > 0 && L[2] > 0 && rc > 0)) return 0;
+  return count_waves_estimate((double)n, m, L, rc, kept_mean);
 }
 
 int nl_get_build_stats(nl_handle_t h, int64_t stats[4]) {
diff --git a/md_neighbor_list_amd/csrc/nl_kernels.hpp b/md_neighbor_list_amd/csrc/nl_kernels.hpp
--- a/md_neighbor_list_amd/csrc/nl_kernels.hpp
+++ b/md_neighbor_list_amd/csrc/nl_kernels.hpp
@@ -835,6 +835,7 @@
   T k[3];
   const double* lat;
   uint64_t* cull_bits = nullptr;
+  int32_t kept_cap = INT32_MAX;
 };
 
 template <typename T>
@@ -1530,6 +1531,33 @@
 }
 
 constexpr int CLS_OWN = 13;
+
+enum {
+  CLS_PH_TABLE, CLS_PH_ISSUED, CLS_PH_LANDED, CLS_PH_BALLOTS, CLS_PH_BARRIER1, CLS_PH_COMPACT, CLS_PH_BARRIER2, CLS_PH_PROLOGUE,
+  CLS_PH_TILES, CLS_PH_EPILOGUE, CLS_PH_FLUSH, CLS_PHASES
+};
+struct ClsStamp {
+#if NL_STAMP
+  uint64_t prev = __builtin_amdgcn_s_memtime(), tests = 0;
+  uint32_t acc[CLS_PHASES] = {};
+  __device__ __forceinline__ void operator()(int phase) {
+    const uint64_t now = __builtin_amdgcn_s_memtime();
+    acc[phase] += (uint32_t)(now - prev);
+    prev = now;
+  }
+  __device__ __forceinline__ void write(unsigned long long* dbg_buf, int lane) const {
+    if (lane != 0) return;
+    unsigned long long* const slot = dbg_buf + 64 + (blockIdx.x & 1023) * 16;
+    for (int ph = 0; ph < CLS_PHASES; ph++) atomicAdd(slot + (ph < 8 ? ph : ph + 2), (unsigned long long)acc[ph]);
+    atomicAdd(slot + 8, (unsigned long long)tests);
+    atomicAdd(slot + 9, 1ull);
+  }
+#else
+  __device__ __forceinline__ void operator()(int) {}
+  __device__ __forceinline__ void write(unsigned long long*, int) const {}
+#endif
+};
+
 template <int IDC> struct ClsCtx {
   static constexpr int NWIN = 27 * IDC, NT = (NWIN + WAVE - 1) / WAVE;
   int32_t ibeg, ni, total_j;
@@ -1659,7 +1687,8 @@
 }
 
 template <int IDC, int NW, int CAP>
-__device__ __forceinline__ void cls_cull(const SweepArgs<float>& a, ClsCtx<IDC>& c, Pos<float>* buf, int32_t cell, int tid, int lane, int wave) {
+__device__ __forceinline__ void cls_cull(const SweepArgs<float>& a, ClsCtx<IDC>& c, Pos<float>* buf, int32_t cell, int tid, int lane, int wave,
+                                         ClsStamp& st) {
   constexpr int TW = (CAP / WAVE + NW - 1) / NW;
   static_assert(CAP / WAVE == CULL_WORDS && CAP % WAVE == 0, "a ballot word per tile of the buffer");
   const int32_t nj = c.total_j, ntiles = (nj + WAVE - 1) / WAVE;
@@ -1703,7 +1732,9 @@
     if (t == ntiles - 1) kept &= ~0ull >> (ntiles * WAVE - nj);
     if (lane == 0) words[t] = kept;
   }
+  st(CLS_PH_BALLOTS);
   asm volatile("s_waitcnt lgkmcnt(0)\n\ts_barrier" ::: "memory");
+  st(CLS_PH_BARRIER1);
   const CullMap m = cull_map(lane < ntiles ? words[lane] : 0ull);
   if (wave == 0 && lane < ntiles) out[lane] = (uint64_t)m.hi << 32 | m.lo;
 #pragma unroll
@@ -1720,7 +1751,114 @@
     buf[pad] = sentinel;
   }
   cull_offsets<IDC>(m, c);
+  st(CLS_PH_COMPACT);
   asm volatile("s_waitcnt lgkmcnt(0)\n\ts_barrier" ::: "memory");
+  st(CLS_PH_BARRIER2);
+}
+
+template <int IDC> __device__ __forceinline__ int32_t cls_tile_source(const ClsCtx<IDC>& c, int32_t t, int lane) {
+  typedef ClsCtx<IDC> X;
+  const int32_t s0 = t * WAVE, s = s0 + lane;
+  int32_t w = -1;
+#pragma unroll
+  for (int j = 0; j < X::NT; j++) w += __popcll(__builtin_amdgcn_ballot_w64(j * WAVE + lane < X::NWIN && c.off[j] <= s0));
+  int32_t at = -1;
+#pragma unroll 1
+  for (; w < X::NWIN; w++) {
+    const int32_t off = c.get(c.off, w);
+    if (off >= s0 + WAVE) break;
+    const int32_t d = s - off;
+    at = (uint32_t)d < (uint32_t)c.get(c.len, w) ? c.get(c.src, w) + d : at;
+  }
+  return at;
+}
+typedef uint32_t cls_u4 __attribute__((ext_vector_type(4)));
+__device__ __forceinline__ cls_u4 cls_load_tile(const Pos<float>* __restrict__ from, int32_t at, cls_u4 sentinel) {
+  static_assert(sizeof(Pos<float>) == sizeof(cls_u4), "x, y, z and the id");
+  cls_u4 e = sentinel;
+  if (at >= 0) e = *reinterpret_cast<const cls_u4*>(from + at);
+  return e;
+}
+__device__ __forceinline__ Pos<float> cls_pos(cls_u4 v) {
+  const uint32_t x = v.x, y = v.y, z = v.z, w = v.w;
+  Pos<float> p;
+  p.x = __builtin_bit_cast(float, x), p.y = __builtin_bit_cast(float, y), p.z = __builtin_bit_cast(float, z), p.gid = (int32_t)w;
+  return p;
+}
+
+template <int IDC, int NW, int CAP>
+__device__ __forceinline__ bool cls_cull_reg(const SweepArgs<float>& a, ClsCtx<IDC>& c, Pos<float>* buf, int32_t cell, int tid, int lane, int wave,
+                                             ClsStamp& st) {
+  constexpr int TW = (CULL_WORDS + NW - 1) / NW;
+  static_assert(CAP % WAVE == 0 && CAP >= 2 * WAVE && CULL_WORDS <= WAVE, "a tile for the ballots behind the compacted stream");
+  const int32_t nj = c.total_j, ntiles = (nj + WAVE - 1) / WAVE;
+  uint64_t* const out = a.cull_bits + (size_t)cell * CULL_WORDS;
+  uint64_t* const words = reinterpret_cast<uint64_t*>(buf + CAP) - CULL_WORDS;
+  const cls_u4 sentinel = {__builtin_bit_cast(uint32_t, 1.0e18f), 0u, 0u, (uint32_t)INT32_MIN};
+  int32_t at[TW];
+#pragma unroll
+  for (int u = 0; u < TW; u++) at[u] = wave + u * NW < ntiles ? cls_tile_source<IDC>(c, wave + u * NW, lane) : -1;
+  Pos<float> own = a.sorted[c.ibeg + min(lane, c.ni - 1)];
+  cls_u4 p[TW];
+#pragma unroll
+  for (int u = 0; u < TW; u++) p[u] = cls_load_tile(a.sorted, at[u], sentinel);
+  st(CLS_PH_ISSUED);
+  asm volatile("" : "+v"(own.x), "+v"(own.y), "+v"(own.z)::"memory");
+  const float inf = __builtin_inff();
+  float bx[6] = {inf, inf, inf, inf, inf, inf};
+  float chk = 0.f;
+  for (int32_t kb = 0;;) {
+    bx[0] = min_raw(bx[0], own.x), bx[1] = min_raw(bx[1], own.y), bx[2] = min_raw(bx[2], own.z);
+    bx[3] = min_raw(bx[3], -own.x), bx[4] = min_raw(bx[4], -own.y), bx[5] = min_raw(bx[5], -own.z);
+    chk = chk + ((own.x + own.y) + own.z);
+    if ((kb += WAVE) >= c.ni) break;
+    own = a.sorted[c.ibeg + min(kb + lane, c.ni - 1)];
+  }
+  wave_min6(bx);
+  const float lx = bx[0], ly = bx[1], lz = bx[2], hx = -bx[3], hy = -bx[4], hz = -bx[5];
+  const float reach = __builtin_amdgcn_ballot_w64(chk != chk) != 0 ? inf : mul_rn(a.rc2, 1.0f + CULL_DELTA);
+#if NL_STAMP
+#pragma unroll
+  for (int u = 0; u < TW; u++) asm volatile("" : "+v"(p[u]));
+#endif
+  st(CLS_PH_LANDED);
+#pragma unroll
+  for (int u = 0; u < TW; u++) {
+    const int32_t t = wave + u * NW;
+    if (t >= ntiles) break;
+    const Pos<float> pj = cls_pos(p[u]);
+    const float gx = fmaxf(fmaxf(sub_rn(pj.x, hx), sub_rn(lx, pj.x)), 0.f);
+    const float gy = fmaxf(fmaxf(sub_rn(pj.y, hy), sub_rn(ly, pj.y)), 0.f);
+    const float gz = fmaxf(fmaxf(sub_rn(pj.z, hz), sub_rn(lz, pj.z)), 0.f);
+    float g2 = add_rn(add_rn(mul_rn(gx, gx), mul_rn(gy, gy)), mul_rn(gz, gz));
+    g2 = __builtin_fmaf(add_rn(add_rn(pj.x, pj.y), pj.z), 0.f, g2);
+    uint64_t kept = __builtin_amdgcn_ballot_w64(!(g2 > reach));
+    if (t == ntiles - 1) kept &= ~0ull >> (ntiles * WAVE - nj);
+    if (lane == 0) words[t] = kept;
+  }
+  st(CLS_PH_BALLOTS);
+  asm volatile("s_waitcnt lgkmcnt(0)\n\ts_barrier" ::: "memory");
+  st(CLS_PH_BARRIER1);
+  const CullMap m = cull_map(lane < ntiles ? words[lane] : 0ull);
+  if (wave == 0 && lane < ntiles) out[lane] = (uint64_t)m.hi << 32 | m.lo;
+  if (m.kept > CAP - WAVE) {
+    if (tid == 0) a.full27_list[atomicAdd(a.full27_count, 1)] = cell;
+    return false;
+  }
+#pragma unroll
+  for (int u = 0; u < TW; u++) {
+    const int32_t t = wave + u * NW;
+    if (t >= ntiles) break;
+    int32_t dst;
+    if (cull_slot(m, t, dst)) buf[dst] = cls_pos(p[u]);
+  }
+  const int32_t pad = m.kept + tid;
+  if (pad < ((m.kept + WAVE - 1) & ~(WAVE - 1))) buf[pad] = cls_pos(sentinel);
+  cull_offsets<IDC>(m, c);
+  st(CLS_PH_COMPACT);
+  asm volatile("s_waitcnt lgkmcnt(0)\n\ts_barrier" ::: "memory");
+  st(CLS_PH_BARRIER2);
+  return true;
 }
 
 template <bool FULL> constexpr int EXPAND_RMAX_OF = FULL ? 192 : 160;
@@ -1777,6 +1915,10 @@
   if constexpr (IDC > 0) {
     cull = a.cull_bits != nullptr;
     if (cull) cm = cull_map(lane < staged_tiles ? kept_word : 0ull);
+    if (cull && cm.kept > a.kept_cap) {
+      if (tid == 0) a.full27_list[atomicAdd(a.fill_list_count, 1)] = c.cx + (c.cy + c.cz * a.my) * a.mx;
+      return;
+    }
   }
   const bool hi_plane = hi_plane_used(1, ((cull ? cm.kept : c.total_j) + WAVE - 1) / WAVE);
   auto load_rows = [&](int32_t r0) {
diff --git a/md_neighbor_list_amd/csrc/nl_lean.hpp b/md_neighbor_list_amd/csrc/nl_lean.hpp
--- a/md_neighbor_list_amd/csrc/nl_lean.hpp
+++ b/md_neighbor_list_amd/csrc/nl_lean.hpp
@@ -112,7 +112,7 @@
 
 template <int GC>
 __device__ __forceinline__ int32_t class_group(const SweepArgs<float>& a, const Pos<float>* tile, int32_t t0, int32_t tsplit,
-                                               int32_t ntiles, int lane, const Pos<float>& pi_l, uint32_t* words) {
+                                               int32_t ntiles, int lane, const Pos<float>& pi_l, uint32_t* words, ClsStamp& st) {
   float xi[GC], yi[GC], zi[GC];
   uint32_t gi1[GC], bits[GC];
 #pragma unroll
@@ -140,6 +140,7 @@
   const int32_t last = (ntiles - 1) * WAVE + lane;
   Pos<float> pa = tile[t0 * WAVE + lane], pb;
   int32_t t = t0;
+  st(CLS_PH_PROLOGUE);
   __builtin_amdgcn_s_setprio(0);
   for (; t + 1 < tsplit; t += 2) {
     pb = tile[(t + 1) * WAVE + lane];
@@ -161,6 +162,12 @@
   if (t < ntiles) test_tile(pa, no_id);
   __builtin_amdgcn_s_setprio(NL_PRIO);
   const int32_t nt = ntiles - t0;
+#if NL_STAMP
+#pragma unroll
+  for (int k = 0; k < GC; k++) asm volatile("" : "+v"(bits[k]));
+  st.tests += (uint64_t)(GC * nt);
+#endif
+  st(CLS_PH_TILES);
   uint32_t tot[GC];
 #pragma unroll
   for (int k = 0; k < GC; k++) words[k] = __brev(~bits[k]) >> (32 - nt);
@@ -178,16 +185,20 @@
 
 template <int GC>
 __device__ __forceinline__ void class_pipe_group(const SweepArgs<float>& a, const Pos<float>* tile, int32_t t0, int32_t tsplit,
-                                                 int32_t ntiles, int lane, const Pos<float>& pi_l, PipePending& p) {
+                                                 int32_t ntiles, int lane, const Pos<float>& pi_l, PipePending& p, ClsStamp& st) {
   uint32_t words[GC];
-  p.mine = class_group<GC>(a, tile, t0, tsplit, ntiles, lane, pi_l, words);
+  p.mine = class_group<GC>(a, tile, t0, tsplit, ntiles, lane, pi_l, words, st);
 #pragma unroll
   for (int k = 0; k < GC; k++) p.w[k] = words[k];
+#if NL_STAMP
+  asm volatile("" : "+v"(p.mine));
+#endif
+  st(CLS_PH_EPILOGUE);
 }
 
 template <int IDC, int NW>
 __device__ __forceinline__ void class_search(const SweepArgs<float>& a, const ClsCtx<IDC>& c, const Pos<float>* tile, int lane, int wave,
-                                             PipePending& p) {
+                                             PipePending& p, ClsStamp& st) {
   constexpr int G = PIPE_G, NP = IDC / 2, WP = NW / NP;
   static_assert(NW % NP == 0, "waves a pair of classes");
   const int32_t ntiles = (c.total_j + WAVE - 1) / WAVE;
@@ -207,51 +218,65 @@
       const int32_t i0 = g * gbase + min(g, grem);
       const int32_t gcount = gbase + (g < grem ? 1 : 0);
       if (gcount <= 0) break;
-      pipe_flush<NW == SWEEP_WAVES>(a, p, lane, hi);
+      pipe_flush<(NW > 2)>(a, p, lane, hi);
+      st(CLS_PH_FLUSH);
       const int32_t kk = min(lane, gcount - 1);
       Pos<float> pi_l = tile[own + i0 + kk];
       const int32_t row_l = pi_l.gid;
       if (lane >= gcount) pi_l.x = 0, pi_l.y = 0, pi_l.z = 0, pi_l.gid = 0;
       switch (gcount) {
-        case 1: class_pipe_group<1>(a, tile, t0, tsplit, ntiles, lane, pi_l, p); break;
-        case 2: class_pipe_group<2>(a, tile, t0, tsplit, ntiles, lane, pi_l, p); break;
-        case 3: class_pipe_group<3>(a, tile, t0, tsplit, ntiles, lane, pi_l, p); break;
-        case 4: class_pipe_group<4>(a, tile, t0, tsplit, ntiles, lane, pi_l, p); break;
-        case 5: class_pipe_group<5>(a, tile, t0, tsplit, ntiles, lane, pi_l, p); break;
-        case 6: class_pipe_group<6>(a, tile, t0, tsplit, ntiles, lane, pi_l, p); break;
-        default: class_pipe_group<7>(a, tile, t0, tsplit, ntiles, lane, pi_l, p); break;
+        case 1: class_pipe_group<1>(a, tile, t0, tsplit, ntiles, lane, pi_l, p, st); break;
+        case 2: class_pipe_group<2>(a, tile, t0, tsplit, ntiles, lane, pi_l, p, st); break;
+        case 3: class_pipe_group<3>(a, tile, t0, tsplit, ntiles, lane, pi_l, p, st); break;
+        case 4: class_pipe_group<4>(a, tile, t0, tsplit, ntiles, lane, pi_l, p, st); break;
+        case 5: class_pipe_group<5>(a, tile, t0, tsplit, ntiles, lane, pi_l, p, st); break;
+        case 6: class_pipe_group<6>(a, tile, t0, tsplit, ntiles, lane, pi_l, p, st); break;
+        default: class_pipe_group<7>(a, tile, t0, tsplit, ntiles, lane, pi_l, p, st); break;
       }
       p.row_l = row_l, p.slot0 = slot_b + i0, p.gcount = gcount;
     }
   }
 }
 
-template <int IDC, int NW = SWEEP_WAVES, int CAP = SweepCfg<float>::CAP>
+constexpr int CLS3_WAVES = 3, CLS3_CAP = 1024;
+template <int IDC, int NW = SWEEP_WAVES, int CAP = SweepCfg<float>::CAP, bool REG = false>
 __global__ void __launch_bounds__(NW* WAVE, 8) __attribute__((amdgpu_num_sgpr(80))) k_sweep_class_f32(SweepArgs<float> a) {
   if (gate_closed(a.gate)) return;
   __shared__ __attribute__((aligned(32))) Pos<float> buf[CAP];
+  static_assert(REG || CAP == SweepCfg<float>::CAP, "the LDS-DMA form stages the whole stream");
   const int tid = threadIdx.x, lane = tid & 63, wave = __builtin_amdgcn_readfirstlane(tid >> 6);
   __builtin_amdgcn_s_setprio(NL_PRIO);
+  ClsStamp st;
   ClsCtx<IDC> c;
   if (!cls_setup<IDC>(a, lane, c)) return;
-  if (c.total_j > CAP) {
+  if (c.total_j > SweepCfg<float>::CAP) {
     if (tid == 0) a.full27_list[atomicAdd(a.full27_count, 1)] = c.cx + (c.cy + c.cz * a.my) * a.mx;
     return;
   }
-  cls_stage<IDC, NW>(a.sorted, c, buf, lane, wave);
-  const int32_t pad = c.total_j + tid;
-  if (pad < ((c.total_j + WAVE - 1) & ~(WAVE - 1))) {
-    Pos<float> sentinel;
-    sentinel.x = 1.0e18f, sentinel.y = 0.f, sentinel.z = 0.f, sentinel.gid = INT32_MIN;
-    buf[pad] = sentinel;
-  }
-  asm volatile("s_waitcnt vmcnt(0) lgkmcnt(0)\n\ts_barrier" ::: "memory");
-  if (a.cull_bits) cls_cull<IDC, NW, CAP>(a, c, buf, c.cx + (c.cy + c.cz * a.my) * a.mx, tid, lane, wave);
+  st(CLS_PH_TABLE);
+  if constexpr (REG) {
+    if (!cls_cull_reg<IDC, NW, CAP>(a, c, buf, c.cx + (c.cy + c.cz * a.my) * a.mx, tid, lane, wave, st)) return;
+  } else {
+    cls_stage<IDC, NW>(a.sorted, c, buf, lane, wave);
+    const int32_t pad = c.total_j + tid;
+    if (pad < ((c.total_j + WAVE - 1) & ~(WAVE - 1))) {
+      Pos<float> sentinel;
+      sentinel.x = 1.0e18f, sentinel.y = 0.f, sentinel.z = 0.f, sentinel.gid = INT32_MIN;
+      buf[pad] = sentinel;
+    }
+    st(CLS_PH_ISSUED);
+    asm volatile("s_waitcnt vmcnt(0) lgkmcnt(0)\n\ts_barrier" ::: "memory");
+    st(CLS_PH_LANDED);
+    if (a.cull_bits) cls_cull<IDC, NW, CAP>(a, c, buf, c.cx + (c.cy + c.cz * a.my) * a.mx, tid, lane, wave, st);
+  }
   PipePending pend;
   pend.gcount = 0, pend.mine = 0, pend.row_l = 0, pend.slot0 = 0;
-  class_search<IDC, NW>(a, c, buf, lane, wave, pend);
-  pipe_flush<NW == SWEEP_WAVES>(a, pend, lane, hi_plane_used(1, (c.total_j + WAVE - 1) / WAVE));
-}
+  class_search<IDC, NW>(a, c, buf, lane, wave, pend, st);
+  pipe_flush<(NW > 2)>(a, pend, lane, hi_plane_used(1, (c.total_j + WAVE - 1) / WAVE));
+  st(CLS_PH_FLUSH);
+  st.write(a.dbg_buf, lane);
+}
+
 
 template <bool FULL>
 __global__ void __launch_bounds__(SWEEP_WAVES* WAVE) __attribute__((amdgpu_num_sgpr(80))) k_sweep_list_f32(SweepArgs<float> a) {
diff --git a/md_neighbor_list_amd/neighlist.py b/md_neighbor_list_amd/neighlist.py
--- a/md_neighbor_list_amd/neighlist.py
+++ b/md_neighbor_list_amd/neighlist.py
@@ -584,7 +584,8 @@
                 "offset_bits": int(info[4]), "mask_rows": int(info[5]), "fine_rows": int(info[6]),
                 "small_cells": int(info[7]) & 0xFF, "id_classes": int(info[7]) >> 8 & 0xFF,
                 "binning": ("two_pass", "bucket", "atomic")[int(info[7]) >> 16 & 3],
-                "reach_cull": bool(int(info[7]) >> 18 & 1)}
+                "reach_cull": bool(int(info[7]) >> 18 & 1), "count_waves": int(info[7]) >> 19 & 7,
+                "count_staging": ("registers" if int(info[7]) >> 22 & 1 else "lds") if int(info[7]) >> 19 & 7 else ""}
 
     def build_stats(self):
         st = (C.c_int64 * 4)()
```

Measured after the change: 169,300. -6.9%, worse.
